# Farama-Foundation/Gymnasium-Robotics

Measured on AMD Instinct MI355X. Metric: env-steps/s (whole node), higher is better.
Workload: dtype f32

## Files before the change

__graft_entry__.py:

```python
import os
import subprocess
import sys

ROOT = os.path.dirname(os.path.abspath(__file__))
sys.path.insert(0, ROOT)

HIP_SRC = os.path.join(ROOT, "gymnasium_robotics_amd", "csrc", "grx_kernels.hip")
import glob

HIP_DEPS = sorted(glob.glob(os.path.join(ROOT, "gymnasium_robotics_amd", "csrc", "*.h")) + glob.glob(os.path.join(ROOT, "include", "*")))
HIP_SO = os.path.join(ROOT, "gymnasium_robotics_amd", "_lib", "libgrx_hip.so")
ENV_SRC = os.path.join(ROOT, "gymnasium_robotics_amd", "csrc", "grx_env.hip")
ENV_DEPS = [os.path.join(ROOT, "include", "grx_env.h"), os.path.join(ROOT, "include", "grx_replay.h"), os.path.join(ROOT, "include", "grx_capi.h"),
            os.path.join(ROOT, "gymnasium_robotics_amd", "csrc", "grx_env_maze.inc"), os.path.join(ROOT, "gymnasium_robotics_amd", "csrc", "grx_env_replay.inc")]
ENV_SO = os.path.join(ROOT, "gymnasium_robotics_amd", "_lib", "libgrx_env.so")


HIPCC_FLAGS = ["--offload-arch=gfx950", "-O3", "-std=c++17", "-shared", "-fPIC", "-fno-hip-fp32-correctly-rounded-divide-sqrt"]
HIP_UNITS = ("FETCH", "HAND", "POINT", "ADROIT", "KITCHEN", "API")


def _stale(target, deps):
    return not os.path.exists(target) or any(os.path.getmtime(d) > os.path.getmtime(target) for d in deps)


def build_hip(out=HIP_SO, extra_flags=()):
    hipcc = os.environ.get("HIPCC", "/opt/rocm/bin/hipcc")
    objdir = os.path.join(os.path.dirname(out), ".obj_" + os.path.splitext(os.path.basename(out))[0])
    os.makedirs(objdir, exist_ok=True)
    compile_flags = [f for f in HIPCC_FLAGS if f != "-shared"] + list(extra_flags)
    procs = []
    for u in HIP_UNITS:
        obj = os.path.join(objdir, f"grx_{u.lower()}.o")
        procs.append((obj, subprocess.Popen([hipcc] + compile_flags + [f"-DGRX_TU_{u}=1", "-c", "-o", obj, HIP_SRC])))
    for obj, p in procs:
        if p.wait() != 0:
            raise subprocess.CalledProcessError(p.returncode, p.args)
    subprocess.check_call([hipcc, "--offload-arch=gfx950", "-shared", "-fPIC", "-o", out] + [o for o, _ in procs])


def build_env(out=ENV_SO):
    hipcc = os.environ.get("HIPCC", "/opt/rocm/bin/hipcc")
    subprocess.check_call([hipcc, "--offload-arch=gfx950", "-O3", "-std=c++17", "-shared", "-fPIC", "-I", os.path.join(ROOT, "include"), "-o", out, ENV_SRC,
                           "-L", os.path.dirname(HIP_SO), "-lgrx_hip", "-Wl,-rpath,$ORIGIN"])


def build(force: bool = False) -> None:
    os.makedirs(os.path.dirname(HIP_SO), exist_ok=True)
    if force or _stale(HIP_SO, [HIP_SRC] + HIP_DEPS):
        build_hip()
    if force or _stale(ENV_SO, [ENV_SRC, HIP_SO] + ENV_DEPS):
        build_env()
    from oracle import oracle_sim

    oracle_sim.build(force)
    sys.path.insert(0, os.path.join(ROOT, "tests", "emu"))
    import emu_sim

    emu_sim.build(force)
    import gymnasium_robotics_amd
    from gymnasium_robotics_amd import _native

    _native.lib()


def smoke() -> None:
    import numpy as np
# ... 31 lines not shown
```

gymnasium_robotics_amd/_native.py:

```python
import ctypes
import os

_HERE = os.path.dirname(os.path.abspath(__file__))
LIB_PATH = os.environ.get("GRX_HIP_LIB") or os.path.join(_HERE, "_lib", "libgrx_hip.so")
_lib = None


class OverflowLaneStruct(ctypes.Structure):
    _fields_ = [(n, ctypes.c_void_p) for n in ("skip", "entry_count", "entry_list", "list", "count", "next_flags", "next_count", "next_list", "ttl")] + [
        (n, ctypes.c_int) for n in ("soft_maxefc", "soft_jpool", "soft_maxcon", "ttl_init", "grid", "entry_cap", "next_cap")] + [
        (n, ctypes.c_void_p) for n in ("ready", "progress", "poll_list")] + [(n, ctypes.c_int) for n in ("ready_cap", "progress_total", "poll_grid", "pad_")]


class FetchBuffersStruct(ctypes.Structure):
    _fields_ = [(n, ctypes.c_void_p) for n in (
        "qpos", "qvel", "qacc_ws", "mocap", "aux", "goal", "action", "obs", "achieved", "reward", "success", "status", "mask", "order", "cost", "packed", "hullcache", "handoff")] + [
        ("handoff_stride", ctypes.c_int), ("handoff_large", ctypes.c_int), ("split_state", ctypes.c_void_p), ("split_parts", ctypes.c_int), ("split_pad_", ctypes.c_int), ("lane", OverflowLaneStruct)]


class FetchResetArgsStruct(ctypes.Structure):
    _fields_ = [(n, ctypes.c_void_p) for n in ("idx", "samples", "init_qpos", "init_qvel", "init_mocap")] + [("obj_qadr", ctypes.c_int), ("keep_outcome", ctypes.c_int), ("final_packed", ctypes.c_void_p)]


class PointTaskStruct(ctypes.Structure):
    _fields_ = [("n_substeps", ctypes.c_int), ("sparse_reward", ctypes.c_int), ("continuing_task", ctypes.c_int), ("agent", ctypes.c_int),
                ("goal_radius", ctypes.c_double), ("vel_clip", ctypes.c_float)]


class PointBuffersStruct(ctypes.Structure):
    _fields_ = [(n, ctypes.c_void_p) for n in (
        "qpos", "qvel", "qacc_ws", "goal", "action", "obs", "achieved", "reward", "success", "terminated", "status", "mask", "packed", "split_state")] + [
        ("split_parts", ctypes.c_int), ("split_pad_", ctypes.c_int)]


class AdroitTaskStruct(ctypes.Structure):
    _fields_ = [("n_substeps", ctypes.c_int), ("sparse_reward", ctypes.c_int), ("kind", ctypes.c_int), ("site", ctypes.c_int * 5), ("obj_body", ctypes.c_int),
                ("nq_obs", ctypes.c_int), ("obs_dim", ctypes.c_int), ("qadr", ctypes.c_int * 2), ("len", ctypes.c_float * 2)]


class AdroitBuffersStruct(ctypes.Structure):
    _fields_ = [(n, ctypes.c_void_p) for n in ("qpos", "qvel", "qacc_ws", "shift", "target", "action", "act_mean", "act_rng", "obs", "reward", "success", "status", "mask")] + [("lane", OverflowLaneStruct), ("compact", ctypes.c_void_p), ("n_compact", ctypes.c_int), ("order", ctypes.c_void_p), ("cost", ctypes.c_void_p), ("split_rows", ctypes.c_void_p), ("split_state", ctypes.c_void_p), ("split_stride", ctypes.c_int), ("split_parts", ctypes.c_int)]


class KitchenTaskStruct(ctypes.Structure):
    _fields_ = [("n_substeps", ctypes.c_int), ("obs_dim", ctypes.c_int), ("dt", ctypes.c_float), ("vel_lo", ctypes.c_float * 9), ("vel_hi", ctypes.c_float * 9),
                ("pos_lo", ctypes.c_float * 9), ("pos_hi", ctypes.c_float * 9), ("noise_scale", ctypes.c_float * 59), ("task_adr", ctypes.c_int * 7),
                ("task_num", ctypes.c_int * 7), ("task_goal", ctypes.c_float * 17), ("bonus_thresh", ctypes.c_float)]


class KitchenBuffersStruct(ctypes.Structure):
    _fields_ = [(n, ctypes.c_void_p) for n in ("qpos", "qvel", "qacc_ws", "last_qpos", "action", "noise", "obs", "completed", "status", "mask", "skin")] + [
        ("skin_stride", ctypes.c_int), ("skin_radius", ctypes.c_float), ("order", ctypes.c_void_p), ("cost", ctypes.c_void_p), ("lane", OverflowLaneStruct),
        ("split_rows", ctypes.c_void_p), ("split_state", ctypes.c_void_p), ("split_stride", ctypes.c_int), ("split_parts", ctypes.c_int)]


class KitchenBookStruct(ctypes.Structure):
    _fields_ = [(n, ctypes.c_void_p) for n in ("completed", "stepped", "tasks_to_complete", "episode_completions", "elapsed", "step_completions", "reward", "terminated",
                                               "truncated", "needs_reset", "reset_now", "qpos", "qvel", "qacc_ws", "init_qpos")] + [
        (n, ctypes.c_int) for n in ("nq", "nv", "all_mask", "max_steps", "remove_when_completed", "terminate_when_completed", "mode")] + [("final_info", ctypes.c_void_p)]


class HerArgsStruct(ctypes.Structure):
    _fields_ = [("rows", ctypes.c_void_p), ("acts", ctypes.c_void_p)] + [(n, ctypes.c_int) for n in ("T", "N", "W", "obs_dim", "goal_dim", "act_dim")] + [
        (n, ctypes.c_void_p) for n in ("t_idx", "w_idx", "t_goal")] + [("kind", ctypes.c_int), ("p0", ctypes.c_double), ("p1", ctypes.c_double)] + [
        (n, ctypes.c_int) for n in ("sparse", "ignore_pos", "ignore_rot", "ignore_z")] + [("out", ctypes.c_void_p), ("term_rows", ctypes.c_void_p), ("term_t", ctypes.c_void_p)]


class MazeResetArgsStruct(ctypes.Structure):
    _fields_ = [(n, ctypes.c_void_p) for n in ("idx", "stage", "qpos0")] + [(n, ctypes.c_int) for n in ("nq", "nv", "obs_dim", "obs_skip")] + [
        ("goal_radius", ctypes.c_double), ("keep_outcome", ctypes.c_int)] + [
        (n, ctypes.c_void_p) for n in ("qpos", "qvel", "qacc_ws", "goal", "obs", "achieved", "reward", "success", "packed")]


class HandCommitArgsStruct(ctypes.Structure):
    _fields_ = [("idx", ctypes.c_void_p), ("k", ctypes.c_int)] + [(n, ctypes.c_int) for n in ("nq", "nv", "obs_dim", "goal_dim")] + [
        (n, ctypes.c_void_p) for n in ("s_qpos", "s_qvel", "s_qacc_ws", "s_obs", "s_achieved", "s_palm", "s_goal", "s_packed", "s_status",
                                       "qpos", "qvel", "qacc_ws", "obs", "achieved", "palm", "goal", "packed", "status")]


class FetchCommitArgsStruct(ctypes.Structure):
    _fields_ = [("idx", ctypes.c_void_p), ("k", ctypes.c_int)] + [(n, ctypes.c_int) for n in ("nq", "nv", "mocap_words", "obs_dim")] + [
        (n, ctypes.c_void_p) for n in ("s_qpos", "s_qvel", "s_qacc_ws", "s_mocap", "s_aux", "s_goal", "s_obs", "s_achieved", "s_status",
                                       "qpos", "qvel", "qacc_ws", "mocap", "aux", "goal", "obs", "achieved", "packed", "final_packed", "status")]


class AdroitCommitArgsStruct(ctypes.Structure):
    _fields_ = [("idx", ctypes.c_void_p), ("k", ctypes.c_int)] + [(n, ctypes.c_int) for n in ("nq", "nv", "obs_dim")] + [
        (n, ctypes.c_void_p) for n in ("s_qpos", "s_qvel", "s_qacc_ws", "s_shift", "s_target", "s_obs", "s_status", "qpos", "qvel", "qacc_ws", "shift", "target", "obs", "status")]


class HandBuffersStruct(ctypes.Structure):
    _fields_ = [(n, ctypes.c_void_p) for n in (
        "qpos", "qvel", "qacc_ws", "goal", "action", "obs", "achieved", "palm", "reward", "success", "status", "mask", "order", "cost", "packed")] + [("lane", OverflowLaneStruct),
        ("split_rows", ctypes.c_void_p), ("split_state", ctypes.c_void_p), ("split_stride", ctypes.c_int), ("split_parts", ctypes.c_int)]


def lib():
    global _lib
    if _lib is None:
        if not os.path.exists(LIB_PATH):
            raise RuntimeError(
                f"HIP extension not built: {LIB_PATH} is missing. Run `python -c 'import __graft_entry__ as g; g.build()'` "
                "(hipcc --offload-arch=gfx950). There is no CPU fallback.")
        import torch

        L = ctypes.CDLL(LIB_PATH)
        vp, ci = ctypes.c_void_p, ctypes.c_int
        L.grx_last_error.restype = ctypes.c_char_p
        L.grx_model_create.argtypes = [vp, ci, vp, ci, vp, ci, ci, ctypes.POINTER(vp)]
        L.grx_model_destroy.argtypes = [vp]
        L.grx_model_set_table.argtypes = [vp, ctypes.c_char_p, vp, ci]
        L.grx_model_lds_bytes.argtypes = [vp]
        L.grx_model_dim.argtypes = [vp, ctypes.c_char_p]
        L.grx_fetch_step.argtypes = [vp, vp, vp, ci, vp]
        L.grx_fetch_forward.argtypes = [vp, vp, vp, ci, ci, vp]
        L.grx_fetch_reset.argtypes = [vp, vp, vp, vp, ci, vp]
        L.grx_fetch_compute_reward.argtypes = [vp, vp, ctypes.c_int64, ctypes.c_double, ci, vp, vp]
        L.grx_her_relabel.argtypes = [vp, ctypes.c_int64, vp]
        L.grx_her_sample.argtypes = [vp, ci, ci, ci, ci, ctypes.c_uint64, ctypes.c_uint64, ctypes.c_int64, vp, vp, vp, vp]
        L.grx_her_sample_final.argtypes = [vp, vp, vp, ci, ci, ci, ci, ctypes.c_uint64, ctypes.c_uint64, ctypes.c_int64, vp, vp, vp, vp]
        L.grx_her_mark_resets.argtypes = [vp, ci, ci, vp, vp, vp, vp]
        L.grx_her_sample_relabel.argtypes = [vp, vp, vp, ci, ci, ctypes.c_uint64, ctypes.c_uint64, ctypes.c_int64, vp, vp, vp]
        L.grx_kitchen_step.argtypes = [vp, vp, vp, ci, ci, vp]
        L.grx_sample_uniform_rows.argtypes = [vp, vp, ci, ci, vp]
        L.grx_uniform_rows_device.argtypes = [vp, vp, ci, ci, vp, vp]
        L.grx_kitchen_bookkeeping.argtypes = [vp, ci, vp]
        L.grx_point_step.argtypes = [vp, vp, vp, ci, vp]
        L.grx_maze_compute_reward.argtypes = [vp, vp, ctypes.c_int64, ctypes.c_double, ci, vp, vp]
        L.grx_hand_step.argtypes = [vp, vp, vp, ci, ci, vp]
        L.grx_hand_step_repeat.argtypes = [vp, vp, vp, ci, ci, vp]
        L.grx_adroit_step.argtypes = [vp, vp, vp, ci, ci, vp]
        L.grx_goal_compute_reward.argtypes = [vp, vp, ctypes.c_int64, ci, ctypes.c_double, ci, vp, vp]
        L.grx_manip_compute_reward.argtypes = [vp, vp, ctypes.c_int64, ci, ci, ci, ctypes.c_float, ctypes.c_float, ci, vp, vp]
        L.grx_order_by_cost.argtypes = [vp, vp, ctypes.c_float, ci, vp, vp]
        L.grx_order_by_cost_slots.argtypes = [vp, vp, ctypes.c_float, ci, ci, vp, vp]
        L.grx_maze_reset_rows.argtypes = [vp, ci, vp]
        L.grx_hand_commit_rows.argtypes = [vp, vp]
        L.grx_fetch_commit_rows.argtypes = [vp, vp]
        L.grx_adroit_commit_rows.argtypes = [vp, vp]
        cd = ctypes.c_double
        L.grx_fetch_sample_resets.argtypes = [vp, vp, ci, ci, ci, cd, cd, vp, vp, cd, vp, vp]
        L.grx_fetch_sample_resets_device.argtypes = [vp, vp, ci, ci, ci, cd, cd, vp, vp, cd, vp, vp]
        L.grx_adroit_sample_resets_device.argtypes = [vp, vp, ci, ci, vp, vp, vp, vp, vp, vp]
        L.grx_maze_sample_resets_device.argtypes = [vp, vp, ci, vp, ci, vp, ci, cd, cd, vp, vp, vp, vp]
        _lib = L
    return _lib


def build_id(path: str = None) -> str:
    import hashlib
    import struct

    with open(path or LIB_PATH, "rb") as f:
        blob = f.read()
    if blob[:4] != b"\x7fELF" or blob[4] != 2:
        raise RuntimeError("libgrx_hip.so is not an ELF64 file")
    shoff, = struct.unpack_from("<Q", blob, 0x28)
    shentsize, shnum, shstrndx = struct.unpack_from("<HHH", blob, 0x3A)
    sec = lambda i: struct.unpack_from("<IIQQQQIIQQ", blob, shoff + i * shentsize)
    stroff = sec(shstrndx)[4]
    for i in range(shnum):
        name, _, _, _, off, size = sec(i)[:6]
        end = blob.index(b"\0", stroff + name)
        if blob[stroff + name: end] == b".hip_fatbin":
            return hashlib.sha256(blob[off: off + size]).hexdigest()[:16]
    raise RuntimeError("libgrx_hip.so holds no .hip_fatbin section (not a HIP build)")


def check(rc: int):
    if rc != 0:
        raise RuntimeError("libgrx_hip: " + lib().grx_last_error().decode())


EXPORTED_SYMBOLS = [
    "grx_model_create", "grx_model_destroy", "grx_model_set_table", "grx_model_lds_bytes", "grx_model_dim",
    "grx_fetch_step", "grx_fetch_forward", "grx_fetch_reset", "grx_fetch_compute_reward", "grx_her_relabel", "grx_her_sample", "grx_her_sample_final", "grx_her_mark_resets", "grx_her_sample_relabel", "grx_fetch_sample_resets", "grx_fetch_sample_resets_device", "grx_adroit_sample_resets_device", "grx_maze_sample_resets_device", "grx_point_step", "grx_maze_compute_reward", "grx_hand_step", "grx_hand_step_repeat", "grx_adroit_step", "grx_kitchen_step", "grx_sample_uniform_rows", "grx_uniform_rows_device", "grx_kitchen_bookkeeping", "grx_goal_compute_reward", "grx_manip_compute_reward", "grx_order_by_cost", "grx_order_by_cost_slots", "grx_maze_reset_rows", "grx_maze_reset_rows_list", "grx_maze_sample_resets_list", "grx_maze_episode_end", "grx_hand_commit_rows", "grx_fetch_commit_rows", "grx_adroit_commit_rows", "grx_last_error",
]


_MODEL_LOCK = __import__("threading").Lock()
_MODELS = {}
_MODEL_KEYS = {}


def acquire_model(H, I, F, device_index):
    import hashlib

    key = (int(device_index), hashlib.sha1(H.tobytes() + I.tobytes() + F.tobytes()).hexdigest(), os.environ.get("GRX_NO_HULLCELLS") is not None)
    with _MODEL_LOCK:
        ent = _MODELS.get(key)
        if ent is None:
            h = ctypes.c_void_p()
            check(lib().grx_model_create(H.ctypes.data, H.size, I.ctypes.data, I.size, F.ctypes.data, F.size, int(device_index), ctypes.byref(h)))
            ent = _MODELS[key] = [h, 0]
            _MODEL_KEYS[h.value] = key
        ent[1] += 1
        return ent[0]


def release_model(h):
    if h is None or not getattr(h, "value", None):
        return
    with _MODEL_LOCK:
        key = _MODEL_KEYS.get(h.value)
        if key is None:
            return
        ent = _MODELS[key]
        ent[1] -= 1
        if ent[1] <= 0:
            del _MODELS[key], _MODEL_KEYS[h.value]
            lib().grx_model_destroy(h)
```

gymnasium_robotics_amd/csrc/grx_env.hip:

```cpp
#include <hip/hip_runtime.h>

#include <sys/random.h>

#include <cstdio>
#include <cstring>
#include <map>
#include <string>
#include <vector>

#include "grx_capi.h"
#include "grx_env.h"
#include "grx_replay.h"

namespace {

constexpr int kEntryCap = 256;
constexpr int kSplitParts = 4;
constexpr int kSplitWide = 12288;
constexpr double kLaneMargin = 0.8;
constexpr int kLaneTtl = 4;
constexpr float kBalanceAlpha = 0.1f;
constexpr int kHullWords = 90;
constexpr int kPinSlots = 16;

thread_local std::string g_err;
int fail(int code, const std::string& msg) { g_err = msg; return code; }

#define ENV_HIP(expr) do { hipError_t e_ = (expr); if (e_ != hipSuccess) return fail(GRX_ENV_EHIP, std::string(#expr) + ": " + hipGetErrorString(e_)); } while (0)
#define ENV_GRX(expr) do { if ((expr) != 0) return fail(GRX_ENV_EHIP, std::string(#expr) + ": " + grx_last_error()); } while (0)
#define ENV_TRY(expr) do { int r_ = (expr); if (r_ != 0) return r_; } while (0)

__global__ void __launch_bounds__(64) grx_env_mask_kernel(unsigned char* __restrict__ mask, const int* __restrict__ idx, int k) {
  const int j = blockIdx.x * 64 + threadIdx.x;
  if (j < k) mask[idx[j]] = 0;
}

__global__ void __launch_bounds__(64) grx_env_zero_outcome_kernel(float* __restrict__ reward, float* __restrict__ packed, int pdim, const int* __restrict__ idx, int k) {
  const int j = blockIdx.x * 64 + threadIdx.x;
  if (j >= k) return;
  const int w = idx[j];
  reward[w] = 0.0f;
  packed[(size_t)w * pdim + pdim - 2] = 0.0f;
}

__global__ void __launch_bounds__(64) grx_env_gather_kernel(float* __restrict__ rows, const float* __restrict__ src, int width, const int* __restrict__ idx, int k) {
  const int j = blockIdx.x * 64 + threadIdx.x;
  if (j >= k) return;
  const float* s = src + (size_t)idx[j] * width;
  float* d = rows + (size_t)j * width;
  for (int c = 0; c < width; ++c) d[c] = s[c];
}

__global__ void __launch_bounds__(64) grx_env_scatter_rng_kernel(unsigned long long* __restrict__ rng, const unsigned long long* __restrict__ rows, const int* __restrict__ idx, int k) {
  const int j = blockIdx.x * 64 + threadIdx.x;
  if (j >= k) return;
  for (int c = 0; c < 4; ++c) rng[(size_t)idx[j] * 4 + c] = rows[(size_t)j * 4 + c];
}

unsigned blocks(int k) { return (unsigned)((k + 63) / 64); }

void pcg64_from_entropy(const std::vector<uint32_t>& ent, uint64_t out[4]) {
  const uint32_t INIT_A = 0x43b0d7e5u, MULT_A = 0x931e8875u, INIT_B = 0x8b51f9ddu, MULT_B = 0x58f38dedu, MIX_L = 0xca01f9ddu, MIX_R = 0x4973f715u;
  uint32_t hc = INIT_A, pool[4];
  auto hashmix = [&hc, MULT_A](uint32_t v) { v ^= hc; hc *= MULT_A; v *= hc; v ^= v >> 16; return v; };
  auto mix = [MIX_L, MIX_R](uint32_t x, uint32_t y) { uint32_t r = MIX_L * x - MIX_R * y; r ^= r >> 16; return r; };
// ... 119 lines not shown
struct MazeEnv;
void maze_free(MazeEnv* m);

int parse_desc(const Container& c, Desc* d) {
  ENV_TRY(take<int32_t>(c, "H", -1, &d->H));
  ENV_TRY(take<int32_t>(c, "I", -1, &d->I));
  ENV_TRY(take<double>(c, "F", -1, &d->F));
  ENV_TRY(take<int32_t>(c, "H_rerun", (int64_t)(d->H.size() * 4), &d->Hr));
  ENV_TRY(take<int32_t>(c, "I_rerun", (int64_t)(d->I.size() * 4), &d->Ir));
  ENV_TRY(take<double>(c, "F_rerun", (int64_t)(d->F.size() * 8), &d->Fr));
  ENV_TRY(take<uint8_t>(c, "task", sizeof(grx_fetch_task), nullptr, &d->task));
  ENV_TRY(take<int32_t>(c, "dims", sizeof d->dims, nullptr, d->dims));
  ENV_TRY(take<double>(c, "consts", sizeof d->consts, nullptr, d->consts));
  ENV_TRY(take<int32_t>(c, "fast_caps", sizeof d->caps, nullptr, d->caps));
  const int nq = d->dims[0], nv = d->dims[1], nmocap = d->dims[2], obs_dim = d->dims[4];
  if (nq <= 0 || nv <= 0 || nmocap != 1 || obs_dim != d->task.obs_dim || d->task.goal_dim != 3 || d->dims[5] >= nq)
    return fail(GRX_ENV_EDESC, "environment description: inconsistent sizes: dims (nq " + std::to_string(nq) + ", nv " + std::to_string(nv) + ", nmocap " + std::to_string(nmocap) +
                                   ", obs_dim " + std::to_string(obs_dim) + ") disagree with the task struct (obs_dim " + std::to_string(d->task.obs_dim) + ")");
  ENV_TRY(take<double>(c, "q0", (int64_t)nq * 8, &d->q0));
  ENV_TRY(take<double>(c, "mocap0", (int64_t)nmocap * 56, &d->mocap0));
  return 0;
}

}

struct grx_env {
  int device = 0, n = 0, mode = GRX_ENV_NEXT_STEP, max_steps = 0;
  uint64_t seed_offset = 0;
  Desc d;
  MazeEnv* mz = nullptr;
  grx_model *h = nullptr, *hbig = nullptr;
  int nq = 0, nv = 0, nmocap = 0, nu = 0, obs_dim = 0, pdim = 0, obj_qadr = -1;
  double g0[3] = {0, 0, 0}, toff[3] = {0, 0, 0}, height_offset = 0, dt = 0;
  int soft[4] = {0, 0, 0, 0};
  std::vector<void*> allocs;
  float *qpos, *qvel, *qacc_ws, *mocap, *aux, *goal, *action, *obs, *achieved, *reward, *packed, *final_packed, *final_rows, *hullcache, *cost_ema = nullptr;
  unsigned char *success, *mask;
  int *status, *cost = nullptr, *order = nullptr;
  float* split_rows = nullptr;
  int* split_state = nullptr;
  uint64_t *rng, *rng_rows;
  float *init_qpos, *init_qvel, *init_mocap;
  int *idx_main, *idx_ahead;
  float *samp_main, *samp_ahead;
  int* lane_head;
  int *lane_next_list, *lane_entry_list;
  signed char* lane_ttl;
  size_t lane_head_bytes = 0;
  float *a_qpos, *a_qvel, *a_qacc_ws, *a_mocap, *a_aux, *a_goal, *a_obs, *a_achieved, *a_reward;
  unsigned char* a_success;
  int* a_status;
  grx_fetch_buffers bufs{}, bufs_masked{}, lane_plain{}, lane_masked{}, ahead_bufs{};
  bool balance = false, ahead = false;
  int slots_per_xcd = 0, split = 1;
  hipStream_t side = nullptr;
  hipEvent_t ev_before = nullptr, ev_ahead = nullptr;
  void* pin[kPinSlots] = {};
  hipEvent_t pin_ev[kPinSlots] = {};
  bool pin_live[kPinSlots] = {};
  size_t pin_bytes = 0;
  int pin_next = 0;
  std::vector<int64_t> elapsed;
  std::vector<uint8_t> needs_reset, terminated, truncated;
  std::vector<int32_t> final_idx, list, will;
  int n_final = 0;
  uint8_t has_reset = 0;
  grx_replay* replay = nullptr;
  const int* step_list = nullptr;
  const int* step_count_dev = nullptr;
  int step_count = 0;
  uint64_t steps = 0, epoch = 0;

  ~grx_env() {
    (void)hipSetDevice(device);
    if (side) (void)hipStreamSynchronize(side);
    (void)hipDeviceSynchronize();
    for (int s = 0; s < kPinSlots; ++s) {
      if (pin_ev[s]) (void)hipEventDestroy(pin_ev[s]);
      if (pin[s]) (void)hipHostFree(pin[s]);
    }
    if (ev_before) (void)hipEventDestroy(ev_before);
    if (ev_ahead) (void)hipEventDestroy(ev_ahead);
    if (side) (void)hipStreamDestroy(side);
    for (void* p : allocs) (void)hipFree(p);
    if (h) grx_model_destroy(h);
    if (hbig) grx_model_destroy(hbig);
    maze_free(mz);
  }

  template <class T>
  int zalloc(T** p, size_t count) {
    void* q = nullptr;
    ENV_HIP(hipMalloc(&q, count * sizeof(T) > 0 ? count * sizeof(T) : 1));
    allocs.push_back(q);
    ENV_HIP(hipMemset(q, 0, count * sizeof(T)));
    *p = (T*)q;
    return 0;
  }

  int upload(void* dst, const void* src, size_t bytes, hipStream_t s) {
    if (bytes == 0) return 0;
    const int k = pin_next;
    pin_next = (pin_next + 1) % kPinSlots;
    if (pin_live[k] && hipEventQuery(pin_ev[k]) == hipErrorNotReady) ENV_HIP(hipEventSynchronize(pin_ev[k]));
    std::memcpy(pin[k], src, bytes);
    ENV_HIP(hipMemcpyAsync(dst, pin[k], bytes, hipMemcpyHostToDevice, s));
    ENV_HIP(hipEventRecord(pin_ev[k], s));
    pin_live[k] = true;
    return 0;
  }
};

namespace {

struct DeviceGuard {
  int prev = -1;
  explicit DeviceGuard(int dev) { if (hipGetDevice(&prev) != hipSuccess) prev = -1; if (prev != dev) (void)hipSetDevice(dev); }
  ~DeviceGuard() { int cur; if (prev >= 0 && hipGetDevice(&cur) == hipSuccess && cur != prev) (void)hipSetDevice(prev); }
};

grx_fetch_buffers make_bufs(grx_env* e, float* qpos, float* qvel, float* qacc, float* mocap, float* aux, float* goal, float* obs, float* ach, float* rew, unsigned char* succ,
                            int* status, const unsigned char* mask, const int* order, int* cost, float* packed, float* hullcache) {
  grx_fetch_buffers b;
  std::memset(&b, 0, sizeof b);
  b.qpos = qpos; b.qvel = qvel; b.qacc_ws = qacc; b.mocap = mocap; b.aux = aux; b.goal = goal; b.action = e->action; b.obs = obs; b.achieved = ach;
  b.reward = rew; b.success = succ; b.status = status; b.mask = mask; b.order = order; b.cost = cost; b.packed = packed; b.hullcache = hullcache;
  return b;
}

int launch_step(grx_env* e, bool masked, hipStream_t s) {
  grx_fetch_buffers& fb = masked ? e->bufs_masked : e->bufs;
  ENV_HIP(hipMemsetAsync(e->lane_head, 0, e->lane_head_bytes, s));
  int* counts = e->lane_head + (e->lane_head_bytes / 4 - 2);
  std::memset(&fb.lane, 0, sizeof fb.lane);
  fb.lane.entry_count = counts + 1; fb.lane.entry_list = e->lane_entry_list; fb.lane.entry_cap = kEntryCap;
  const int rc = grx_fetch_step(e->h, &e->d.task, &fb, e->n, s);
  std::memset(&fb.lane, 0, sizeof fb.lane);
  if (rc != 0) return fail(GRX_ENV_EHIP, std::string("grx_fetch_step: ") + grx_last_error());
  grx_fetch_buffers& b = masked ? e->lane_masked : e->lane_plain;
  std::memset(&b.lane, 0, sizeof b.lane);
  b.lane.grid = kEntryCap; b.lane.list = e->lane_entry_list; b.lane.count = counts + 1;
  b.lane.next_flags = (unsigned char*)e->lane_head; b.lane.next_count = counts; b.lane.next_list = e->lane_next_list; b.lane.ttl = e->lane_ttl; b.lane.next_cap = 0;
  b.lane.soft_maxefc = e->soft[0]; b.lane.soft_jpool = e->soft[1]; b.lane.soft_maxcon = e->soft[2]; b.lane.ttl_init = e->soft[3];
  ENV_GRX(grx_fetch_step(e->hbig, &e->d.task, &b, e->n, s));
  if (e->balance) ENV_GRX(grx_order_by_cost_slots(e->cost, e->cost_ema, kBalanceAlpha, e->n, e->slots_per_xcd, e->order, s));
  return 0;
}

int sample_resets(grx_env* e, const int* idx_dev, int k, float* samples, hipStream_t s) {
  const double* c = e->d.consts;
  ENV_GRX(grx_fetch_sample_resets_device(e->rng, idx_dev, k, (int)c[0], (int)c[2], c[7], c[8], e->toff, e->g0, e->height_offset, samples, s));
  return 0;
}

int reset_inline(grx_env* e, const int* idx_dev, int k, const float* samples, bool keep_outcome, hipStream_t s) {
  grx_fetch_reset_args a;
  std::memset(&a, 0, sizeof a);
  a.idx = idx_dev; a.samples = samples; a.init_qpos = e->init_qpos; a.init_qvel = e->init_qvel; a.init_mocap = e->init_mocap; a.obj_qadr = e->obj_qadr;
  a.keep_outcome = keep_outcome ? 1 : 0; a.final_packed = keep_outcome ? e->final_packed : nullptr;
  ENV_GRX(grx_fetch_reset(e->h, &e->d.task, &e->bufs, &a, k, s));
  return 0;
}

void mark_reset(grx_env* e, const std::vector<int32_t>& idx) {
  for (int w : idx) { e->elapsed[w] = 0; e->needs_reset[w] = 0; }
}

int env_setup(grx_env* e) {
  grx_env one;
  one.device = e->device;
  float *qpos, *qvel, *qacc, *mocap, *aux, *goal, *action, *obs, *ach, *rew, *packed, *hull;
  unsigned char* succ;
  int* status;
  ENV_TRY(one.zalloc(&qpos, e->nq)); ENV_TRY(one.zalloc(&qvel, e->nv)); ENV_TRY(one.zalloc(&qacc, e->nv)); ENV_TRY(one.zalloc(&mocap, 7 * e->nmocap));
  ENV_TRY(one.zalloc(&aux, 8)); ENV_TRY(one.zalloc(&goal, 3)); ENV_TRY(one.zalloc(&action, 4)); ENV_TRY(one.zalloc(&obs, e->obs_dim)); ENV_TRY(one.zalloc(&ach, 3));
  ENV_TRY(one.zalloc(&rew, 1)); ENV_TRY(one.zalloc(&succ, 1)); ENV_TRY(one.zalloc(&status, 1)); ENV_TRY(one.zalloc(&packed, e->pdim)); ENV_TRY(one.zalloc(&hull, kHullWords));
  one.action = action;
  grx_fetch_buffers b = make_bufs(&one, qpos, qvel, qacc, mocap, aux, goal, obs, ach, rew, succ, status, nullptr, nullptr, nullptr, packed, hull);
  std::vector<float> q0(e->d.q0.begin(), e->d.q0.end()), m0(e->d.mocap0.begin(), e->d.mocap0.end());
  ENV_HIP(hipMemcpy(qpos, q0.data(), q0.size() * 4, hipMemcpyHostToDevice));
  ENV_HIP(hipMemcpy(mocap, m0.data(), m0.size() * 4, hipMemcpyHostToDevice));
  hipStream_t s = e->side;
  ENV_GRX(grx_fetch_forward(e->h, &e->d.task, &b, 1, 0, s));
  ENV_HIP(hipStreamSynchronize(s));
  float o[3];
  ENV_HIP(hipMemcpy(o, obs, 12, hipMemcpyDeviceToHost));
  const double geh = e->d.consts[3];
  const double target[3] = {-0.498 + (double)o[0], 0.005 + (double)o[1], (-0.431 + geh) + (double)o[2]};
  const float mrow[7] = {(float)target[0], (float)target[1], (float)target[2], 1.0f, 0.0f, 1.0f, 0.0f};
  ENV_HIP(hipMemcpy(mocap, mrow, sizeof mrow, hipMemcpyHostToDevice));
  ENV_GRX(grx_fetch_forward(e->h, &e->d.task, &b, 1, 10 * e->d.task.n_substeps, s));
  ENV_HIP(hipStreamSynchronize(s));
  int st = 0;
  float a[3];
  ENV_HIP(hipMemcpy(&st, status, 4, hipMemcpyDeviceToHost));
  if (st != 0) return fail(GRX_ENV_EHIP, "engine reported status " + std::to_string(st) + " during env setup");
  ENV_HIP(hipMemcpy(o, obs, 12, hipMemcpyDeviceToHost));
  ENV_HIP(hipMemcpy(a, ach, 12, hipMemcpyDeviceToHost));
  for (int i = 0; i < 3; ++i) e->g0[i] = (double)o[i];
  e->height_offset = e->d.consts[0] != 0.0 ? (double)a[2] : 0.0;
  ENV_HIP(hipMemcpy(e->init_qpos, qpos, e->nq * 4, hipMemcpyDeviceToDevice));
  ENV_HIP(hipMemcpy(e->init_qvel, qvel, e->nv * 4, hipMemcpyDeviceToDevice));
  ENV_HIP(hipMemcpy(e->init_mocap, m0.data(), m0.size() * 4, hipMemcpyHostToDevice));
  return 0;
}

int alloc_all(grx_env* e) {
  const int n = e->n;
  ENV_TRY(e->zalloc(&e->qpos, (size_t)n * e->nq)); ENV_TRY(e->zalloc(&e->qvel, (size_t)n * e->nv)); ENV_TRY(e->zalloc(&e->qacc_ws, (size_t)n * e->nv));
  ENV_TRY(e->zalloc(&e->mocap, (size_t)n * 7 * e->nmocap)); ENV_TRY(e->zalloc(&e->aux, (size_t)n * 8)); ENV_TRY(e->zalloc(&e->goal, (size_t)n * 3));
  ENV_TRY(e->zalloc(&e->action, (size_t)n * 4)); ENV_TRY(e->zalloc(&e->obs, (size_t)n * e->obs_dim)); ENV_TRY(e->zalloc(&e->achieved, (size_t)n * 3));
  ENV_TRY(e->zalloc(&e->reward, n)); ENV_TRY(e->zalloc(&e->success, n)); ENV_TRY(e->zalloc(&e->status, n)); ENV_TRY(e->zalloc(&e->mask, n));
  ENV_HIP(hipMemset(e->mask, 1, n));
  ENV_TRY(e->zalloc(&e->packed, (size_t)n * e->pdim)); ENV_TRY(e->zalloc(&e->final_packed, (size_t)n * e->pdim)); ENV_TRY(e->zalloc(&e->final_rows, (size_t)n * e->pdim));
  ENV_TRY(e->zalloc(&e->hullcache, (size_t)n * kHullWords));
  ENV_TRY(e->zalloc(&e->rng, (size_t)n * 4)); ENV_TRY(e->zalloc(&e->rng_rows, (size_t)n * 4));
  ENV_TRY(e->zalloc(&e->init_qpos, e->nq)); ENV_TRY(e->zalloc(&e->init_qvel, e->nv)); ENV_TRY(e->zalloc(&e->init_mocap, 7 * e->nmocap));
  ENV_TRY(e->zalloc(&e->idx_main, n)); ENV_TRY(e->zalloc(&e->idx_ahead, n)); ENV_TRY(e->zalloc(&e->samp_main, (size_t)n * 5)); ENV_TRY(e->zalloc(&e->samp_ahead, (size_t)n * 5));
  e->lane_head_bytes = (size_t)((n + 3) / 4 + 2) * 4;
  ENV_TRY(e->zalloc(&e->lane_head, e->lane_head_bytes / 4)); ENV_TRY(e->zalloc(&e->lane_next_list, n)); ENV_TRY(e->zalloc(&e->lane_entry_list, n)); ENV_TRY(e->zalloc(&e->lane_ttl, n));
  e->balance = n % 8 == 0 && n >= 1024 && n <= 65536 * 8;
  if (e->balance) {
    ENV_TRY(e->zalloc(&e->cost, n)); ENV_TRY(e->zalloc(&e->cost_ema, n)); ENV_TRY(e->zalloc(&e->order, n));
    const int lds = grx_model_lds_bytes(e->h);
    const int granules = (lds + 1279) / 1280;
    const int per_cu = granules > 0 ? (160 * 1024) / (granules * 1280) : 8;
    e->slots_per_xcd = 32 * (per_cu < 8 ? per_cu : 8);
    std::vector<int> ord(n);
    const int per = n / 8;
    for (int j = 0; j < n; ++j) ord[j] = (j % 8) * per + j / 8;
    ENV_HIP(hipMemcpy(e->order, ord.data(), (size_t)n * 4, hipMemcpyHostToDevice));
  }
  e->bufs = make_bufs(e, e->qpos, e->qvel, e->qacc_ws, e->mocap, e->aux, e->goal, e->obs, e->achieved, e->reward, e->success, e->status, nullptr, e->order, e->cost, e->packed, e->hullcache);
  e->bufs_masked = e->bufs;
  e->bufs_masked.mask = e->mask;
  e->lane_plain = make_bufs(e, e->qpos, e->qvel, e->qacc_ws, e->mocap, e->aux, e->goal, e->obs, e->achieved, e->reward, e->success, e->status, nullptr, nullptr, nullptr, e->packed,
                            e->hullcache);
  e->lane_masked = e->lane_plain;
  e->lane_masked.mask = e->mask;
  e->split = n >= 64 && n > 2048 ? (n <= kSplitWide ? kSplitParts : 2) : 1;
  if (e->split > 1) {
    const int stride = (2 + e->nu + 7 * e->nmocap + e->nq + 2 * e->nv + 15) / 16 * 16;
    ENV_TRY(e->zalloc(&e->split_rows, (size_t)n * stride)); ENV_TRY(e->zalloc(&e->split_state, (size_t)n * 2));
    for (grx_fetch_buffers* b : {&e->bufs, &e->bufs_masked}) { b->handoff = e->split_rows; b->handoff_stride = stride; b->split_state = e->split_state; b->split_parts = e->split; }
  }
  e->ahead = n > 1;
  if (e->ahead) {
    ENV_TRY(e->zalloc(&e->a_qpos, (size_t)n * e->nq)); ENV_TRY(e->zalloc(&e->a_qvel, (size_t)n * e->nv)); ENV_TRY(e->zalloc(&e->a_qacc_ws, (size_t)n * e->nv));
    ENV_TRY(e->zalloc(&e->a_mocap, (size_t)n * 7 * e->nmocap)); ENV_TRY(e->zalloc(&e->a_aux, (size_t)n * 8)); ENV_TRY(e->zalloc(&e->a_goal, (size_t)n * 3));
    ENV_TRY(e->zalloc(&e->a_obs, (size_t)n * e->obs_dim)); ENV_TRY(e->zalloc(&e->a_achieved, (size_t)n * 3)); ENV_TRY(e->zalloc(&e->a_reward, n));
    ENV_TRY(e->zalloc(&e->a_success, n)); ENV_TRY(e->zalloc(&e->a_status, n));
    e->ahead_bufs = make_bufs(e, e->a_qpos, e->a_qvel, e->a_qacc_ws, e->a_mocap, e->a_aux, e->a_goal, e->a_obs, e->a_achieved, e->a_reward, e->a_success, e->a_status, nullptr,
                              nullptr, nullptr, nullptr, nullptr);
  }
  e->pin_bytes = (size_t)n * 32;
  for (int s = 0; s < kPinSlots; ++s) {
    ENV_HIP(hipHostMalloc(&e->pin[s], e->pin_bytes, hipHostMallocDefault));
    ENV_HIP(hipEventCreateWithFlags(&e->pin_ev[s], hipEventDisableTiming));
  }
  ENV_HIP(hipEventCreateWithFlags(&e->ev_before, hipEventDisableTiming));
  ENV_HIP(hipEventCreateWithFlags(&e->ev_ahead, hipEventDisableTiming));
  e->elapsed.assign(n, 0);
  e->needs_reset.assign(n, 0);
  e->terminated.assign(n, 0);
  e->truncated.assign(n, 0);
  e->final_idx.reserve(n);
  e->list.reserve(n);
  e->will.reserve(n);
  return 0;
}

struct Section { const char* name; void* ptr; size_t bytes; bool host; };

#include "grx_env_maze.inc"
// ... 154 lines not shown
  auto& L = e->list;
  L.clear();
  for (int i = 0; i < e->n; ++i)
    if (!mask || mask[i]) L.push_back(i);
  e->n_final = 0;
  std::fill(e->terminated.begin(), e->terminated.end(), 0);
  std::fill(e->truncated.begin(), e->truncated.end(), 0);
  e->has_reset = 1;
  const int k = (int)L.size();
  if (k == 0) return 0;
  ENV_TRY(e->upload(e->idx_main, L.data(), (size_t)k * 4, s));
  if (seeds) {
    std::vector<uint64_t> rows((size_t)k * 4);
    for (int j = 0; j < k; ++j) pcg64_from_seed(seeds[L[j]], &rows[(size_t)j * 4]);
    ENV_TRY(e->upload(e->rng_rows, rows.data(), rows.size() * 8, s));
    hipLaunchKernelGGL(grx_env_scatter_rng_kernel, dim3(blocks(k)), dim3(64), 0, s, (unsigned long long*)e->rng, (const unsigned long long*)e->rng_rows, e->idx_main, k);
    ENV_HIP(hipGetLastError());
  }
  ENV_TRY(sample_resets(e, e->idx_main, k, e->samp_main, s));
  ENV_TRY(reset_inline(e, e->idx_main, k, e->samp_main, false, s));
  mark_reset(e, L);
  return 0;
}

extern "C" int grx_env_step(grx_env* e, const float* actions, void* stream) {
  if (!e) return fail(GRX_ENV_EINVAL, "grx_env_step: NULL handle");
  if (!actions) return fail(GRX_ENV_EINVAL, "grx_env_step: actions is NULL");
  if (!e->has_reset) return fail(GRX_ENV_EINVAL, "grx_env_step: cannot step before grx_env_reset");
  DeviceGuard g(e->device);
  hipStream_t s = (hipStream_t)stream;
  e->steps += 1;
  e->step_list = nullptr; e->step_count_dev = nullptr; e->step_count = 0;
  if (e->mz) return maze_step(e, actions, s);
  const int n = e->n;
  ENV_HIP(hipMemcpyAsync(e->action, actions, (size_t)n * 16, hipMemcpyDefault, s));
  auto& pending = e->list;
  pending.clear();
  if (e->mode == GRX_ENV_NEXT_STEP)
    for (int i = 0; i < n; ++i)
      if (e->needs_reset[i]) pending.push_back(i);
  auto& will = e->will;
  will.clear();
  if (e->ahead && e->mode == GRX_ENV_SAME_STEP && e->max_steps > 0)
    for (int i = 0; i < n; ++i)
      if (e->elapsed[i] + 1 >= e->max_steps) will.push_back(i);
  const int kp = (int)pending.size(), kw = (int)will.size();
  if (kw) ENV_HIP(hipEventRecord(e->ev_before, s));
  if (kp) {
    ENV_TRY(e->upload(e->idx_main, pending.data(), (size_t)kp * 4, s));
    ENV_HIP(hipMemsetAsync(e->mask, 1, n, s));
    hipLaunchKernelGGL(grx_env_mask_kernel, dim3(blocks(kp)), dim3(64), 0, s, e->mask, (const int*)e->idx_main, kp);
    ENV_HIP(hipGetLastError());
  }
  ENV_TRY(launch_step(e, kp > 0, s));
  if (kw) {
    ENV_HIP(hipStreamWaitEvent(e->side, e->ev_before, 0));
    ENV_TRY(e->upload(e->idx_ahead, will.data(), (size_t)kw * 4, e->side));
    ENV_TRY(sample_resets(e, e->idx_ahead, kw, e->samp_ahead, e->side));
    grx_fetch_reset_args a;
    std::memset(&a, 0, sizeof a);
    a.idx = e->idx_ahead; a.samples = e->samp_ahead; a.init_qpos = e->init_qpos; a.init_qvel = e->init_qvel; a.init_mocap = e->init_mocap; a.obj_qadr = e->obj_qadr;
    a.keep_outcome = 1; a.final_packed = nullptr;
    ENV_GRX(grx_fetch_reset(e->h, &e->d.task, &e->ahead_bufs, &a, kw, e->side));
    ENV_HIP(hipEventRecord(e->ev_ahead, e->side));
  }
  e->n_final = 0;
  e->final_idx.clear();
  for (int i = 0; i < n; ++i) {
    const bool stepped = !(kp && e->needs_reset[i]);
    if (stepped) e->elapsed[i] += 1;
    e->truncated[i] = stepped && e->max_steps > 0 && e->elapsed[i] >= e->max_steps;
    e->terminated[i] = 0;
    if (e->truncated[i]) e->final_idx.push_back(i);
  }
  if (kp) {
    ENV_TRY(sample_resets(e, e->idx_main, kp, e->samp_main, s));
    ENV_TRY(reset_inline(e, e->idx_main, kp, e->samp_main, false, s));
    mark_reset(e, pending);
    e->step_list = e->idx_main; e->step_count = kp;
    hipLaunchKernelGGL(grx_env_zero_outcome_kernel, dim3(blocks(kp)), dim3(64), 0, s, e->reward, e->packed, e->pdim, (const int*)e->idx_main, kp);
    ENV_HIP(hipGetLastError());
  }
  const int kd = (int)e->final_idx.size();
  if (e->mode == GRX_ENV_SAME_STEP && kd) {
    const int* idx_dev;
    if (kw) {
      if (kw != kd || !std::equal(will.begin(), will.end(), e->final_idx.begin()))
        return fail(GRX_ENV_EINVAL, "grx_env_step: the worlds reset ahead of the step are not the ones it truncated");
      ENV_HIP(hipStreamWaitEvent(s, e->ev_ahead, 0));
      grx_fetch_commit_args c;
      std::memset(&c, 0, sizeof c);
      c.idx = e->idx_ahead; c.k = kd; c.nq = e->nq; c.nv = e->nv; c.mocap_words = 7 * e->nmocap; c.obs_dim = e->obs_dim;
      c.s_qpos = e->a_qpos; c.s_qvel = e->a_qvel; c.s_qacc_ws = e->a_qacc_ws; c.s_mocap = e->a_mocap; c.s_aux = e->a_aux; c.s_goal = e->a_goal; c.s_obs = e->a_obs;
      c.s_achieved = e->a_achieved; c.s_status = e->a_status;
      c.qpos = e->qpos; c.qvel = e->qvel; c.qacc_ws = e->qacc_ws; c.mocap = e->mocap; c.aux = e->aux; c.goal = e->goal; c.obs = e->obs; c.achieved = e->achieved;
      c.packed = e->packed; c.final_packed = e->final_packed; c.status = e->status;
      ENV_GRX(grx_fetch_commit_rows(&c, s));
      idx_dev = e->idx_ahead;
    } else {
      ENV_TRY(e->upload(e->idx_main, e->final_idx.data(), (size_t)kd * 4, s));
      ENV_TRY(sample_resets(e, e->idx_main, kd, e->samp_main, s));
      ENV_TRY(reset_inline(e, e->idx_main, kd, e->samp_main, true, s));
      idx_dev = e->idx_main;
    }
    mark_reset(e, e->final_idx);
    hipLaunchKernelGGL(grx_env_gather_kernel, dim3(blocks(kd)), dim3(64), 0, s, e->final_rows, (const float*)e->final_packed, e->pdim, idx_dev, kd);
    ENV_HIP(hipGetLastError());
    e->n_final = kd;
    e->step_list = idx_dev; e->step_count = kd;
  } else {
    if (e->mode == GRX_ENV_NEXT_STEP)
      for (int w : e->final_idx) e->needs_reset[w] = 1;
    e->final_idx.clear();
  }
  return 0;
}

extern "C" int grx_env_outputs(const grx_env* e, grx_env_device_outputs* out) {
  if (!e || !out) return fail(GRX_ENV_EINVAL, "grx_env_outputs: NULL argument");
  if (e->mz) return maze_outputs(e, out);
  out->num_envs = e->n; out->obs_dim = e->obs_dim; out->goal_dim = 3; out->packed_dim = e->pdim;
  out->obs = e->obs; out->achieved = e->achieved; out->desired = e->goal; out->reward = e->reward; out->success = e->success; out->status = e->status; out->packed = e->packed;
  out->terminated = e->terminated.data(); out->truncated = e->truncated.data();
  out->n_final = e->n_final; out->final_idx = e->final_idx.data(); out->final_rows = e->final_rows;
  return 0;
}

extern "C" int grx_env_copy_outputs(grx_env* e, grx_env_host_outputs* out) {
  if (!e || !out) return fail(GRX_ENV_EINVAL, "grx_env_copy_outputs: NULL argument");
  DeviceGuard g(e->device);
  if (e->mz) return maze_copy_outputs(e, out);
  ENV_HIP(hipDeviceSynchronize());
  const size_t n = e->n;
  auto d2h = [](void* dst, const void* src, size_t bytes) { return (dst && bytes) ? hipMemcpy(dst, src, bytes, hipMemcpyDeviceToHost) : hipSuccess; };
  ENV_HIP(d2h(out->obs, e->obs, n * e->obs_dim * 4));
  ENV_HIP(d2h(out->achieved, e->achieved, n * 12));
  ENV_HIP(d2h(out->desired, e->goal, n * 12));
  ENV_HIP(d2h(out->reward, e->reward, n * 4));
  ENV_HIP(d2h(out->success, e->success, n));
  ENV_HIP(d2h(out->status, e->status, n * 4));
  ENV_HIP(d2h(out->packed, e->packed, n * e->pdim * 4));
  ENV_HIP(d2h(out->final_rows, e->final_rows, (size_t)e->n_final * e->pdim * 4));
  if (out->terminated) std::memcpy(out->terminated, e->terminated.data(), n);
  if (out->truncated) std::memcpy(out->truncated, e->truncated.data(), n);
  if (out->n_final) *out->n_final = e->n_final;
  if (out->final_idx && e->n_final) std::memcpy(out->final_idx, e->final_idx.data(), (size_t)e->n_final * 4);
  return 0;
}

extern "C" int grx_env_compute_reward(const grx_env* e, const float* achieved, const float* desired, int64_t batch, float* out, void* stream) {
  if (!e || !achieved || !desired || !out) return fail(GRX_ENV_EINVAL, "grx_env_compute_reward: NULL argument");
  if (batch < 0) return fail(GRX_ENV_EINVAL, "grx_env_compute_reward: negative batch");
  DeviceGuard g(e->device);
  if (e->mz) {
    ENV_GRX(grx_maze_compute_reward(achieved, desired, batch, e->mz->d.task.goal_radius, e->mz->d.task.sparse_reward, out, stream));
    return 0;
  }
  ENV_GRX(grx_fetch_compute_reward(achieved, desired, batch, e->d.task.distance_threshold, e->d.task.sparse_reward, out, stream));
  return 0;
}

extern "C" int grx_env_state_size(const grx_env* e, size_t* bytes) {
  if (!e || !bytes) return fail(GRX_ENV_EINVAL, "grx_env_state_size: NULL argument");
  *bytes = state_layout(const_cast<grx_env*>(e), nullptr);
  return 0;
}

// ... 63 lines not shown
```

gymnasium_robotics_amd/csrc/grx_env_replay.inc:

```

struct grx_replay {
  grx_env* e = nullptr;
  int T = 0, R = 0, n = 0, W = 0, od = 0, gd = 0, ad = 0, OW = 0;
  int64_t capacity = 0, max_batch = 0, head = 0, size = 0;
  uint64_t seed = 0, calls = 0;
  bool track = false;
  float *episode = nullptr, *actions = nullptr, *rows = nullptr, *term_rows = nullptr;
  int *start = nullptr, *prev_start = nullptr, *term_t = nullptr, *scratch = nullptr, *valid = nullptr;
  std::vector<void*> allocs;
  int t = 0;
  bool begun = false;
  uint64_t epoch = 0, last_step = 0;
  grx_her_args ha{};
};

namespace {

struct ReplayAppend {
  const float *packed, *action;
  float *row_dst, *act_dst;
  long long n_row, n_act;
  const int* list;
  const int* count_dev;
  int count, max_n, t;
  int *start, *prev_start, *term_t;
  const float* final_rows;
  float* term_rows;
  int W;
};

__device__ __forceinline__ void replay_copy(float* __restrict__ dst, const float* __restrict__ src, long long n, long long tid, long long nth) {
  if ((((uintptr_t)dst | (uintptr_t)src) & 15) == 0) {
    const long long n4 = n >> 2;
    const float4* __restrict__ s4 = (const float4*)src;
    float4* __restrict__ d4 = (float4*)dst;
    for (long long i = tid; i < n4; i += nth) d4[i] = s4[i];
    for (long long i = (n4 << 2) + tid; i < n; i += nth) dst[i] = src[i];
  } else {
    for (long long i = tid; i < n; i += nth) dst[i] = src[i];
  }
}

__global__ void __launch_bounds__(256) grx_replay_append_kernel(ReplayAppend a) {
  const long long tid = (long long)blockIdx.x * blockDim.x + threadIdx.x, nth = (long long)gridDim.x * blockDim.x;
  replay_copy(a.row_dst, a.packed, a.n_row, tid, nth);
  replay_copy(a.act_dst, a.action, a.n_act, tid, nth);
  int k = a.count_dev ? *a.count_dev : a.count;
  k = k < 0 ? 0 : (k > a.max_n ? a.max_n : k);
  for (long long j = tid; j < k; j += nth) {
    const int w = a.list[j];
    if ((unsigned)w >= (unsigned)a.max_n) continue;
    if (a.prev_start) { a.prev_start[w] = a.start[w]; a.term_t[w] = a.t; }
    a.start[w] = a.t;
  }
  if (a.term_rows)
    for (long long i = tid; i < (long long)k * a.W; i += nth) {
      const long long j = i / a.W;
      const int w = a.list[j];
      if ((unsigned)w < (unsigned)a.max_n) a.term_rows[(size_t)w * a.W + (i - j * a.W)] = a.final_rows[i];
    }
}

__global__ void __launch_bounds__(256) grx_replay_begin_kernel(const float* __restrict__ packed, float* __restrict__ row0, long long n_row, const long long* __restrict__ elapsed, int n,
                                                               int* __restrict__ start, int* __restrict__ prev_start, int* __restrict__ term_t) {
  const long long tid = (long long)blockIdx.x * blockDim.x + threadIdx.x, nth = (long long)gridDim.x * blockDim.x;
  replay_copy(row0, packed, n_row, tid, nth);
  for (long long w = tid; w < n; w += nth) {
    if (elapsed) start[w] = -(int)elapsed[w];
    prev_start[w] = 0;
    term_t[w] = -1;
  }
}

unsigned replay_blocks(long long words) {
  long long b = (words / 4 + 255) / 256;
  return (unsigned)(b < 1 ? 1 : (b > 1024 ? 1024 : b));
}

const float* replay_packed(const grx_env* e) { return e->mz ? e->mz->packed : e->packed; }
const float* replay_action(const grx_env* e) { return e->mz ? e->mz->action : e->action; }

template <class T>
int replay_zalloc(grx_replay* r, T** p, size_t count) {
  void* q = nullptr;
  ENV_HIP(hipMalloc(&q, count * sizeof(T) > 0 ? count * sizeof(T) : 1));
  r->allocs.push_back(q);
  ENV_HIP(hipMemset(q, 0, count * sizeof(T)));
  *p = (T*)q;
  return 0;
}

void replay_free(grx_replay* r) {
  for (void* p : r->allocs) (void)hipFree(p);
  delete r;
}

}

extern "C" int grx_replay_create(grx_env* e, const grx_replay_config* cfg, grx_replay** out) {
  if (!out) return fail(GRX_ENV_EINVAL, "grx_replay_create: out is NULL");
  *out = nullptr;
  if (!cfg) return fail(GRX_ENV_EINVAL, "grx_replay_create: NULL config");
  if (cfg->horizon < 1 || cfg->horizon > (1 << 20)) return fail(GRX_ENV_EINVAL, "grx_replay_create: horizon " + std::to_string(cfg->horizon) + " out of range (>= 1)");
  if (cfg->capacity < 1) return fail(GRX_ENV_EINVAL, "grx_replay_create: capacity " + std::to_string(cfg->capacity) + " out of range (>= 1)");
  if (cfg->max_batch > cfg->capacity)
    return fail(GRX_ENV_EINVAL, "grx_replay_create: batch " + std::to_string(cfg->max_batch) + " larger than the replay capacity " + std::to_string(cfg->capacity));
  if (!e) return fail(GRX_ENV_EINVAL, "grx_replay_create: NULL handle");
  if (e->replay) return fail(GRX_ENV_EINVAL, "grx_replay_create: the handle already has a replay attached");
  DeviceGuard g(e->device);
  grx_replay* r = new grx_replay();
  r->e = e;
  r->T = cfg->horizon; r->R = r->T + 1; r->n = e->n; r->W = e->pdim; r->od = e->obs_dim; r->gd = e->mz ? 2 : 3; r->ad = e->mz ? e->mz->nu : 4;
  r->OW = 2 * r->od + 3 * r->gd + r->ad + 2;
  r->capacity = cfg->capacity; r->max_batch = cfg->max_batch > 0 ? cfg->max_batch : cfg->capacity;
  r->seed = cfg->seed;
  r->track = cfg->keep_final != 0 && e->mode == GRX_ENV_SAME_STEP;
  const size_t n = (size_t)r->n;
  int rc = [&]() -> int {
    ENV_TRY(replay_zalloc(r, &r->episode, (size_t)r->R * n * r->W));
    ENV_TRY(replay_zalloc(r, &r->actions, (size_t)r->R * n * r->ad));
    ENV_TRY(replay_zalloc(r, &r->rows, (size_t)r->capacity * r->OW));
    ENV_TRY(replay_zalloc(r, &r->start, n)); ENV_TRY(replay_zalloc(r, &r->prev_start, n)); ENV_TRY(replay_zalloc(r, &r->term_t, n));
    ENV_TRY(replay_zalloc(r, &r->scratch, (size_t)3 * r->max_batch)); ENV_TRY(replay_zalloc(r, &r->valid, 1));
    ENV_HIP(hipMemset(r->term_t, 0xFF, n * 4));
    if (r->track) {
      if (e->mz) ENV_TRY(replay_zalloc(r, &r->term_rows, n * r->W));
      else r->term_rows = e->final_packed;
    }
    ENV_HIP(hipDeviceSynchronize());
    return 0;
  }();
  if (rc != 0) { std::string msg = g_err; replay_free(r); g_err = msg; return rc; }
  grx_her_args& a = r->ha;
  std::memset(&a, 0, sizeof a);
  a.rows = r->episode; a.acts = r->actions; a.T = r->T; a.N = r->n; a.W = r->W; a.obs_dim = r->od; a.goal_dim = r->gd; a.act_dim = r->ad;
  if (e->mz) { a.kind = 2; a.p0 = e->mz->d.task.goal_radius; a.sparse = e->mz->d.task.sparse_reward; }
  else { a.kind = 0; a.p0 = e->d.task.distance_threshold; a.sparse = e->d.task.sparse_reward; }
  if (r->track) { a.term_rows = r->term_rows; a.term_t = r->term_t; }
  e->replay = r;
  *out = r;
  return 0;
}

extern "C" int grx_replay_destroy(grx_replay* r) {
  if (!r) return fail(GRX_ENV_EINVAL, "grx_replay_destroy: NULL replay");
  DeviceGuard g(r->e->device);
  (void)hipDeviceSynchronize();
  r->e->replay = nullptr;
  replay_free(r);
  return 0;
}

extern "C" int grx_replay_dims(const grx_replay* r, int* row_width, int* obs_dim, int* goal_dim, int* act_dim) {
  if (!r) return fail(GRX_ENV_EINVAL, "grx_replay_dims: NULL replay");
  if (row_width) *row_width = r->OW;
  if (obs_dim) *obs_dim = r->od;
  if (goal_dim) *goal_dim = r->gd;
  if (act_dim) *act_dim = r->ad;
  return 0;
}

extern "C" int grx_replay_begin(grx_replay* r, void* stream) {
  if (!r) return fail(GRX_ENV_EINVAL, "grx_replay_begin: NULL replay");
  grx_env* e = r->e;
  if (!e->has_reset) return fail(GRX_ENV_EINVAL, "grx_replay_begin: cannot begin before grx_env_reset");
  DeviceGuard g(e->device);
  hipStream_t s = (hipStream_t)stream;
  const long long* elapsed_dev = nullptr;
  if (e->mz && !e->mz->host_book) elapsed_dev = e->mz->elapsed;
  else {
    const std::vector<int64_t>& el = e->mz ? e->mz->h_elapsed : e->elapsed;
    std::vector<int32_t> neg((size_t)r->n);
    for (int i = 0; i < r->n; ++i) neg[i] = -(int32_t)el[i];
    ENV_TRY(e->upload(r->start, neg.data(), (size_t)r->n * 4, s));
  }
  const long long n_row = (long long)r->n * r->W;
  hipLaunchKernelGGL(grx_replay_begin_kernel, dim3(replay_blocks(n_row)), dim3(256), 0, s, replay_packed(e), r->episode, n_row, elapsed_dev, r->n, r->start, r->prev_start, r->term_t);
  ENV_HIP(hipGetLastError());
  r->t = 0;
  r->begun = true;
  r->epoch = e->epoch;
  r->last_step = e->steps;
  return 0;
}

extern "C" int grx_replay_append(grx_replay* r, void* stream) {
  if (!r) return fail(GRX_ENV_EINVAL, "grx_replay_append: NULL replay");
  grx_env* e = r->e;
  if (!r->begun) return fail(GRX_ENV_EINVAL, "grx_replay_append: append before grx_replay_begin");
  if (e->epoch != r->epoch) return fail(GRX_ENV_EINVAL, "grx_replay_append: grx_env_reset / grx_env_set_state since grx_replay_begin: call grx_replay_begin again");
  if (e->steps == r->last_step) return fail(GRX_ENV_EINVAL, "grx_replay_append: no grx_env_step since the last append (double append)");
  if (e->steps != r->last_step + 1) return fail(GRX_ENV_EINVAL, "grx_replay_append: " + std::to_string(e->steps - r->last_step) + " steps since the last append: every step is appended");
  if (r->t == INT32_MAX - 1) return fail(GRX_ENV_EINVAL, "grx_replay_append: row counter exhausted: call grx_replay_begin");
  DeviceGuard g(e->device);
  const int t = r->t + 1, row = t % r->R;
  ReplayAppend a;
  std::memset(&a, 0, sizeof a);
  a.packed = replay_packed(e); a.action = replay_action(e);
  a.n_row = (long long)r->n * r->W; a.n_act = (long long)r->n * r->ad;
  a.row_dst = r->episode + (size_t)row * a.n_row; a.act_dst = r->actions + (size_t)row * a.n_act;
  a.list = e->step_list; a.count_dev = e->step_count_dev; a.count = e->step_list ? e->step_count : 0; a.max_n = r->n; a.t = t;
  a.start = r->start;
  if (r->track) {
    a.prev_start = r->prev_start; a.term_t = r->term_t;
    if (e->mz) { a.final_rows = e->mz->final_rows; a.term_rows = r->term_rows; }
  }
  a.W = r->W;
  hipLaunchKernelGGL(grx_replay_append_kernel, dim3(replay_blocks(a.n_row)), dim3(256), 0, (hipStream_t)stream, a);
  ENV_HIP(hipGetLastError());
  r->t = t;
  r->last_step = e->steps;
  return 0;
}

extern "C" int grx_replay_relabel(grx_replay* r, int64_t batch, int k_future, grx_replay_batch* out, void* stream) {
  if (!r) return fail(GRX_ENV_EINVAL, "grx_replay_relabel: NULL replay");
  if (batch < 1) return fail(GRX_ENV_EINVAL, "grx_replay_relabel: batch " + std::to_string(batch) + " out of range (>= 1)");
  if (batch > r->capacity) return fail(GRX_ENV_EINVAL, "grx_replay_relabel: batch " + std::to_string(batch) + " larger than the replay capacity " + std::to_string(r->capacity));
  if (batch > r->max_batch) return fail(GRX_ENV_EINVAL, "grx_replay_relabel: batch " + std::to_string(batch) + " larger than max_batch " + std::to_string(r->max_batch));
  if (k_future < 0) return fail(GRX_ENV_EINVAL, "grx_replay_relabel: negative k_future");
  DeviceGuard g(r->e->device);
  if (r->head + batch > r->capacity) r->head = 0;
  grx_her_args a = r->ha;
  a.out = r->rows + (size_t)r->head * r->OW;
  ENV_GRX(grx_her_sample_relabel(&a, r->start, r->track ? r->prev_start : nullptr, r->t, k_future, r->seed, r->calls, batch, r->scratch, r->valid, stream));
  r->calls += 1;
  if (out) { out->rows = a.out; out->batch = batch; out->offset = r->head; out->valid = r->valid; }
  r->head += batch;
  if (r->head > r->size) r->size = r->head;
  return 0;
}

extern "C" int grx_replay_reseed(grx_replay* r, uint64_t seed) {
  if (!r) return fail(GRX_ENV_EINVAL, "grx_replay_reseed: NULL replay");
  r->seed = seed;
  r->calls = 0;
  return 0;
}

extern "C" int grx_replay_ring(const grx_replay* r, const float** rows, int64_t* capacity, int64_t* head, int64_t* size) {
  if (!r) return fail(GRX_ENV_EINVAL, "grx_replay_ring: NULL replay");
  if (rows) *rows = r->rows;
  if (capacity) *capacity = r->capacity;
  if (head) *head = r->head;
  if (size) *size = r->size;
  return 0;
}
```

gymnasium_robotics_amd/csrc/grx_kernels.hip:

```cpp
#if !defined(GRX_TU_FETCH) && !defined(GRX_TU_HAND) && !defined(GRX_TU_POINT) && !defined(GRX_TU_ADROIT) && !defined(GRX_TU_KITCHEN) && !defined(GRX_TU_API)
#define GRX_TU_FETCH 1
#define GRX_TU_HAND 1
#define GRX_TU_POINT 1
#define GRX_TU_ADROIT 1
#define GRX_TU_KITCHEN 1
#define GRX_TU_API 1
#endif
#if GRX_TU_FETCH && !defined(GRX_NO_HULL_HINTS)
#define GRX_HULL_HINTS 1
#endif
#include <hip/hip_runtime.h>

#include <cmath>
#include <cstdio>
#include <cstring>
#include <string>

#include "../../include/grx_capi.h"
#include "grx_fetch_task.h"
#include "grx_point_task.h"
#include "grx_hand_task.h"
#include "grx_adroit_task.h"
#include "grx_kitchen_task.h"
#include "grx_host_model.h"

static_assert(sizeof(grx_fetch_task) == sizeof(GrxFetchTask), "grx_fetch_task must mirror GrxFetchTask");
static_assert(sizeof(grx_fetch_buffers) == sizeof(GrxFetchBuffers), "grx_fetch_buffers must mirror GrxFetchBuffers");
static_assert(sizeof(grx_point_task) == sizeof(GrxPointTask), "grx_point_task must mirror GrxPointTask");
static_assert(sizeof(grx_point_buffers) == sizeof(GrxPointBuffers), "grx_point_buffers must mirror GrxPointBuffers");
static_assert(sizeof(grx_hand_task) == sizeof(GrxHandTask), "grx_hand_task must mirror GrxHandTask");
static_assert(sizeof(grx_hand_buffers) == sizeof(GrxHandBuffers), "grx_hand_buffers must mirror GrxHandBuffers");
static_assert(sizeof(grx_adroit_task) == sizeof(GrxAdroitTask), "grx_adroit_task must mirror GrxAdroitTask");
static_assert(sizeof(grx_adroit_buffers) == sizeof(GrxAdroitBuffers), "grx_adroit_buffers must mirror GrxAdroitBuffers");
static_assert(sizeof(grx_kitchen_task) == sizeof(GrxKitchenTask), "grx_kitchen_task must mirror GrxKitchenTask");
static_assert(sizeof(grx_kitchen_buffers) == sizeof(GrxKitchenBuffers), "grx_kitchen_buffers must mirror GrxKitchenBuffers");

__device__ __forceinline__ void grx_load_world(const GrxModel& m, const GrxFetchBuffers& b, GrxCtx& c, int w, float* lds, int words, int lane_) {
  for (int i = lane_; i < words; i += 64) lds[i] = 0.0f;
  __syncthreads();
  for (int i = lane_; i < m.nq; i += 64) c.qpos[i] = b.qpos[(size_t)w * m.nq + i];
  for (int i = lane_; i < m.nv; i += 64) { c.qvel[i] = b.qvel[(size_t)w * m.nv + i]; c.qacc_ws[i] = b.qacc_ws[(size_t)w * m.nv + i]; }
  for (int i = lane_; i < 7 * m.nmocap; i += 64) {
    int k = i / 7, e = i - 7 * k; float v = b.mocap[(size_t)w * 7 * m.nmocap + i];
    if (e < 3) c.mocap_pos[3 * k + e] = v; else c.mocap_quat[4 * k + e - 3] = v;
  }
  __syncthreads();
}

__device__ __forceinline__ int grx_status_word(int old, int now) { now &= 15; return now | ((((old >> 16) | now) & 0xFFFF) << 16); }

__device__ __forceinline__ void grx_lane_setup(const GrxLane& L, GrxCtx& c, int w, bool stepping) {
  c.bail = (stepping && L.entry_count != nullptr) ? 1 : 0;
  if (c.bail) { c.lane_entry_count = L.entry_count; c.lane_entry_list = L.entry_list; c.lane_entry_cap = L.entry_cap; c.lane_world = w; c.lane_ready = L.ready; c.lane_ready_cap = L.ready_cap; }
  if (stepping && (L.list != nullptr || L.entry_count != nullptr)) { c.soft_maxefc = L.soft_maxefc; c.soft_jpool = L.soft_jpool; c.soft_maxcon = L.soft_maxcon; }
}
__device__ __forceinline__ bool grx_lane_overflowed(const GrxCtx& c) { return c.bail == 2; }
__device__ __forceinline__ void grx_lane_append(const GrxLane& L, int w) {
  const int idx = atomicAdd(L.next_count, 1);
  if (idx < L.next_cap) { L.next_list[idx] = w; L.next_flags[w] = 1; }
}
__device__ __forceinline__ void grx_lane_join(const GrxLane& L, const GrxCtx& c, int w, int lane_) {
  if (L.entry_count == nullptr || L.next_list == nullptr || lane_ != 0 || !(c.cnt[2] & GRX_ST_SOFT)) return;
  L.ttl[w] = (signed char)L.ttl_init;
  grx_lane_append(L, w);
}
__device__ __forceinline__ void grx_lane_ticket(const GrxLane& L, int st, int w, int lane_) {
  if (L.list == nullptr || lane_ != 0) return;
  int t = L.ttl[w];
  if (st >= 0) { t = (st & GRX_ST_SOFT) ? L.ttl_init : (t > 0 ? t - 1 : 0); L.ttl[w] = (signed char)t; }
  else if (t <= 0) t = 1;
  if (t > 0) grx_lane_append(L, w);
}
__device__ __forceinline__ void grx_lane_progress(const GrxLane& L) { if (L.progress && threadIdx.x == 0) atomicAdd(L.progress, 1); }
__device__ __forceinline__ int grx_lane_taken(const GrxLane& L, int e) {
  if (!L.ready || L.poll_grid != 0 || e >= L.ready_cap) return 0;
  int r = 0;
  if (threadIdx.x == 0) r = atomicCAS(L.ready + e, 1, 2) != 1;
// ... 1003 lines not shown
extern "C" __global__ void __launch_bounds__(256)
grx_manip_reward_kernel(const float* __restrict__ ag, const float* __restrict__ dg, long long B, int ignore_pos, int ignore_rot, int ignore_z, float thr_pos, float thr_rot,
                        int sparse, float* __restrict__ out) {
  for (long long i = (long long)blockIdx.x * blockDim.x + threadIdx.x; i < B; i += (long long)gridDim.x * blockDim.x) {
    float dp, dr;
    grx_manip_distance(ag + i * 7, dg + i * 7, ignore_pos, ignore_rot, ignore_z, &dp, &dr);
    out[i] = grx_manip_reward(dp, dr, thr_pos, thr_rot, sparse);
  }
}

extern "C" __global__ void __launch_bounds__(256)
grx_maze_reward_kernel(const float* __restrict__ ag, const float* __restrict__ dg, long long B, double radius, int sparse, float* __restrict__ out) {
  for (long long i = (long long)blockIdx.x * blockDim.x + threadIdx.x; i < B; i += (long long)gridDim.x * blockDim.x) {
    float a[2] = {ag[2 * i], ag[2 * i + 1]}, g[2] = {dg[2 * i], dg[2 * i + 1]};
    out[i] = grx_maze_reward(grx_goal_distance2(a, g), radius, sparse);
  }
}

extern "C" __global__ void __launch_bounds__(256)
grx_fetch_reward_kernel(const float* __restrict__ ag, const float* __restrict__ dg, long long B, double thresh, int sparse, float* __restrict__ out) {
  for (long long i = (long long)blockIdx.x * blockDim.x + threadIdx.x; i < B; i += (long long)gridDim.x * blockDim.x) {
    float a[3] = {ag[3 * i], ag[3 * i + 1], ag[3 * i + 2]}, g[3] = {dg[3 * i], dg[3 * i + 1], dg[3 * i + 2]};
    out[i] = grx_fetch_reward(grx_goal_distance3(a, g), thresh, sparse);
  }
}

struct GrxHerArgs {
  const float* rows; const float* acts;
  int T, N, W, obs_dim, goal_dim, act_dim;
  const int *t_idx, *w_idx, *t_goal;
  int kind;
  double p0, p1;
  int sparse, ignore_pos, ignore_rot, ignore_z;
  float* out;
  const float* term_rows; const int* term_t;
};
static_assert(sizeof(grx_her_args) == sizeof(GrxHerArgs), "grx_her_args must mirror GrxHerArgs");
GRX_DEV void grx_her_outcome(const GrxHerArgs& a, const float* ag, const float* g, float* reward, float* success) {
  if (a.kind == 3) {
    float dp, dr;
    grx_manip_distance(ag, g, a.ignore_pos, a.ignore_rot, a.ignore_z, &dp, &dr);
    *reward = grx_manip_reward(dp, dr, (float)a.p0, (float)a.p1, a.sparse); *success = grx_manip_success(dp, dr, (float)a.p0, (float)a.p1) ? 1.0f : 0.0f;
  } else if (a.kind == 2) {
    const double d = grx_goal_distance2(ag, g);
    *reward = grx_maze_reward(d, a.p0, a.sparse); *success = (d <= a.p0) ? 1.0f : 0.0f;
  } else if (a.kind == 1) {
    const double d = grx_goal_distance_n(ag, g, a.goal_dim);
    *reward = grx_hand_reward(d, a.p0, a.sparse); *success = (d < a.p0) ? 1.0f : 0.0f;
  } else {
    const double d = grx_goal_distance3(ag, g);
    *reward = grx_fetch_reward(d, a.p0, a.sparse); *success = (d < a.p0) ? 1.0f : 0.0f;
  }
}
GRX_DEV float grx_her_word(const GrxHerArgs& a, long long b, int e) {
  const int od = a.obs_dim, gd = a.goal_dim, ad = a.act_dim, OW = 2 * od + 3 * gd + ad + 2;
  const int R = a.T + 1, t = a.t_idx[b] % R, t1 = (a.t_idx[b] + 1) % R, w = a.w_idx[b], tg = a.t_goal[b];
  const int tt = a.term_t ? a.term_t[w] : -1;
  const float* r0 = a.rows + ((size_t)t * a.N + w) * a.W;
  const float* r1 = (a.t_idx[b] + 1 == tt) ? a.term_rows + (size_t)w * a.W : a.rows + ((size_t)t1 * a.N + w) * a.W;
  const float* g = tg < 0 ? r0 + od + gd : ((tg == tt ? a.term_rows + (size_t)w * a.W : a.rows + ((size_t)(tg % R) * a.N + w) * a.W) + od);
  float v;
  if (e < od + gd) v = r0[e];
  else if (e < od + 2 * gd) v = g[e - od - gd];
  else if (e < od + 2 * gd + ad) v = a.acts[((size_t)t1 * a.N + w) * ad + (e - od - 2 * gd)];
  else if (e == od + 2 * gd + ad || e == OW - 1) {
    float ag[16], gg[16], rw, sc;
    for (int k = 0; k < gd; k++) { ag[k] = r1[od + k]; gg[k] = g[k]; }
    grx_her_outcome(a, ag, gg, &rw, &sc);
    v = (e == OW - 1) ? sc : rw;
  } else v = r1[e - (od + 2 * gd + ad + 1)];
  return v;
}
extern "C" __global__ void __launch_bounds__(256)
grx_her_relabel_kernel(GrxHerArgs a, long long B) {
  const int OW = 2 * a.obs_dim + 3 * a.goal_dim + a.act_dim + 2;
  for (long long i = (long long)blockIdx.x * blockDim.x + threadIdx.x; i < B * OW; i += (long long)gridDim.x * blockDim.x) {
    const long long b = i / OW;
    a.out[i] = grx_her_word(a, b, (int)(i - b * OW));
  }
}
extern "C" __global__ void __launch_bounds__(256)
grx_her_relabel_valid_kernel(GrxHerArgs a, long long B, const int* __restrict__ valid) {
  const int OW = 2 * a.obs_dim + 3 * a.goal_dim + a.act_dim + 2;
  const bool ok = *valid != 0;
  for (long long i = (long long)blockIdx.x * blockDim.x + threadIdx.x; i < B * OW; i += (long long)gridDim.x * blockDim.x) {
    const long long b = i / OW;
    a.out[i] = ok ? grx_her_word(a, b, (int)(i - b * OW)) : 0.0f;
  }
}

extern "C" __global__ void __launch_bounds__(64)
grx_debug_kernel(int mode, int nv, int nefc, const float* A_in, const float* b_in, const float* J_in, const float* D_in, float* out) {
  extern __shared__ float lds[];
  const int lane_ = threadIdx.x;
  GrxModel m; m.nv = nv;
  GrxCtx c;
  c.A = lds; c.M = c.A + nv * nv; c.Jp = c.M + nv * nv; c.efc_D = c.Jp + GRX_MAXEFC * nv; c.efc_jv = c.efc_D + GRX_MAXEFC;
  c.efc_quad = (int*)(c.efc_jv + GRX_MAXEFC); c.efc_row = c.efc_quad + GRX_MAXEFC; c.tmpv = (float*)(c.efc_row + GRX_MAXEFC);
  c.grad = c.tmpv + nv; c.efc_force = c.grad + nv; c.efc_id = (int*)(c.efc_force + GRX_MAXEFC);
  for (int i = lane_; i < nv * nv; i += 64) { c.A[i] = A_in[i]; c.M[i] = A_in[i]; }
  for (int i = lane_; i < nv; i += 64) c.tmpv[i] = b_in[i];
  const int na = nv / 3, nb = nv - nv / 3, two = (mode == 2), rl = two ? na + (nv - nb) : nv;
  for (int i = lane_; i < nefc * nv; i += 64) {
    const int r = i / nv, d = i - r * nv;
    if (!two) c.Jp[i] = J_in[i];
    else if (d < na) c.Jp[r * rl + d] = J_in[i];
    else if (d >= nb) c.Jp[r * rl + na + d - nb] = J_in[i];
  }
  for (int i = lane_; i < nefc; i += 64) {
    c.efc_D[i] = fabsf(D_in[i]); c.efc_quad[i] = D_in[i] > 0 ? 1 : 0; c.efc_force[i] = 0.5f + 0.01f * (float)i;
    c.efc_row[i] = GRX_ROW_PACK(i * rl, 0, two ? na : nv); c.efc_id[i] = two ? ((nb << 12) | ((nv - nb) << 20)) : 0;
  }
  __syncthreads();
  if (mode == 0) {
    GrxEngine<GrxShapeAny>::grx_sym_solve_full(c.A, nv, c.tmpv, lane_);
    for (int i = lane_; i < nv; i += 64) out[i] = c.tmpv[i];
  } else {
    GrxEngine<GrxShapeAny>::grx_hessian(&m, &c, nefc, lane_);
    for (int i = lane_; i < nv * nv; i += 64) out[i] = c.A[i];
    for (int i = lane_; i < nv; i += 64) out[nv * nv + i] = c.grad[i];
  }
}

static int g_slot_used[GRX_MAX_MODELS];

// ... 230 lines not shown
  const bool split = b.split_parts > 1 && !b.compact && !forward_only && !b.lane.list;
  if (split) {
    if (!b.split_state || !b.split_rows || b.split_stride < m->dev.nq + 2 * m->dev.nv) return fail("grx_adroit_step: a split step needs split_state [N, 4] and carrier rows split_rows [N, split_stride >= nq + 2 nv]");
    if (b.split_parts > t.n_substeps || b.split_parts > 8) return fail("grx_adroit_step: split_parts <= min(frame_skip, 8): a part runs whole substeps");
  } else b.split_parts = 0;
  const int e = grx_tu_adroit_launch(m->shape, (b.lane.list ? (unsigned)(b.lane.grid > 0 ? b.lane.grid : GRX_LANE_GRID) : (b.compact ? (unsigned)b.n_compact : (split ? (unsigned)b.split_parts : 1u) * grx_grid_for(n_worlds))), (size_t)m->words * 4 + m->lds_pad, stream, m->slot, &t, &b, n_worlds, m->words, forward_only);
  if (e) return fail(std::string("grx_adroit_step launch: ") + hipGetErrorString((hipError_t)e));
  return 0;
}

static const int32_t* grx_host_itable(const grx_model* m, const char* name, int* n) {
  for (size_t k = 0; k < m->pm.name.size(); k++)
    if (m->pm.kind[k] == 'i' && m->pm.name[k] == name) { *n = m->pm.cnt[k]; return m->pm.i.data() + m->pm.off[k]; }
  *n = 0; return nullptr;
}
static bool grx_planes_static(const grx_model* m) {
  int ng, nb, n;
  const int32_t *gt = grx_host_itable(m, "geom_type", &ng), *gb = grx_host_itable(m, "geom_bodyid", &n), *bp = grx_host_itable(m, "body_parent", &nb),
                *dn = grx_host_itable(m, "body_dofnum", &n), *mc = grx_host_itable(m, "body_mocapid", &n);
  if (!gt || !gb || !bp || !dn || !mc) return false;
  for (int g = 0; g < ng; g++) {
    if (gt[g] != 0) continue;
    for (int b = gb[g]; b > 0; b = bp[b]) if (dn[b] > 0 || mc[b] >= 0) return false;
  }
  return true;
}

extern "C" int grx_kitchen_step(const grx_model* m, const grx_kitchen_task* task, const grx_kitchen_buffers* buf, int n_worlds, int forward_only, void* stream) {
  if (!m || !task || !buf) return fail("grx_kitchen_step: null argument");
  if (!buf->qpos || !buf->qvel || !buf->qacc_ws || !buf->last_qpos || !buf->obs || !buf->completed || !buf->status) return fail("grx_kitchen_step: null buffer");
  if (!forward_only && !buf->action) return fail("grx_kitchen_step: null action buffer");
  if (n_worlds <= 0) return 0;
  GrxKitchenTask t; memcpy(&t, task, sizeof(t));
  GrxKitchenBuffers b; memcpy(&b, buf, sizeof(b));
  const GrxModel& g = m->dev;
  if (g.nu != GRX_KITCHEN_NROBOT || t.obs_dim != g.nq + g.nv || t.obs_dim > GRX_KITCHEN_OBS || t.n_substeps <= 0) return fail("grx_kitchen_step: the model is not the kitchen scene (nu 9, obs = nq + nv <= 59)");
  for (int j = 0; j < GRX_KITCHEN_NTASK; j++)
    if (t.task_adr[j] < 0 || t.task_num[j] < 0 || t.task_adr[j] + t.task_num[j] > g.nq) return fail("grx_kitchen_step: task qpos slice out of range");
  if (b.skin) {
    if (b.skin_stride < 4 + 3 * g.ngeom + g.ndevpair || !(b.skin_radius > 0.0f)) return fail("grx_kitchen_step: skin rows need 4 + 3 ngeom + ndevpair words and a positive radius");
    if (!grx_planes_static(m)) return fail("grx_kitchen_step: the skin list needs static plane geoms");
  }
  if (b.lane.list && m->shape != 0 && m->shape < 100) return fail("grx_kitchen_step: the large-table launch of the overflow lane needs a model that runs on the generic kernel (capacities that match no specialised shape)");
  const bool split = b.split_parts > 1 && !forward_only && !b.lane.list;
  if (split) {
    if (!b.split_state || !b.split_rows || b.split_stride < g.nq + 2 * g.nv) return fail("grx_kitchen_step: a split step needs split_state [N, 4] and carrier rows split_rows [N, split_stride >= nq + 2 nv]");
    if (b.split_parts > t.n_substeps || b.split_parts > 8) return fail("grx_kitchen_step: split_parts <= min(n_substeps, 8): a part runs whole substeps");
  } else b.split_parts = 0;
  const int e = grx_tu_kitchen_launch(m->shape, (b.lane.list ? (unsigned)(b.lane.grid > 0 ? b.lane.grid : GRX_LANE_GRID) : (split ? (unsigned)b.split_parts : 1u) * grx_grid_for(n_worlds)), (size_t)m->words * 4 + m->lds_pad, stream, m->slot, &t, &b, n_worlds, m->words, forward_only);
  if (e) return fail(std::string("grx_kitchen_step launch: ") + hipGetErrorString((hipError_t)e));
  return 0;
}

extern "C" __global__ void __launch_bounds__(256)
grx_order_kernel(const int* __restrict__ cost, float* __restrict__ ema, float alpha, int per, int npow2, int slots, int* __restrict__ order) {
  extern __shared__ unsigned long long keys[];
  const int s = blockIdx.x, base = s * per;
  for (int i = threadIdx.x; i < npow2; i += 256) {
    unsigned k = 0;
    if (i < per) {
      float c = (float)cost[base + i];
      if (ema) { c = (1.0f - alpha) * ema[base + i] + alpha * c; ema[base + i] = c; }
      k = (unsigned)fminf(fmaxf(c * 16.0f, 0.0f), 4.0e9f);
    }
    keys[i] = i < per ? (((unsigned long long)k << 32) | (unsigned)(0x7FFFFFFF - i)) : 0ull;
  }
  __syncthreads();
  for (int k = 2; k <= npow2; k <<= 1)
    for (int j = k >> 1; j > 0; j >>= 1) {
      for (int i = threadIdx.x; i < npow2; i += 256) {
        const int l = i ^ j;
        if (l > i) {
          const unsigned long long a = keys[i], b = keys[l];
          const bool desc = (i & k) == 0;
          if (desc ? (a < b) : (a > b)) { keys[i] = b; keys[l] = a; }
        }
      }
      __syncthreads();
    }
  __shared__ int sM;
  if (threadIdx.x == 0) {
    int M = 0;
    if (slots > 0 && per > slots && per <= 2 * slots) {
      const unsigned long long thr = 2ull * (keys[per - 1] >> 32);
      int K = 0, hi = per;
      while (K < hi) { const int mid = (K + hi) >> 1; if ((keys[mid] >> 32) > thr) K = mid + 1; else hi = mid; }
      M = per - 2 * slots + K;
      if (M < 0 || 3 * M > per - slots || M > slots / 4) M = 0;
    }
    sM = M;
  }
  __syncthreads();
  const int M = sM;
  for (int pos = threadIdx.x; pos < per; pos += 256) {
    int i = pos;
    if (M > 0) {
      if (pos < slots - M) i = pos;
      else if (pos < slots) i = per - M + (pos - (slots - M));
      else if (pos < slots + M) i = per - 2 * M + (pos - slots);
      else if (pos < per - M) i = pos - 2 * M;
      else i = per - 3 * M + (pos - (per - M));
    }
    order[pos * 8 + s] = base + (0x7FFFFFFF - (int)(unsigned)(keys[i] & 0xFFFFFFFFull));
  }
}

extern "C" int grx_order_by_cost_slots(const int* cost, float* ema, float alpha, int n_worlds, int slots_per_xcd, int* order, void* stream);
extern "C" int grx_order_by_cost(const int* cost, float* ema, float alpha, int n_worlds, int* order, void* stream) { return grx_order_by_cost_slots(cost, ema, alpha, n_worlds, 0, order, stream); }
extern "C" int grx_order_by_cost_slots(const int* cost, float* ema, float alpha, int n_worlds, int slots_per_xcd, int* order, void* stream) {
  if (!cost || !order) return fail("grx_order_by_cost: null argument");
  if (ema && !(alpha > 0.0f && alpha <= 1.0f)) return fail("grx_order_by_cost: alpha must be in (0, 1]");
  if (n_worlds <= 0 || (n_worlds & 7)) return fail("grx_order_by_cost: the number of worlds must be a positive multiple of 8 (one contiguous slice per XCD)");
  const int per = n_worlds >> 3;
  int npow2 = 1;
  while (npow2 < per) npow2 <<= 1;
  if ((size_t)npow2 * 8 > 64 * 1024) return fail("grx_order_by_cost: more than 65536 worlds per launch are not supported");
  hipLaunchKernelGGL(grx_order_kernel, dim3(8), dim3(256), (size_t)npow2 * 8, (hipStream_t)stream, cost, ema, alpha, per, npow2, slots_per_xcd < 0 ? 0 : slots_per_xcd, order);
  HIP_OK(hipGetLastError());
  return 0;
}

extern "C" int grx_goal_compute_reward(const float* achieved, const float* desired, int64_t batch, int dim, double distance_threshold, int sparse,
                                       float* reward_out, void* stream) {
  if (!achieved || !desired || !reward_out || dim <= 0) return fail("grx_goal_compute_reward: bad argument");
  if (batch <= 0) return 0;
  long long blocks = (batch + 255) / 256;
  if (blocks > 2048) blocks = 2048;
  hipLaunchKernelGGL(grx_goal_reward_kernel, dim3((unsigned)blocks), dim3(256), 0, (hipStream_t)stream, achieved, desired, (long long)batch, dim,
                     distance_threshold, sparse, reward_out);
  HIP_OK(hipGetLastError());
  return 0;
}
// ... 38 lines not shown
  hipLaunchKernelGGL(grx_her_relabel_kernel, dim3((unsigned)blocks), dim3(256), 0, (hipStream_t)stream, a, (long long)batch);
  HIP_OK(hipGetLastError());
  return 0;
}

static __device__ __forceinline__ unsigned long long grx_splitmix(unsigned long long& s) {
  unsigned long long z = (s += 0x9E3779B97F4A7C15ull);
  z = (z ^ (z >> 30)) * 0xBF58476D1CE4E5B9ull; z = (z ^ (z >> 27)) * 0x94D049BB133111EBull;
  return z ^ (z >> 31);
}
static __device__ __forceinline__ bool grx_her_draw(const int* __restrict__ start, const int* __restrict__ prev_start, const int* __restrict__ term_t, int N, int t_now, int T,
                                                    int k_future, unsigned long long seed, unsigned long long call, long long b, int* t_out, int* w_out, int* tg_out) {
  const int lo_min = t_now - T > 0 ? t_now - T : 0;
#define GRX_HER_LO(W_) ((term_t && term_t[W_] == t_now) ? (prev_start[W_] > lo_min ? prev_start[W_] : lo_min) : (start[W_] > lo_min ? start[W_] : lo_min))
  unsigned long long s = seed * 0xD1342543DE82EF95ull + call * 0x2545F4914F6CDD1Dull + (unsigned long long)b;
  (void)grx_splitmix(s);
  int w = 0, lo = t_now;
  for (int attempt = 0; attempt < 64 && lo >= t_now; attempt++) {
    w = (int)(((grx_splitmix(s) >> 32) * (unsigned long long)N) >> 32);
    lo = GRX_HER_LO(w);
  }
  for (int probe = 0; probe < N && lo >= t_now; probe++) { w = w + 1 < N ? w + 1 : 0; lo = GRX_HER_LO(w); }
#undef GRX_HER_LO
  const unsigned long long r = grx_splitmix(s), r2 = grx_splitmix(s);
  const float u0 = (float)(r >> 40) * (1.0f / 16777216.0f), u1 = (float)((r >> 16) & 0xFFFFFF) * (1.0f / 16777216.0f), u2 = (float)(r2 >> 40) * (1.0f / 16777216.0f);
  int t = lo + (int)(u0 * (float)(t_now - lo));
  if (t > t_now - 1) t = t_now - 1;
  int fut = t + 1 + (int)(u1 * (float)(t_now - t));
  if (fut > t_now) fut = t_now;
  *t_out = t; *w_out = w;
  *tg_out = (u2 >= (float)k_future / ((float)k_future + 1.0f)) ? -1 : fut;
  return lo < t_now;
}
extern "C" __global__ void __launch_bounds__(256)
grx_her_sample_kernel(const int* __restrict__ start, const int* __restrict__ prev_start, const int* __restrict__ term_t, int N, int t_now, int T, int k_future,
                      unsigned long long seed, unsigned long long call, long long B, int* __restrict__ t_idx, int* __restrict__ w_idx, int* __restrict__ t_goal) {
  for (long long b = (long long)blockIdx.x * blockDim.x + threadIdx.x; b < B; b += (long long)gridDim.x * blockDim.x) {
    int t, w, tg;
    (void)grx_her_draw(start, prev_start, term_t, N, t_now, T, k_future, seed, call, b, &t, &w, &tg);
    t_idx[b] = t; w_idx[b] = w; t_goal[b] = tg;
  }
}
extern "C" __global__ void __launch_bounds__(256)
grx_her_sample_valid_kernel(const int* __restrict__ start, const int* __restrict__ prev_start, const int* __restrict__ term_t, int N, int t_now, int T, int k_future,
                            unsigned long long seed, unsigned long long call, long long B, int* __restrict__ t_idx, int* __restrict__ w_idx, int* __restrict__ t_goal,
                            int* __restrict__ valid) {
  for (long long b = (long long)blockIdx.x * blockDim.x + threadIdx.x; b < B; b += (long long)gridDim.x * blockDim.x) {
    int t, w, tg;
    const bool found = grx_her_draw(start, prev_start, term_t, N, t_now, T, k_future, seed, call, b, &t, &w, &tg);
    t_idx[b] = t; w_idx[b] = w; t_goal[b] = tg;
    if (b == 0) *valid = found ? (int)B : 0;
  }
}
extern "C" int grx_her_sample_final(const int* episode_start, const int* prev_start, const int* term_t, int n_worlds, int t_now, int T, int k_future, uint64_t seed,
                                    uint64_t call, int64_t batch, int* t_idx, int* w_idx, int* t_goal, void* stream) {
  if (!episode_start || !t_idx || !w_idx || !t_goal) return fail("grx_her_sample: null argument");
  if ((prev_start == nullptr) != (term_t == nullptr)) return fail("grx_her_sample_final: prev_start and term_t go together");
  if (n_worlds <= 0 || T <= 0 || t_now <= 0 || k_future < 0) return fail("grx_her_sample: n_worlds, T and t_now must be positive, k_future >= 0");
  if (batch <= 0) return 0;
  long long blocks = (batch + 255) / 256;
  if (blocks > 4096) blocks = 4096;
  hipLaunchKernelGGL(grx_her_sample_kernel, dim3((unsigned)blocks), dim3(256), 0, (hipStream_t)stream, episode_start, prev_start, term_t, n_worlds, t_now, T, k_future,
                     (unsigned long long)seed, (unsigned long long)call, (long long)batch, t_idx, w_idx, t_goal);
  HIP_OK(hipGetLastError());
  return 0;
}
extern "C" int grx_her_sample(const int* episode_start, int n_worlds, int t_now, int T, int k_future, uint64_t seed, uint64_t call, int64_t batch,
                              int* t_idx, int* w_idx, int* t_goal, void* stream) {
  return grx_her_sample_final(episode_start, nullptr, nullptr, n_worlds, t_now, T, k_future, seed, call, batch, t_idx, w_idx, t_goal, stream);
}
extern "C" int grx_her_sample_relabel(const grx_her_args* args, const int* episode_start, const int* prev_start, int t_now, int k_future, uint64_t seed, uint64_t call,
                                      int64_t batch, int* scratch, int* valid, void* stream) {
  if (!args || !episode_start || !scratch || !valid) return fail("grx_her_sample_relabel: null argument");
  GrxHerArgs a; memcpy(&a, args, sizeof(a));
  if (!a.rows || !a.acts || !a.out) return fail("grx_her_sample_relabel: null buffer");
  if ((a.term_rows == nullptr) != (a.term_t == nullptr) || (prev_start == nullptr) != (a.term_t == nullptr))
    return fail("grx_her_sample_relabel: term_rows, term_t and prev_start go together");
  if (a.T <= 0 || a.N <= 0 || a.obs_dim <= 0 || a.goal_dim <= 0 || a.goal_dim > 16 || a.act_dim <= 0 || a.W < a.obs_dim + 2 * a.goal_dim)
    return fail("grx_her_sample_relabel: dimensions out of range (goal_dim <= 16, W >= obs_dim + 2 goal_dim)");
  if (a.kind < 0 || a.kind > 3 || (a.kind == 0 && a.goal_dim != 3) || (a.kind == 2 && a.goal_dim != 2) || (a.kind == 3 && a.goal_dim != 7))
    return fail("grx_her_sample_relabel: reward kind does not fit goal_dim");
  if (t_now < 0 || k_future < 0 || batch <= 0 || batch > (1ll << 30)) return fail("grx_her_sample_relabel: t_now, k_future >= 0 and 1 <= batch <= 2^30");
  a.t_idx = scratch; a.w_idx = scratch + batch; a.t_goal = scratch + 2 * batch;
  long long blocks = (batch + 255) / 256;
  if (blocks > 4096) blocks = 4096;
  hipLaunchKernelGGL(grx_her_sample_valid_kernel, dim3((unsigned)blocks), dim3(256), 0, (hipStream_t)stream, episode_start, prev_start, a.term_t, a.N, t_now, a.T, k_future,
                     (unsigned long long)seed, (unsigned long long)call, (long long)batch, scratch, scratch + batch, scratch + 2 * batch, valid);
  HIP_OK(hipGetLastError());
  const long long words = (long long)batch * (2 * a.obs_dim + 3 * a.goal_dim + a.act_dim + 2);
  blocks = (words + 255) / 256;
  if (blocks > 4096) blocks = 4096;
  hipLaunchKernelGGL(grx_her_relabel_valid_kernel, dim3((unsigned)blocks), dim3(256), 0, (hipStream_t)stream, a, (long long)batch, (const int*)valid);
  HIP_OK(hipGetLastError());
  return 0;
}
extern "C" __global__ void __launch_bounds__(256)
grx_her_mark_kernel(const unsigned char* __restrict__ mask, int N, int t, int* __restrict__ start, int* __restrict__ prev_start, int* __restrict__ term_t) {
  const int w = blockIdx.x * blockDim.x + threadIdx.x;
  if (w >= N || !mask[w]) return;
  if (prev_start) { prev_start[w] = start[w]; term_t[w] = t; }
  start[w] = t;
}
extern "C" int grx_her_mark_resets(const unsigned char* reset_mask, int n_worlds, int t, int* episode_start, int* prev_start, int* term_t, void* stream) {
  if (!reset_mask || !episode_start || n_worlds <= 0) return fail("grx_her_mark_resets: null argument");
  if ((prev_start == nullptr) != (term_t == nullptr)) return fail("grx_her_mark_resets: prev_start and term_t go together");
  hipLaunchKernelGGL(grx_her_mark_kernel, dim3((unsigned)((n_worlds + 255) / 256)), dim3(256), 0, (hipStream_t)stream, reset_mask, n_worlds, t, episode_start, prev_start, term_t);
  HIP_OK(hipGetLastError());
  return 0;
}

__device__ __forceinline__ void grx_maze_reset_row(const grx_maze_reset_args& a, int k, int l, float* desired) {
  const int w = a.idx[k];
  const float sx = a.stage[4 * k], sy = a.stage[4 * k + 1], gx = a.stage[4 * k + 2], gy = a.stage[4 * k + 3];
  const int nobs_q = a.nq - a.obs_skip;
  float* row = a.packed ? a.packed + (size_t)w * (a.obs_dim + 6) : nullptr;
  for (int i = l; i < a.nq; i += 64) a.qpos[(size_t)w * a.nq + i] = i == 0 ? sx : (i == 1 ? sy : a.qpos0[i]);
  for (int i = l; i < a.nv; i += 64) { a.qvel[(size_t)w * a.nv + i] = 0.0f; a.qacc_ws[(size_t)w * a.nv + i] = 0.0f; }
  for (int i = l; i < a.obs_dim; i += 64) {
    const int q = i + a.obs_skip;
    const float v = i < nobs_q ? (q == 0 ? sx : (q == 1 ? sy : a.qpos0[q])) : 0.0f;
    a.obs[(size_t)w * a.obs_dim + i] = v;
    if (row) row[i] = v;
  }
  if (l == 0) {
    a.goal[2 * (size_t)w] = gx; a.goal[2 * (size_t)w + 1] = gy;
    a.achieved[2 * (size_t)w] = sx; a.achieved[2 * (size_t)w + 1] = sy;
    const float sg[2] = {sx, sy}, gg[2] = {gx, gy};
    const int succ = grx_goal_distance2(sg, gg) <= a.goal_radius;
    a.success[w] = (unsigned char)succ;
    if (row) {
      row[a.obs_dim] = sx; row[a.obs_dim + 1] = sy; row[a.obs_dim + 2] = gx; row[a.obs_dim + 3] = gy;
      if (!a.keep_outcome) { row[a.obs_dim + 4] = 0.0f; row[a.obs_dim + 5] = succ ? 1.0f : 0.0f; }
    }
    if (!a.keep_outcome) a.reward[w] = 0.0f;
    if (desired) { desired[2 * (size_t)w] = gx; desired[2 * (size_t)w + 1] = gy; }
  }
}
extern "C" __global__ void __launch_bounds__(64)
grx_maze_reset_kernel(grx_maze_reset_args a, int n_reset) {
  if ((int)blockIdx.x < n_reset) grx_maze_reset_row(a, (int)blockIdx.x, threadIdx.x, nullptr);
}
__global__ void __launch_bounds__(64)
grx_maze_reset_list_kernel(grx_maze_reset_args a, const int* __restrict__ count, int max_n, float* desired) {
  const int n = *count < max_n ? *count : max_n;
  for (int k = blockIdx.x; k < n; k += gridDim.x) grx_maze_reset_row(a, k, threadIdx.x, desired);
}
extern "C" int grx_maze_reset_rows(const grx_maze_reset_args* args, int n_reset, void* stream) {
  if (!args) return fail("grx_maze_reset_rows: null argument");
  const grx_maze_reset_args& a = *args;
  if (!a.idx || !a.stage || !a.qpos0 || !a.qpos || !a.qvel || !a.qacc_ws || !a.goal || !a.obs || !a.achieved || !a.reward || !a.success) return fail("grx_maze_reset_rows: null buffer");
  if (a.nq < 2 || a.nv <= 0 || a.obs_skip < 0 || a.obs_skip > 2 || a.obs_dim != a.nq + a.nv - a.obs_skip) return fail("grx_maze_reset_rows: obs_dim must be nq + nv - obs_skip");
  if (n_reset <= 0) return 0;
  hipLaunchKernelGGL(grx_maze_reset_kernel, dim3((unsigned)n_reset), dim3(64), 0, (hipStream_t)stream, a, n_reset);
  HIP_OK(hipGetLastError());
  return 0;
}

extern "C" __global__ void __launch_bounds__(64)
grx_hand_commit_kernel(grx_hand_commit_args a) {
  const int j = blockIdx.x, l = threadIdx.x;
  if (j >= a.k) return;
  const size_t w = (size_t)a.idx[j], s = (size_t)j;
  const int od = a.obs_dim, gd = a.goal_dim, pw = od + 2 * gd + 2;
  for (int i = l; i < a.nq; i += 64) a.qpos[w * a.nq + i] = a.s_qpos[s * a.nq + i];
  for (int i = l; i < a.nv; i += 64) { a.qvel[w * a.nv + i] = a.s_qvel[s * a.nv + i]; a.qacc_ws[w * a.nv + i] = a.s_qacc_ws[s * a.nv + i]; }
  for (int i = l; i < od; i += 64) { const float v = a.s_obs[s * od + i]; a.obs[w * od + i] = v; }
  for (int i = l; i < gd; i += 64) { a.achieved[w * gd + i] = a.s_achieved[s * gd + i]; a.goal[w * gd + i] = a.s_goal[s * gd + i]; }
  if (l < 3) a.palm[w * 3 + l] = a.s_palm[s * 3 + l];
  for (int i = l; i < od + gd; i += 64) a.packed[w * pw + i] = a.s_packed[s * pw + i];
  for (int i = l; i < gd; i += 64) a.packed[w * pw + od + gd + i] = a.s_goal[s * gd + i];
  if (l == 0) a.status[w] |= a.s_status[s] & (int)0xFFFF0000;
}
extern "C" int grx_hand_commit_rows(const grx_hand_commit_args* args, void* stream) {
  if (!args) return fail("grx_hand_commit_rows: null argument");
  const grx_hand_commit_args& a = *args;
  if (!a.idx || !a.s_qpos || !a.s_qvel || !a.s_qacc_ws || !a.s_obs || !a.s_achieved || !a.s_palm || !a.s_goal || !a.s_packed || !a.s_status || !a.qpos || !a.qvel ||
      !a.qacc_ws || !a.obs || !a.achieved || !a.palm || !a.goal || !a.packed || !a.status) return fail("grx_hand_commit_rows: null buffer");
  if (a.nq <= 0 || a.nv <= 0 || a.obs_dim <= 0 || a.goal_dim <= 0) return fail("grx_hand_commit_rows: bad dimensions");
  if (a.k <= 0) return 0;
  hipLaunchKernelGGL(grx_hand_commit_kernel, dim3((unsigned)a.k), dim3(64), 0, (hipStream_t)stream, a);
  HIP_OK(hipGetLastError());
  return 0;
}

extern "C" __global__ void __launch_bounds__(64)
grx_fetch_commit_kernel(grx_fetch_commit_args a) {
  const int j = blockIdx.x, l = threadIdx.x;
  if (j >= a.k) return;
  const size_t w = (size_t)a.idx[j];
  const int od = a.obs_dim, pw = od + 8;
  for (int i = l; i < a.nq; i += 64) a.qpos[w * a.nq + i] = a.s_qpos[w * a.nq + i];
  for (int i = l; i < a.nv; i += 64) { a.qvel[w * a.nv + i] = a.s_qvel[w * a.nv + i]; a.qacc_ws[w * a.nv + i] = a.s_qacc_ws[w * a.nv + i]; }
  for (int i = l; i < a.mocap_words; i += 64) a.mocap[w * a.mocap_words + i] = a.s_mocap[w * a.mocap_words + i];
  if (l < 8) a.aux[w * 8 + l] = a.s_aux[w * 8 + l];
  if (l < 3) { a.goal[w * 3 + l] = a.s_goal[w * 3 + l]; a.achieved[w * 3 + l] = a.s_achieved[w * 3 + l]; }
  for (int i = l; i < od; i += 64) a.obs[w * od + i] = a.s_obs[w * od + i];
  for (int i = l; i < pw; i += 64) {
    const float old = a.packed[w * pw + i];
    if (a.final_packed) a.final_packed[w * pw + i] = old;
    a.packed[w * pw + i] = i < od ? a.s_obs[w * od + i] : (i < od + 3 ? a.s_achieved[w * 3 + i - od] : (i < od + 6 ? a.s_goal[w * 3 + i - od - 3] : old));
  }
  if (l == 0) a.status[w] = grx_status_word(a.status[w], a.s_status[w]);
}
extern "C" int grx_fetch_commit_rows(const grx_fetch_commit_args* args, void* stream) {
  if (!args) return fail("grx_fetch_commit_rows: null argument");
  const grx_fetch_commit_args& a = *args;
  if (!a.idx || !a.s_qpos || !a.s_qvel || !a.s_qacc_ws || !a.s_aux || !a.s_goal || !a.s_obs || !a.s_achieved || !a.s_status || !a.qpos || !a.qvel || !a.qacc_ws || !a.aux ||
      !a.goal || !a.obs || !a.achieved || !a.packed || !a.status || (a.mocap_words > 0 && (!a.s_mocap || !a.mocap))) return fail("grx_fetch_commit_rows: null buffer");
  if (a.nq <= 0 || a.nv <= 0 || a.obs_dim <= 0 || a.mocap_words < 0) return fail("grx_fetch_commit_rows: bad dimensions");
  if (a.k <= 0) return 0;
  hipLaunchKernelGGL(grx_fetch_commit_kernel, dim3((unsigned)a.k), dim3(64), 0, (hipStream_t)stream, a);
  HIP_OK(hipGetLastError());
  return 0;
}

extern "C" __global__ void __launch_bounds__(64)
grx_adroit_commit_kernel(grx_adroit_commit_args a) {
  const int j = blockIdx.x, l = threadIdx.x;
  if (j >= a.k) return;
  const size_t w = (size_t)a.idx[j];
  for (int i = l; i < a.nq; i += 64) a.qpos[w * a.nq + i] = a.s_qpos[w * a.nq + i];
  for (int i = l; i < a.nv; i += 64) { a.qvel[w * a.nv + i] = a.s_qvel[w * a.nv + i]; a.qacc_ws[w * a.nv + i] = a.s_qacc_ws[w * a.nv + i]; }
  for (int i = l; i < a.obs_dim; i += 64) a.obs[w * a.obs_dim + i] = a.s_obs[w * a.obs_dim + i];
  if (a.shift && l < 7) a.shift[w * 7 + l] = a.s_shift[w * 7 + l];
  if (a.target && l < 3) a.target[w * 3 + l] = a.s_target[w * 3 + l];
  if (l == 0) a.status[w] = grx_status_word(a.status[w], a.s_status[w]);
}
extern "C" int grx_adroit_commit_rows(const grx_adroit_commit_args* args, void* stream) {
  if (!args) return fail("grx_adroit_commit_rows: null argument");
  const grx_adroit_commit_args& a = *args;
  if (!a.idx || !a.s_qpos || !a.s_qvel || !a.s_qacc_ws || !a.s_obs || !a.s_status || !a.qpos || !a.qvel || !a.qacc_ws || !a.obs || !a.status) return fail("grx_adroit_commit_rows: null buffer");
  if ((a.shift != nullptr) != (a.s_shift != nullptr) || (a.target != nullptr) != (a.s_target != nullptr)) return fail("grx_adroit_commit_rows: shift / target need both the staged and the live buffer");
  if (a.nq <= 0 || a.nv <= 0 || a.obs_dim <= 0) return fail("grx_adroit_commit_rows: bad dimensions");
  if (a.k <= 0) return 0;
  hipLaunchKernelGGL(grx_adroit_commit_kernel, dim3((unsigned)a.k), dim3(64), 0, (hipStream_t)stream, a);
  HIP_OK(hipGetLastError());
  return 0;
}

extern "C" int grx_debug_primitive(int mode, int nv, int nefc, const float* A, const float* b, const float* J, const float* D, float* out, void* stream) {
  int bytes = (2 * nv * nv + GRX_MAXEFC * nv + 6 * GRX_MAXEFC + 2 * nv + 64) * 4;
  hipLaunchKernelGGL(grx_debug_kernel, dim3(1), dim3(64), bytes, (hipStream_t)stream, mode, nv, nefc, A, b, J, D, out);
  HIP_OK(hipGetLastError());
  return 0;
}

typedef unsigned __int128 grx_u128;
static inline uint64_t grx_pcg64_next(uint64_t* st ) {
  const grx_u128 mult = ((grx_u128)0x2360ED051FC65DA4ULL << 64) | 0x4385DF649FCCF645ULL;
  grx_u128 state = ((grx_u128)st[0] << 64) | st[1], inc = ((grx_u128)st[2] << 64) | st[3];
  state = state * mult + inc;
  st[0] = (uint64_t)(state >> 64); st[1] = (uint64_t)state;
  uint64_t hi = st[0], lo = st[1], x = hi ^ lo; unsigned rot = (unsigned)(hi >> 58);
  return (x >> rot) | (x << ((64 - rot) & 63));
}
static inline double grx_pcg64_uniform(uint64_t* st, double lo, double hi) {
  return lo + (hi - lo) * ((double)(grx_pcg64_next(st) >> 11) * (1.0 / 9007199254740992.0));
}

extern "C" int grx_fetch_sample_resets(uint64_t* states, const int64_t* idx, int n, int has_object, int target_in_the_air, double obj_range,
                                       double target_range, const double* target_offset, const double* gripper_xpos, double height_offset,
                                       double* out_oxy, double* out_goal) {
  if (!states || !idx || !out_goal || !gripper_xpos || !target_offset) return fail("grx_fetch_sample_resets: null argument");
  for (int k = 0; k < n; k++) {
// ... 388 lines not shown
```

gymnasium_robotics_amd/envs/fetch.py:

```python
import ctypes
import os
from typing import Optional

import numpy as np
import torch

from .. import _native
from ..core import create_rerun_model, GoalVecEnv, OverflowLane, np_random
from ..mjcf import CompiledModel, compile_mjcf, load_model
from ..spaces import Box, Dict, batch_space
from .fetch_spec import DISTANCE_THRESHOLD, FETCH_TASKS, MAX_EPISODE_STEPS, N_SUBSTEPS, make_fetch_task, parse_env_id

_MODELS_DIR = os.path.join(os.path.dirname(os.path.abspath(__file__)), "..", "models")


FETCH_CAPACITY = {"maxcon": 28, "maxefc": 144, "jpool": 2032, "split_spans": False}
FETCH_FAST_CAPACITY = {"maxcon": 24, "maxefc": 96, "jpool": 1024}
FETCH_SPLIT_PARTS = 4
FETCH_SPLIT_WIDE = 12288
HANDOFF_TASKS = ("FetchPickAndPlace",)


def load_fetch_model(task: str, assets_root: Optional[str] = None) -> CompiledModel:
    xml = FETCH_TASKS[task]["xml"]
# ... 58 lines not shown
        self._L = _native.lib()
        H, I, F = self.model.pack()
        dev_index = self.device.index or 0
        self._h = _native.acquire_model(H, I, F, dev_index)
        self.lds_bytes = self._L.grx_model_lds_bytes(self._h)
        self._h_big = create_rerun_model(self._L, self.model, dev_index, overflow_rerun)
        self._h_fast, self._fast_model = None, None
        if task in HANDOFF_TASKS and self._h_big is not None and self.num_envs >= 64 and os.environ.get("GRX_FETCH_HANDOFF", "0") == "1" and os.environ.get("GRX_FETCH_CAP") is None:
            self._fast_model = self.model.with_capacity(**FETCH_FAST_CAPACITY)
            Hf, If, Ff = self._fast_model.pack()
            self._h_fast = _native.acquire_model(Hf, If, Ff, dev_index)
            self.lds_bytes = self._L.grx_model_lds_bytes(self._h_fast)
        self._alloc(self.num_envs)
        self._env_setup()
        self.single_action_space = Box(-1.0, 1.0, (4,), np.float32)
        self.single_observation_space = Dict(dict(
            desired_goal=Box(-np.inf, np.inf, (3,), np.float64), achieved_goal=Box(-np.inf, np.inf, (3,), np.float64),
            observation=Box(-np.inf, np.inf, (self.obs_dim,), np.float64)))
        self.action_space = batch_space(self.single_action_space, self.num_envs)
        self.observation_space = batch_space(self.single_observation_space, self.num_envs)
        self._check_goal_space()
        self._seed_worlds([None] * self.num_envs)
        self._elapsed = np.zeros(self.num_envs, np.int64)
        self._needs_reset = np.zeros(self.num_envs, bool)
        self._has_reset = False
        self.kernel_events = None
        self.step_events = None

    def _launch_step(self, bufs):
        def fast(b):
            ev = self.kernel_events
            if ev is not None:
                e0, e1 = torch.cuda.Event(enable_timing=True), torch.cuda.Event(enable_timing=True)
                e0.record()
            _native.check(self._L.grx_fetch_step(self._h_fast or self._h, ctypes.byref(self.task), ctypes.byref(b), self.num_envs, self._stream()))
            if ev is not None:
                e1.record()
                ev.append((e0, e1))

        if self.lane is None:
            fast(bufs)
        else:
            large = lambda b: _native.check(self._L.grx_fetch_step(self._h_big, ctypes.byref(self.task), ctypes.byref(b), self.num_envs, self._stream()))
            middle = (lambda b: _native.check(self._L.grx_fetch_step(self._h, ctypes.byref(self.task), ctypes.byref(b), self.num_envs, self._stream()))) if self._h_fast else None
            timed = self.kernel_events is not None and self.step_events is not None
            if timed:
                l0, l1 = torch.cuda.Event(enable_timing=True), torch.cuda.Event(enable_timing=True)
                l0.record()
            self.lane.step(self.mask if bufs is self._bufs_masked else None, fast, large, fast_bufs=bufs, launch_lane=middle)
            if timed:
                l1.record()
                self.step_events.append((l0, l1))
        if self.balance:
            self._rebalance()

    def _alloc(self, n):
        d, f32 = self.device, torch.float32
        z = lambda *s, dtype=f32: torch.zeros(*s, dtype=dtype, device=d)
        self.qpos, self.qvel, self.qacc_ws = z(n, self.nq), z(n, self.nv), z(n, self.nv)
        self.mocap, self.aux, self.goal, self.action = z(n, 7 * self.nmocap), z(n, 8), z(n, 3), z(n, 4)
        self.obs, self.achieved, self.reward = z(n, self.obs_dim), z(n, 3), z(n)
        self.success, self.status = z(n, dtype=torch.uint8), z(n, dtype=torch.int32)
        self.mask = torch.ones(n, dtype=torch.uint8, device=d)
        self.balance = bool(self.balance) and n % 8 == 0 and 1024 <= n <= 65536 * 8
        self._reset_stage = z(n, 6)
        self.packed = z(n, self.obs_dim + 8)
        self.final_packed = z(n, self.obs_dim + 8)
        self.cost = torch.zeros(n, dtype=torch.int32, device=d) if self.balance else None
        self.cost_ema = torch.zeros(n, dtype=torch.float32, device=d) if self.balance else None
        self.balance_alpha = float(os.environ.get("GRX_BALANCE_ALPHA", 0.1))
        self.order = None
        self._slots_per_xcd = 32 * min(12 if self._h_fast else 8, (160 * 1024) // (-(-self.lds_bytes // 1280) * 1280)) if (self.balance and os.environ.get("GRX_TAIL_ORDER", "1") != "0") else 0
        if self.balance:
            per = n // 8
            self._slice_base = (torch.arange(8, device=d, dtype=torch.int32) * per).unsqueeze(1)
            self.order = (self._slice_base + torch.arange(per, device=d, dtype=torch.int32).unsqueeze(0)).t().contiguous().view(-1)
        self.hullcache = z(n, 90) if os.environ.get("GRX_NO_HULLCACHE") is None else None
        common = (self.qpos, self.qvel, self.qacc_ws, self.mocap, self.aux, self.goal, self.action, self.obs, self.achieved, self.reward, self.success, self.status)
        self.handoff, self._handoff_stride = None, 0
        if getattr(self, "_h_fast", None):
            self._handoff_stride = -(-(2 + self.model.dim("nu") + 7 * self.nmocap + self.nq + 2 * self.nv) // 16) * 16
            self.handoff = z(n, self._handoff_stride)
        self._bufs = self._make_bufs(*common, None, self.order, self.cost, self.packed, self.hullcache, self.handoff)
        self._bufs_masked = self._make_bufs(*common, self.mask, self.order, self.cost, self.packed, self.hullcache, self.handoff)
        self._bufs.handoff_stride = self._bufs_masked.handoff_stride = self._handoff_stride
        self._split = max(1, int(os.environ.get("GRX_FETCH_SPLIT", str((FETCH_SPLIT_PARTS if n <= FETCH_SPLIT_WIDE else 2) if n > 2048 else 1)))) if self.handoff is None and n >= 64 else 1
        if self._split > 1:
            stride = -(-(2 + self.model.dim("nu") + 7 * self.nmocap + self.nq + 2 * self.nv) // 16) * 16
            self._split_rows, self._split_state = z(n, stride), z(n, 2, dtype=torch.int32)
            for b in (self._bufs, self._bufs_masked):
                b.handoff, b.handoff_stride, b.split_state, b.split_parts = self._split_rows.data_ptr(), stride, self._split_state.data_ptr(), self._split
        self.lane = None
        if self._h_big is not None:
            packed, hullcache, handoff, stride, mk = self.packed, self.hullcache, self.handoff, self._handoff_stride, FetchVecEnv._make_bufs

            def lane_bufs(m):
                b = mk(*common, m, None, None, packed, hullcache, handoff)
                b.handoff_stride = stride
                return b

            if handoff is not None:
                self.lane = OverflowLane(n, d, self._fast_model, lane_bufs, mode="lane", handoff=True, poll_grid=int(os.environ.get("GRX_FETCH_POLL", max(64, n // 32))),
                                         ttl=int(os.environ.get("GRX_FETCH_TTL", 4)), margin=0.9)
            else:
                self.lane = OverflowLane(n, d, self.model, lane_bufs, mode="entry")
        self._ahead = None
        if n > 1 and os.environ.get("GRX_FETCH_AHEAD_RESET", "1") != "0":
            sq, sv, sa, sm, sx, sg, so, sh = z(n, self.nq), z(n, self.nv), z(n, self.nv), z(n, 7 * self.nmocap), z(n, 8), z(n, 3), z(n, self.obs_dim), z(n, 3)
            sr, ss, st = z(n), z(n, dtype=torch.uint8), z(n, dtype=torch.int32)
            self._ahead = dict(qpos=sq, qvel=sv, qacc_ws=sa, mocap=sm, aux=sx, goal=sg, obs=so, achieved=sh, reward=sr, success=ss, status=st)
            self._ahead_bufs = self._make_bufs(sq, sv, sa, sm, sx, sg, self.action, so, sh, sr, ss, st, None, None, None, None, None)
            self._ahead_stream = torch.cuda.Stream(device=d)
            self._ahead_late = os.environ.get("GRX_FETCH_AHEAD_ORDER", "after") == "after"

    def _rebalance(self):
        _native.check(self._L.grx_order_by_cost_slots(self.cost.data_ptr(), self.cost_ema.data_ptr(), self.balance_alpha, self.num_envs, self._slots_per_xcd, self.order.data_ptr(), self._stream()))

    @staticmethod
# ... 41 lines not shown
        mask = (1 << 64) - 1
        for i, sd in enumerate(seeds):
            s = np_random(sd)[0].bit_generator.state["state"]
            st[i] = [s["state"] >> 64, s["state"] & mask, s["inc"] >> 64, s["inc"] & mask]
        self._rng_dev = torch.from_numpy(st.view(np.int64)).to(self.device)

    @property
    def _rng_state(self):
        return self._rng_dev.cpu().numpy().view(np.uint64)

    @_rng_state.setter
    def _rng_state(self, value):
        value = np.ascontiguousarray(value, dtype=np.uint64).reshape(self.num_envs, 4)
        self._rng_dev.copy_(torch.from_numpy(value.view(np.int64)).to(self.device))

    def _stage_reset(self, idx: np.ndarray):
        n = len(idx)
        cfg = self.cfg
        stage = torch.empty(n, dtype=torch.int32, pin_memory=True)
        stage.numpy()[:] = np.ascontiguousarray(idx, dtype=np.int32)
        dev = self._reset_stage.view(-1)[: 6 * n]
        idx_dev, samples = dev[:n].view(torch.int32), dev[n:]
        idx_dev.copy_(stage, non_blocking=True)
        toff = np.ascontiguousarray(np.broadcast_to(np.asarray(cfg["target_offset"], dtype=np.float64), (3,)))
        g0 = np.ascontiguousarray(self.initial_gripper_xpos, dtype=np.float64)
        _native.check(self._L.grx_fetch_sample_resets_device(
            self._rng_dev.data_ptr(), idx_dev.data_ptr(), n, int(cfg["has_object"]), int(cfg["target_in_the_air"]), float(cfg["obj_range"]), float(cfg["target_range"]),
            toff.ctypes.data, g0.ctypes.data, float(self.height_offset), samples.data_ptr(), self._stream()))
        return n, idx_dev, samples

    def _launch_reset(self, staged, idx, keep_outcome=False):
        n, idx_dev, samples = staged
        args = _native.FetchResetArgsStruct(idx_dev.data_ptr(), samples.data_ptr(), self.initial_qpos.data_ptr(), self.initial_qvel.data_ptr(),
                                            self._mocap0.data_ptr(), int(self._obj_qadr), int(keep_outcome), self.final_packed.data_ptr() if keep_outcome else None)
        _native.check(self._L.grx_fetch_reset(self._h, ctypes.byref(self.task), ctypes.byref(self._bufs), ctypes.byref(args), n, self._stream()))
        self._elapsed[idx] = 0
        self._needs_reset[idx] = False

    def _launch_reset_ahead(self, idx: np.ndarray, after=None):
        if after is None:
            self._ahead_stream.wait_stream(torch.cuda.current_stream(self.device))
        else:
            self._ahead_stream.wait_event(after)
        with torch.cuda.stream(self._ahead_stream):
            staged = self._stage_reset(idx)
            n, idx_dev, samples = staged
            args = _native.FetchResetArgsStruct(idx_dev.data_ptr(), samples.data_ptr(), self.initial_qpos.data_ptr(), self.initial_qvel.data_ptr(),
                                                self._mocap0.data_ptr(), int(self._obj_qadr), 1, None)
            _native.check(self._L.grx_fetch_reset(self._h, ctypes.byref(self.task), ctypes.byref(self._ahead_bufs), ctypes.byref(args), n, self._stream()))
            done = torch.cuda.Event()
            done.record(self._ahead_stream)
        return staged, done

    def _commit_ahead(self, ahead, idx):
        (n, idx_dev, _), done = ahead
        torch.cuda.current_stream(self.device).wait_event(done)
        A = self._ahead
        a = _native.FetchCommitArgsStruct(idx_dev.data_ptr(), n, self.nq, self.nv, 7 * self.nmocap, self.obs_dim,
                                          A["qpos"].data_ptr(), A["qvel"].data_ptr(), A["qacc_ws"].data_ptr(), A["mocap"].data_ptr(), A["aux"].data_ptr(), A["goal"].data_ptr(),
                                          A["obs"].data_ptr(), A["achieved"].data_ptr(), A["status"].data_ptr(),
                                          self.qpos.data_ptr(), self.qvel.data_ptr(), self.qacc_ws.data_ptr(), self.mocap.data_ptr(), self.aux.data_ptr(), self.goal.data_ptr(),
                                          self.obs.data_ptr(), self.achieved.data_ptr(), self.packed.data_ptr(), self.final_packed.data_ptr(), self.status.data_ptr())
        _native.check(self._L.grx_fetch_commit_rows(ctypes.byref(a), self._stream()))
        self._elapsed[idx] = 0
        self._needs_reset[idx] = False

    def _reset_worlds(self, idx: np.ndarray):
        if len(idx) == 0:
            return None
        staged = self._stage_reset(idx)
        self._launch_reset(staged, idx)
        return staged[1].long()

    def reset(self, *, seed=None, options=None):
        if seed is not None:
            seeds = [seed + self.seed_offset + i for i in range(self.num_envs)] if np.isscalar(seed) else list(seed)
            self._seed_worlds(seeds)
        with torch.cuda.device(self.device):
            self._reset_worlds(np.arange(self.num_envs))
        self._has_reset = True
        return self._obs_dict(), {}

    def step(self, actions):
        if not self._has_reset:
            raise RuntimeError("Cannot call env.step() before calling env.reset()")
        if isinstance(actions, torch.Tensor):
            if tuple(actions.shape) != (self.num_envs, 4):
                raise ValueError("Action dimension mismatch")
            self.action.copy_(actions.to(torch.float32), non_blocking=True)
        else:
            a = np.asarray(actions, dtype=np.float32)
            if a.shape != (self.num_envs, 4):
                raise ValueError("Action dimension mismatch")
            self.action.copy_(torch.from_numpy(a), non_blocking=True)
        with torch.cuda.device(self.device):
            pending = np.nonzero(self._needs_reset)[0] if self.autoreset_mode == "next_step" else np.zeros(0, np.int64)
            ahead, will, before = None, np.zeros(0, np.int64), None
            if self._ahead is not None and self.autoreset_mode == "same_step" and self.max_episode_steps is not None:
                will = np.nonzero(self._elapsed + 1 >= self.max_episode_steps)[0]
                if len(will) and self._ahead_late:
                    before = torch.cuda.Event()
                    before.record(torch.cuda.current_stream(self.device))
                elif len(will):
                    ahead = (will, self._launch_reset_ahead(will))
            if len(pending):
                self.mask.fill_(1)
                self.mask.index_fill_(0, self._stage_idx(pending), 0)
                self._launch_step(self._bufs_masked)
            else:
                self._launch_step(self._bufs)
            if before is not None:
                ahead = (will, self._launch_reset_ahead(will, after=before))
            stepped = ~self._needs_reset if len(pending) else np.ones(self.num_envs, bool)
            self._elapsed[stepped] += 1
            truncated = np.zeros(self.num_envs, bool)
            if self.max_episode_steps is not None:
                truncated = stepped & (self._elapsed >= self.max_episode_steps)
            terminated = np.zeros(self.num_envs, bool)
            info = {}
            if len(pending):
                tp = self._reset_worlds(pending)
                self.reward.index_fill_(0, tp, 0.0)
                self.packed[:, -2].index_fill_(0, tp, 0.0)
            if self.autoreset_mode == "same_step" and truncated.any():
                done = np.nonzero(truncated)[0]
                if ahead is not None:
                    if not np.array_equal(ahead[0], done):
                        raise RuntimeError("overlapped reset: the worlds reset ahead of the step are not the ones it truncated")
                    staged = ahead[1][0]
                    if self.output != "torch":
                        info["final_obs"] = self._obs_dict(rows=done)
                    self._commit_ahead(ahead[1], done)
                else:
                    staged = self._stage_reset(done)
                    if self.output != "torch":
                        info["final_obs"] = self._obs_dict(rows=done)
                    self._launch_reset(staged, done, keep_outcome=True)
                if self.output == "torch":
                    fo = self.final_packed[staged[1]]
                    info["final_obs"] = {"observation": fo[:, : self.obs_dim], "achieved_goal": fo[:, self.obs_dim: self.obs_dim + 3],
                                         "desired_goal": fo[:, self.obs_dim + 3: self.obs_dim + 6]}
            elif self.autoreset_mode == "next_step":
                self._needs_reset |= truncated
        obs = self._obs_dict()
        if self.output == "torch":
            info["is_success"] = self.success
            return obs, self.reward, torch.from_numpy(terminated), torch.from_numpy(truncated), self._status_info(info)
        info["is_success"] = self.success.cpu().numpy().astype(np.float32)
        self._status_info(info)
        r = self.reward.cpu().numpy()
        return obs, (r if self.reward_type == "sparse" else r.astype(np.float64)), terminated, truncated, info

    def _obs_dict(self, rows=None, rows_dev=None):
        if self.output == "torch":
            if rows is not None and rows_dev is None:
                rows_dev = torch.from_numpy(rows).to(self.device)
            sel = (lambda t: t) if rows is None else (lambda t: t[rows_dev])
            return {"observation": sel(self.obs), "achieved_goal": sel(self.achieved), "desired_goal": sel(self.goal)}
        sel = (lambda a: a) if rows is None else (lambda a: a[rows])
        return {"observation": sel(self.obs.double().cpu().numpy()), "achieved_goal": sel(self.achieved.double().cpu().numpy()),
                "desired_goal": sel(self.goal.double().cpu().numpy())}

    def compute_reward(self, achieved_goal, desired_goal, info=None):
        as_numpy = not isinstance(achieved_goal, torch.Tensor)
        ag = torch.as_tensor(np.asarray(achieved_goal, dtype=np.float32) if as_numpy else achieved_goal, dtype=torch.float32, device=self.device).contiguous()
        dg = torch.as_tensor(np.asarray(desired_goal, dtype=np.float32) if as_numpy else desired_goal, dtype=torch.float32, device=self.device).contiguous()
        if ag.shape != dg.shape or ag.shape[-1] != 3:
            raise ValueError("achieved_goal and desired_goal must have the same (..., 3) shape")
        out = torch.empty(ag.shape[:-1], dtype=torch.float32, device=self.device)
        with torch.cuda.device(self.device):
            _native.check(self._L.grx_fetch_compute_reward(ag.data_ptr(), dg.data_ptr(), out.numel(), DISTANCE_THRESHOLD,
                                                           int(self.reward_type == "sparse"), out.data_ptr(), self._stream()))
        if not as_numpy:
            return out
        r = out.cpu().numpy()
        return r if self.reward_type == "sparse" else r.astype(np.float64)

    def compute_terminated(self, achieved_goal, desired_goal, info=None):
        return np.zeros(np.asarray(achieved_goal).shape[:-1], bool)

    def compute_truncated(self, achieved_goal, desired_goal, info=None):
        return np.zeros(np.asarray(achieved_goal).shape[:-1], bool)


    def close(self):
        if getattr(self, "_h", None):
            _native.release_model(self._h)
            self._h = None
        if getattr(self, "_h_big", None):
            _native.release_model(self._h_big)
            self._h_big = None
        if getattr(self, "_h_fast", None):
            _native.release_model(self._h_fast)
            self._h_fast = None

    def __del__(self):
# ... 5 lines not shown
```

gymnasium_robotics_amd/her.py:

```python
import ctypes
from typing import Optional

import numpy as np
import torch

from . import _native

FETCH, HAND_REACH, MAZE, MANIPULATE = 0, 1, 2, 3


def reward_spec(env) -> dict:
    name = type(env).__name__
    sparse = int(getattr(env, "reward_type", "sparse") == "sparse")
    if name == "FetchVecEnv":
        return dict(kind=FETCH, p0=float(env.task.distance_threshold), p1=0.0, sparse=sparse)
    if name == "HandReachVecEnv":
        return dict(kind=HAND_REACH, p0=float(env.distance_threshold), p1=0.0, sparse=sparse)
    if name in ("PointMazeVecEnv", "AntMazeVecEnv"):
        return dict(kind=MAZE, p0=0.45, p1=0.0, sparse=sparse)
    if name == "HandBlockVecEnv":
        from .envs.manipulate_spec import ROTATION_THRESHOLD

        return dict(kind=MANIPULATE, p0=float(env.distance_threshold), p1=float(ROTATION_THRESHOLD), sparse=sparse, ignore_pos=int(env.target_position == "ignore"),
                    ignore_rot=int(env.target_rotation == "ignore"), ignore_z=int(env._objcfg["ignore_z_target_rotation"]))
    raise TypeError(f"{name} is not a goal-conditioned environment")


class HerReplay:

    def __init__(self, env, horizon: int, capacity: int, obs_dim: Optional[int] = None, goal_dim: Optional[int] = None, seed: int = 0, continuous: bool = False):
        self.env, self.T, self.N = env, int(horizon), int(env.num_envs)
        self.device = env.device
        self.W = int(env.packed.shape[1])
        self.goal_dim = int(goal_dim if goal_dim is not None else env.single_observation_space["desired_goal"].shape[0])
        self.obs_dim = int(obs_dim if obs_dim is not None else self.W - 2 * self.goal_dim - 2)
        self.act_dim = int(env.single_action_space.shape[0])
        self.OW = 2 * self.obs_dim + 3 * self.goal_dim + self.act_dim + 2
        self.spec = reward_spec(env)
        self.continuous = bool(continuous)
        z = lambda *s, dtype=torch.float32: torch.zeros(*s, dtype=dtype, device=self.device)
        self.R = self.T + 1
        self.episode, self.actions = z(self.R, self.N, self.W), z(self.R, self.N, self.act_dim)
        self.episode_start = z(self.N, dtype=torch.int32)
        self.prev_start, self.term_t = z(self.N, dtype=torch.int32), torch.full((self.N,), -1, dtype=torch.int32, device=self.device)
        self._final_rows = None
        self._just_ended = np.zeros(self.N, bool)
        self._start_host = np.zeros(self.N, np.int64)
        self.rows, self.capacity, self.head, self.size = z(int(capacity), self.OW), int(capacity), 0, 0
        self.t = 0
        self._seed, self._calls = int(seed), 0
        self._L = _native.lib()
        self._mask_pin = [dict(buf=torch.empty(self.N, dtype=torch.bool, pin_memory=True), event=None) for _ in range(4)]
        self._mask_next, self._mask_dev = 0, torch.zeros(self.N, dtype=torch.bool, device=self.device)

    def begin_episode(self, packed_rows: torch.Tensor):
        self.episode[0].copy_(packed_rows)
        self.episode_start.zero_()
        self.prev_start.zero_(); self.term_t.fill_(-1)
        self._start_host[:] = 0
        self._just_ended[:] = False
        self.t = 0

    def append(self, actions: torch.Tensor, packed_rows: torch.Tensor, reset_mask: Optional[torch.Tensor] = None, final_rows: Optional[torch.Tensor] = None):
        if self.t >= self.T and not self.continuous:
            raise RuntimeError("episode buffer is full: call begin_episode()")
        self.t += 1
        r = self.t % self.R
        self.actions[r].copy_(actions)
        self.episode[r].copy_(packed_rows)
        if reset_mask is not None:
            host = reset_mask.cpu().numpy() if isinstance(reset_mask, torch.Tensor) else np.asarray(reset_mask)
            self._start_host[host.astype(bool)] = self.t
            if isinstance(reset_mask, torch.Tensor) and reset_mask.device == self.device:
                dev = reset_mask
            else:
                slot = self._mask_pin[self._mask_next]
                self._mask_next = (self._mask_next + 1) % len(self._mask_pin)
                if slot["event"] is not None:
                    slot["event"].synchronize()
                slot["buf"].numpy()[:] = host.astype(bool)
                dev = self._mask_dev
                dev.copy_(slot["buf"], non_blocking=True)
                slot["event"] = torch.cuda.Event()
                slot["event"].record(torch.cuda.current_stream(self.device))
            if final_rows is not None:
                assert tuple(final_rows.shape) == (self.N, self.W) and final_rows.is_contiguous()
                self._final_rows = final_rows
            track = self._final_rows is not None
            self._just_ended = host.astype(bool) if track else self._just_ended
            _native.check(self._L.grx_her_mark_resets(dev.data_ptr(), self.N, self.t, self.episode_start.data_ptr(), self.prev_start.data_ptr() if track else None,
                                                      self.term_t.data_ptr() if track else None, ctypes.c_void_p(torch.cuda.current_stream(self.device).cuda_stream)))
        elif self._final_rows is not None:
            self._just_ended = np.zeros(self.N, bool)

    def set_episode_start(self, starts):
        self._start_host[:] = np.asarray(starts, dtype=np.int64)
        self.episode_start.copy_(torch.from_numpy(self._start_host.astype(np.int32)).to(self.device))

    def reseed(self, seed: int):
        self._seed, self._calls = int(seed), 0

    def sample_indices(self, batch: int, k_future: int = 4):
        track = self._final_rows is not None
        if not ((np.maximum(self._start_host, max(self.t - self.T, 0)) < self.t) | (self._just_ended if track else False)).any():
            return None
        t, w, tg = (torch.empty(batch, dtype=torch.int32, device=self.device) for _ in range(3))
        _native.check(self._L.grx_her_sample_final(self.episode_start.data_ptr(), self.prev_start.data_ptr() if track else None, self.term_t.data_ptr() if track else None,
                                                   self.N, self.t, self.T, int(k_future), self._seed, self._calls, batch,
                                                   t.data_ptr(), w.data_ptr(), tg.data_ptr(), ctypes.c_void_p(torch.cuda.current_stream(self.device).cuda_stream)))
        self._calls += 1
        return t, w, tg

    def relabel_into(self, out: torch.Tensor, t: torch.Tensor, w: torch.Tensor, t_goal: torch.Tensor):
        a = _native.HerArgsStruct()
        a.rows, a.acts = self.episode.data_ptr(), self.actions.data_ptr()
        a.T, a.N, a.W, a.obs_dim, a.goal_dim, a.act_dim = self.T, self.N, self.W, self.obs_dim, self.goal_dim, self.act_dim
        a.t_idx, a.w_idx, a.t_goal, a.out = t.data_ptr(), w.data_ptr(), t_goal.data_ptr(), out.data_ptr()
        if self._final_rows is not None:
            a.term_rows, a.term_t = self._final_rows.data_ptr(), self.term_t.data_ptr()
        for k, v in self.spec.items():
            setattr(a, k, v)
        assert out.is_contiguous() and tuple(out.shape) == (len(t), self.OW) and t.dtype == w.dtype == t_goal.dtype == torch.int32
        _native.check(self._L.grx_her_relabel(ctypes.byref(a), len(t), ctypes.c_void_p(torch.cuda.current_stream(self.device).cuda_stream)))
        return out

    def relabel(self, batch: int, k_future: int = 4):
        if batch > self.capacity:
            raise ValueError("batch larger than the replay capacity")
        if self.head + batch > self.capacity:
            self.head = 0
        idx = self.sample_indices(batch, k_future)
        if idx is None:
            return self.rows[self.head: self.head]
        t, w, tg = idx
        view = self.rows[self.head: self.head + batch]
        self.relabel_into(view, t, w, tg)
        self.head += batch
        self.size = min(self.capacity, max(self.size, self.head))
        return view

    def split(self, rows: torch.Tensor) -> dict:
        o, g, a = self.obs_dim, self.goal_dim, self.act_dim
        c = np.cumsum([0, o, g, g, a, 1, o, g, 1])
        names = ("observation", "achieved_goal", "desired_goal", "action", "reward", "next_observation", "next_achieved_goal", "success")
        return {n: rows[:, c[i]: c[i + 1]] for i, n in enumerate(names)}
```

include/grx_capi.h:

```cpp
#ifndef GRX_CAPI_H
#define GRX_CAPI_H

#include <stdint.h>

#ifdef __cplusplus
extern "C" {
#endif

typedef struct grx_model grx_model;

typedef struct grx_overflow_lane {
  const unsigned char* skip;
  int* entry_count; int* entry_list;
  const int* list; const int* count;
  unsigned char* next_flags; int* next_count; int* next_list;
  signed char* ttl;
  int soft_maxefc, soft_jpool, soft_maxcon, ttl_init;
  int grid;
  int entry_cap, next_cap;
  int* ready; int* progress; const int* poll_list;
  int ready_cap, progress_total, poll_grid, pad_;
} grx_overflow_lane;

typedef struct grx_fetch_task {
// ... 166 lines not shown
  const float* samples;
  const float *init_qpos, *init_qvel, *init_mocap;
  int obj_qadr;
  int keep_outcome;
  float* final_packed;
} grx_fetch_reset_args;
int grx_fetch_reset(const grx_model* m, const grx_fetch_task* task, const grx_fetch_buffers* buf, const grx_fetch_reset_args* args, int n_reset, void* stream);
int grx_order_by_cost(const int* cost, float* ema , float alpha, int n_worlds, int* order, void* stream);
int grx_order_by_cost_slots(const int* cost, float* ema, float alpha, int n_worlds, int slots_per_xcd, int* order, void* stream);
int grx_fetch_compute_reward(const float* achieved, const float* desired, int64_t batch, double distance_threshold, int sparse,
                             float* reward_out, void* stream);
int grx_point_step(const grx_model* m, const grx_point_task* task, const grx_point_buffers* buf, int n_worlds, void* stream);
int grx_maze_compute_reward(const float* achieved, const float* desired, int64_t batch, double goal_radius, int sparse, float* reward_out,
                            void* stream);

int grx_hand_step(const grx_model* m, const grx_hand_task* task, const grx_hand_buffers* buf, int n_worlds, int forward_only, void* stream);
int grx_hand_step_repeat(const grx_model* m, const grx_hand_task* task, const grx_hand_buffers* buf, int n_worlds, int repeat, void* stream);
int grx_adroit_step(const grx_model* m, const grx_adroit_task* task, const grx_adroit_buffers* buf, int n_worlds, int forward_only, void* stream);
int grx_kitchen_step(const grx_model* m, const grx_kitchen_task* task, const grx_kitchen_buffers* buf, int n_worlds, int forward_only, void* stream);
int grx_sample_uniform_rows(uint64_t* states, const int64_t* idx, int n, int count, float* out);
int grx_uniform_rows_device(uint64_t* states, const unsigned char* mask, int n, int count, float* out, void* stream);
typedef struct grx_kitchen_book {
  const int* completed; const unsigned char* stepped;
  int *tasks_to_complete, *episode_completions, *elapsed, *step_completions;
  float* reward; unsigned char *terminated, *truncated, *needs_reset, *reset_now;
  float *qpos, *qvel, *qacc_ws; const float* init_qpos;
  int nq, nv, all_mask, max_steps, remove_when_completed, terminate_when_completed, mode;
  int* final_info;
} grx_kitchen_book;
int grx_kitchen_bookkeeping(const grx_kitchen_book* args, int n_worlds, void* stream);
int grx_goal_compute_reward(const float* achieved, const float* desired, int64_t batch, int dim, double distance_threshold, int sparse,
                            float* reward_out, void* stream);
int grx_manip_compute_reward(const float* achieved, const float* desired, int64_t batch, int ignore_position, int ignore_rotation,
                             int ignore_z, float distance_threshold, float rotation_threshold, int sparse, float* reward_out, void* stream);

typedef struct grx_her_args {
  const float* rows; const float* acts;
  int T, N, W, obs_dim, goal_dim, act_dim;
  const int *t_idx, *w_idx, *t_goal;
  int kind;
  double p0, p1;
  int sparse, ignore_pos, ignore_rot, ignore_z;
  float* out;
  const float* term_rows; const int* term_t;
} grx_her_args;
int grx_her_relabel(const grx_her_args* args, int64_t batch, void* stream);
int grx_her_sample(const int* episode_start, int n_worlds, int t_now, int T, int k_future, uint64_t seed, uint64_t call, int64_t batch,
                   int* t_idx, int* w_idx, int* t_goal, void* stream);
int grx_her_sample_final(const int* episode_start, const int* prev_start, const int* term_t, int n_worlds, int t_now, int T, int k_future, uint64_t seed, uint64_t call,
                         int64_t batch, int* t_idx, int* w_idx, int* t_goal, void* stream);
int grx_her_mark_resets(const unsigned char* reset_mask, int n_worlds, int t, int* episode_start, int* prev_start, int* term_t, void* stream);
int grx_her_sample_relabel(const grx_her_args* args, const int* episode_start, const int* prev_start, int t_now, int k_future, uint64_t seed, uint64_t call, int64_t batch,
                           int* scratch, int* valid, void* stream);

typedef struct grx_maze_reset_args {
  const int* idx; const float* stage; const float* qpos0;
  int nq, nv, obs_dim, obs_skip;
  double goal_radius;
  int keep_outcome;
  float *qpos, *qvel, *qacc_ws, *goal, *obs, *achieved, *reward; unsigned char* success; float* packed;
} grx_maze_reset_args;
int grx_maze_reset_rows(const grx_maze_reset_args* args, int n_reset, void* stream);
int grx_maze_reset_rows_list(const grx_maze_reset_args* args, const int* count, int max_n, float* desired, void* stream);

typedef struct grx_maze_episode_args {
  long long* elapsed;
  unsigned char* needs_reset;
  const unsigned char* success;
  const float* achieved;
  float* goal;
  int* status;
  const float* packed;
  uint64_t* rng;
  const double* goal_xy;
  int n_goal, mode, limit, continuing_task, reset_target, packed_dim;
  double noise_range, scaling, goal_radius;
  unsigned char *terminated, *truncated;
  unsigned char* mask;
  unsigned char* step_success;
  float* desired;
  int *reset_count, *reset_idx;
  int *n_final, *final_idx;
  float* final_rows;
} grx_maze_episode_args;
int grx_maze_episode_end(const grx_maze_episode_args* args, int n_worlds, void* stream);

typedef struct grx_hand_commit_args {
  const int64_t* idx; int k;
  int nq, nv, obs_dim, goal_dim;
  const float *s_qpos, *s_qvel, *s_qacc_ws, *s_obs, *s_achieved, *s_palm, *s_goal, *s_packed; const int* s_status;
  float *qpos, *qvel, *qacc_ws, *obs, *achieved, *palm, *goal, *packed; int* status;
} grx_hand_commit_args;
int grx_hand_commit_rows(const grx_hand_commit_args* args, void* stream);

typedef struct grx_fetch_commit_args {
  const int* idx; int k;
  int nq, nv, mocap_words, obs_dim;
  const float *s_qpos, *s_qvel, *s_qacc_ws, *s_mocap, *s_aux, *s_goal, *s_obs, *s_achieved; const int* s_status;
  float *qpos, *qvel, *qacc_ws, *mocap, *aux, *goal, *obs, *achieved, *packed, *final_packed; int* status;
} grx_fetch_commit_args;
int grx_fetch_commit_rows(const grx_fetch_commit_args* args, void* stream);

typedef struct grx_adroit_commit_args {
  const int64_t* idx; int k;
  int nq, nv, obs_dim;
  const float *s_qpos, *s_qvel, *s_qacc_ws, *s_shift, *s_target, *s_obs; const int* s_status;
  float *qpos, *qvel, *qacc_ws, *shift, *target, *obs; int* status;
} grx_adroit_commit_args;
int grx_adroit_commit_rows(const grx_adroit_commit_args* args, void* stream);

int grx_fetch_sample_resets(uint64_t* states, const int64_t* idx, int n, int has_object, int target_in_the_air, double obj_range,
                            double target_range, const double* target_offset, const double* gripper_xpos, double height_offset,
                            double* out_oxy, double* out_goal);
int grx_fetch_sample_resets_device(uint64_t* states, const int* idx, int n, int has_object, int target_in_the_air, double obj_range, double target_range,
                                   const double* target_offset, const double* gripper_xpos, double height_offset, float* samples, void* stream);
int grx_adroit_sample_resets_device(uint64_t* states, const int64_t* idx, int n, int kind, const double* shift_pos0, double* edit, double* target64, float* shift, float* target,
                                    void* stream);
int grx_maze_sample_resets_device(uint64_t* states, const int* idx, int n, const double* goal_xy, int n_goal, const double* reset_xy, int n_reset, double noise_range, double scaling,
                                  const double* fixed_goal_xy, const double* fixed_reset_xy, float* stage, void* stream);
int grx_maze_sample_resets_list(uint64_t* states, const int* idx, const int* count, int max_n, const double* goal_xy, int n_goal, const double* reset_xy, int n_reset,
                                double noise_range, double scaling, float* stage, void* stream);
const char* grx_last_error(void);

#ifdef __cplusplus
}
#endif
#endif
```

Baseline: 1.427 million.

## Fuse fetch post-step ordering/commit/gather and HER append/sample-relabel kernels

Adds a fused grx_fetch_post_step that combines cost-based world ordering, commit of rows reset ahead, and the final-row gather into one launch in same-step mode. It also moves replay append into a shared grx_her_append kernel that accepts a device mask, and adds a fused draw+relabel path for HER sampling that drops the index scratch buffers. The aim is fewer kernel launches and less host overhead per step. The cost is more complex control flow, including an environment toggle and an error path that must still run the ordering.

```diff
diff --git a/__graft_entry__.py b/__graft_entry__.py
--- a/__graft_entry__.py
+++ b/__graft_entry__.py
@@ -12,7 +12,8 @@
 HIP_SO = os.path.join(ROOT, "gymnasium_robotics_amd", "_lib", "libgrx_hip.so")
 ENV_SRC = os.path.join(ROOT, "gymnasium_robotics_amd", "csrc", "grx_env.hip")
 ENV_DEPS = [os.path.join(ROOT, "include", "grx_env.h"), os.path.join(ROOT, "include", "grx_replay.h"), os.path.join(ROOT, "include", "grx_capi.h"),
-            os.path.join(ROOT, "gymnasium_robotics_amd", "csrc", "grx_env_maze.inc"), os.path.join(ROOT, "gymnasium_robotics_amd", "csrc", "grx_env_replay.inc")]
+            os.path.join(ROOT, "gymnasium_robotics_amd", "csrc", "grx_env_maze.inc"), os.path.join(ROOT, "gymnasium_robotics_amd", "csrc", "grx_env_replay.inc"),
+            os.path.join(ROOT, "gymnasium_robotics_amd", "csrc", "grx_copy.h")]
 ENV_SO = os.path.join(ROOT, "gymnasium_robotics_amd", "_lib", "libgrx_env.so")
 
 
diff --git a/gymnasium_robotics_amd/_native.py b/gymnasium_robotics_amd/_native.py
--- a/gymnasium_robotics_amd/_native.py
+++ b/gymnasium_robotics_amd/_native.py
@@ -64,6 +64,12 @@
     _fields_ = [("rows", ctypes.c_void_p), ("acts", ctypes.c_void_p)] + [(n, ctypes.c_int) for n in ("T", "N", "W", "obs_dim", "goal_dim", "act_dim")] + [
         (n, ctypes.c_void_p) for n in ("t_idx", "w_idx", "t_goal")] + [("kind", ctypes.c_int), ("p0", ctypes.c_double), ("p1", ctypes.c_double)] + [
         (n, ctypes.c_int) for n in ("sparse", "ignore_pos", "ignore_rot", "ignore_z")] + [("out", ctypes.c_void_p), ("term_rows", ctypes.c_void_p), ("term_t", ctypes.c_void_p)]
+
+
+class HerAppendArgsStruct(ctypes.Structure):
+    _fields_ = [(n, ctypes.c_void_p) for n in ("packed", "action", "row_dst", "act_dst")] + [("n_row", ctypes.c_longlong), ("n_act", ctypes.c_longlong)] + [
+        (n, ctypes.c_void_p) for n in ("list", "count_dev", "mask")] + [(n, ctypes.c_int) for n in ("count", "n_worlds", "t", "W")] + [
+        (n, ctypes.c_void_p) for n in ("start", "prev_start", "term_t", "final_rows", "term_rows")]
 
 
 class MazeResetArgsStruct(ctypes.Structure):
@@ -121,6 +127,9 @@
         L.grx_her_sample_final.argtypes = [vp, vp, vp, ci, ci, ci, ci, ctypes.c_uint64, ctypes.c_uint64, ctypes.c_int64, vp, vp, vp, vp]
         L.grx_her_mark_resets.argtypes = [vp, ci, ci, vp, vp, vp, vp]
         L.grx_her_sample_relabel.argtypes = [vp, vp, vp, ci, ci, ctypes.c_uint64, ctypes.c_uint64, ctypes.c_int64, vp, vp, vp]
+        L.grx_her_draw_relabel.argtypes = [vp, vp, vp, ci, ci, ctypes.c_uint64, ctypes.c_uint64, ctypes.c_int64, vp, vp]
+        L.grx_her_append.argtypes = [vp, vp]
+        L.grx_fetch_post_step.argtypes = [vp, vp, ctypes.c_float, ci, ci, vp, vp, vp, vp]
         L.grx_kitchen_step.argtypes = [vp, vp, vp, ci, ci, vp]
         L.grx_sample_uniform_rows.argtypes = [vp, vp, ci, ci, vp]
         L.grx_uniform_rows_device.argtypes = [vp, vp, ci, ci, vp, vp]
@@ -174,7 +183,7 @@
 
 EXPORTED_SYMBOLS = [
     "grx_model_create", "grx_model_destroy", "grx_model_set_table", "grx_model_lds_bytes", "grx_model_dim",
-    "grx_fetch_step", "grx_fetch_forward", "grx_fetch_reset", "grx_fetch_compute_reward", "grx_her_relabel", "grx_her_sample", "grx_her_sample_final", "grx_her_mark_resets", "grx_her_sample_relabel", "grx_fetch_sample_resets", "grx_fetch_sample_resets_device", "grx_adroit_sample_resets_device", "grx_maze_sample_resets_device", "grx_point_step", "grx_maze_compute_reward", "grx_hand_step", "grx_hand_step_repeat", "grx_adroit_step", "grx_kitchen_step", "grx_sample_uniform_rows", "grx_uniform_rows_device", "grx_kitchen_bookkeeping", "grx_goal_compute_reward", "grx_manip_compute_reward", "grx_order_by_cost", "grx_order_by_cost_slots", "grx_maze_reset_rows", "grx_maze_reset_rows_list", "grx_maze_sample_resets_list", "grx_maze_episode_end", "grx_hand_commit_rows", "grx_fetch_commit_rows", "grx_adroit_commit_rows", "grx_last_error",
+    "grx_fetch_step", "grx_fetch_forward", "grx_fetch_reset", "grx_fetch_compute_reward", "grx_her_relabel", "grx_her_sample", "grx_her_sample_final", "grx_her_mark_resets", "grx_her_sample_relabel", "grx_her_draw_relabel", "grx_her_append", "grx_fetch_post_step", "grx_fetch_sample_resets", "grx_fetch_sample_resets_device", "grx_adroit_sample_resets_device", "grx_maze_sample_resets_device", "grx_point_step", "grx_maze_compute_reward", "grx_hand_step", "grx_hand_step_repeat", "grx_adroit_step", "grx_kitchen_step", "grx_sample_uniform_rows", "grx_uniform_rows_device", "grx_kitchen_bookkeeping", "grx_goal_compute_reward", "grx_manip_compute_reward", "grx_order_by_cost", "grx_order_by_cost_slots", "grx_maze_reset_rows", "grx_maze_reset_rows_list", "grx_maze_sample_resets_list", "grx_maze_episode_end", "grx_hand_commit_rows", "grx_fetch_commit_rows", "grx_adroit_commit_rows", "grx_last_error",
 ]
 
 
diff --git a/gymnasium_robotics_amd/csrc/grx_copy.h b/gymnasium_robotics_amd/csrc/grx_copy.h
--- /dev/null
+++ b/gymnasium_robotics_amd/csrc/grx_copy.h
@@ -0,0 +1,15 @@
+#pragma once
+#include <hip/hip_runtime.h>
+#include <cstdint>
+
+static __device__ __forceinline__ void grx_copy_words(float* __restrict__ dst, const float* __restrict__ src, long long n, long long tid, long long nth) {
+  if ((((uintptr_t)dst | (uintptr_t)src) & 15) == 0) {
+    const long long n4 = n >> 2;
+    const float4* __restrict__ s4 = (const float4*)src;
+    float4* __restrict__ d4 = (float4*)dst;
+    for (long long i = tid; i < n4; i += nth) d4[i] = s4[i];
+    for (long long i = (n4 << 2) + tid; i < n; i += nth) dst[i] = src[i];
+  } else {
+    for (long long i = tid; i < n; i += nth) dst[i] = src[i];
+  }
+}
diff --git a/gymnasium_robotics_amd/csrc/grx_env.hip b/gymnasium_robotics_amd/csrc/grx_env.hip
--- a/gymnasium_robotics_amd/csrc/grx_env.hip
+++ b/gymnasium_robotics_amd/csrc/grx_env.hip
@@ -3,6 +3,7 @@
 #include <sys/random.h>
 
 #include <cstdio>
+#include <cstdlib>
 #include <cstring>
 #include <map>
 #include <string>
@@ -11,6 +12,7 @@
 #include "grx_capi.h"
 #include "grx_env.h"
 #include "grx_replay.h"
+#include "grx_copy.h"
 
 namespace {
 
@@ -236,6 +238,7 @@
   int* a_status;
   grx_fetch_buffers bufs{}, bufs_masked{}, lane_plain{}, lane_masked{}, ahead_bufs{};
   bool balance = false, ahead = false;
+  bool fused_tail = true;
   int slots_per_xcd = 0, split = 1;
   hipStream_t side = nullptr;
   hipEvent_t ev_before = nullptr, ev_ahead = nullptr;
@@ -312,7 +315,7 @@
   return b;
 }
 
-int launch_step(grx_env* e, bool masked, hipStream_t s) {
+int launch_step(grx_env* e, bool masked, bool order_now, hipStream_t s) {
   grx_fetch_buffers& fb = masked ? e->bufs_masked : e->bufs;
   ENV_HIP(hipMemsetAsync(e->lane_head, 0, e->lane_head_bytes, s));
   int* counts = e->lane_head + (e->lane_head_bytes / 4 - 2);
@@ -327,7 +330,7 @@
   b.lane.next_flags = (unsigned char*)e->lane_head; b.lane.next_count = counts; b.lane.next_list = e->lane_next_list; b.lane.ttl = e->lane_ttl; b.lane.next_cap = 0;
   b.lane.soft_maxefc = e->soft[0]; b.lane.soft_jpool = e->soft[1]; b.lane.soft_maxcon = e->soft[2]; b.lane.ttl_init = e->soft[3];
   ENV_GRX(grx_fetch_step(e->hbig, &e->d.task, &b, e->n, s));
-  if (e->balance) ENV_GRX(grx_order_by_cost_slots(e->cost, e->cost_ema, kBalanceAlpha, e->n, e->slots_per_xcd, e->order, s));
+  if (e->balance && order_now) ENV_GRX(grx_order_by_cost_slots(e->cost, e->cost_ema, kBalanceAlpha, e->n, e->slots_per_xcd, e->order, s));
   return 0;
 }
 
@@ -404,6 +407,7 @@
   e->lane_head_bytes = (size_t)((n + 3) / 4 + 2) * 4;
   ENV_TRY(e->zalloc(&e->lane_head, e->lane_head_bytes / 4)); ENV_TRY(e->zalloc(&e->lane_next_list, n)); ENV_TRY(e->zalloc(&e->lane_entry_list, n)); ENV_TRY(e->zalloc(&e->lane_ttl, n));
   e->balance = n % 8 == 0 && n >= 1024 && n <= 65536 * 8;
+  { const char* v = std::getenv("GRX_FETCH_FUSED_TAIL"); e->fused_tail = !(v && v[0] == '0' && v[1] == 0); }
   if (e->balance) {
     ENV_TRY(e->zalloc(&e->cost, n)); ENV_TRY(e->zalloc(&e->cost_ema, n)); ENV_TRY(e->zalloc(&e->order, n));
     const int lds = grx_model_lds_bytes(e->h);
@@ -664,7 +668,9 @@
     hipLaunchKernelGGL(grx_env_mask_kernel, dim3(blocks(kp)), dim3(64), 0, s, e->mask, (const int*)e->idx_main, kp);
     ENV_HIP(hipGetLastError());
   }
-  ENV_TRY(launch_step(e, kp > 0, s));
+  const bool post = e->fused_tail && e->mode == GRX_ENV_SAME_STEP && kp == 0;
+  bool ordered = !(post && e->balance);
+  ENV_TRY(launch_step(e, kp > 0, !post, s));
   if (kw) {
     ENV_HIP(hipStreamWaitEvent(e->side, e->ev_before, 0));
     ENV_TRY(e->upload(e->idx_ahead, will.data(), (size_t)kw * 4, e->side));
@@ -694,11 +700,14 @@
     ENV_HIP(hipGetLastError());
   }
   const int kd = (int)e->final_idx.size();
+  bool gathered = false;
   if (e->mode == GRX_ENV_SAME_STEP && kd) {
     const int* idx_dev;
     if (kw) {
-      if (kw != kd || !std::equal(will.begin(), will.end(), e->final_idx.begin()))
+      if (kw != kd || !std::equal(will.begin(), will.end(), e->final_idx.begin())) {
+        if (!ordered) (void)grx_fetch_post_step(e->cost, e->cost_ema, kBalanceAlpha, e->n, e->slots_per_xcd, e->order, nullptr, nullptr, s);
         return fail(GRX_ENV_EINVAL, "grx_env_step: the worlds reset ahead of the step are not the ones it truncated");
+      }
       ENV_HIP(hipStreamWaitEvent(s, e->ev_ahead, 0));
       grx_fetch_commit_args c;
       std::memset(&c, 0, sizeof c);
@@ -707,7 +716,10 @@
       c.s_achieved = e->a_achieved; c.s_status = e->a_status;
       c.qpos = e->qpos; c.qvel = e->qvel; c.qacc_ws = e->qacc_ws; c.mocap = e->mocap; c.aux = e->aux; c.goal = e->goal; c.obs = e->obs; c.achieved = e->achieved;
       c.packed = e->packed; c.final_packed = e->final_packed; c.status = e->status;
-      ENV_GRX(grx_fetch_commit_rows(&c, s));
+      if (post) {
+        ENV_GRX(grx_fetch_post_step(e->cost, e->cost_ema, kBalanceAlpha, e->n, e->slots_per_xcd, e->balance ? e->order : nullptr, &c, e->final_rows, s));
+        ordered = gathered = true;
+      } else ENV_GRX(grx_fetch_commit_rows(&c, s));
       idx_dev = e->idx_ahead;
     } else {
       ENV_TRY(e->upload(e->idx_main, e->final_idx.data(), (size_t)kd * 4, s));
@@ -716,8 +728,10 @@
       idx_dev = e->idx_main;
     }
     mark_reset(e, e->final_idx);
-    hipLaunchKernelGGL(grx_env_gather_kernel, dim3(blocks(kd)), dim3(64), 0, s, e->final_rows, (const float*)e->final_packed, e->pdim, idx_dev, kd);
-    ENV_HIP(hipGetLastError());
+    if (!gathered) {
+      hipLaunchKernelGGL(grx_env_gather_kernel, dim3(blocks(kd)), dim3(64), 0, s, e->final_rows, (const float*)e->final_packed, e->pdim, idx_dev, kd);
+      ENV_HIP(hipGetLastError());
+    }
     e->n_final = kd;
     e->step_list = idx_dev; e->step_count = kd;
   } else {
@@ -725,6 +739,7 @@
       for (int w : e->final_idx) e->needs_reset[w] = 1;
     e->final_idx.clear();
   }
+  if (!ordered) ENV_GRX(grx_fetch_post_step(e->cost, e->cost_ema, kBalanceAlpha, e->n, e->slots_per_xcd, e->order, nullptr, nullptr, s));
   return 0;
 }
 
diff --git a/gymnasium_robotics_amd/csrc/grx_env_replay.inc b/gymnasium_robotics_amd/csrc/grx_env_replay.inc
--- a/gymnasium_robotics_amd/csrc/grx_env_replay.inc
+++ b/gymnasium_robotics_amd/csrc/grx_env_replay.inc
@@ -6,7 +6,7 @@
   uint64_t seed = 0, calls = 0;
   bool track = false;
   float *episode = nullptr, *actions = nullptr, *rows = nullptr, *term_rows = nullptr;
-  int *start = nullptr, *prev_start = nullptr, *term_t = nullptr, *scratch = nullptr, *valid = nullptr;
+  int *start = nullptr, *prev_start = nullptr, *term_t = nullptr, *valid = nullptr;
   std::vector<void*> allocs;
   int t = 0;
   bool begun = false;
@@ -16,55 +16,10 @@
 
 namespace {
 
-struct ReplayAppend {
-  const float *packed, *action;
-  float *row_dst, *act_dst;
-  long long n_row, n_act;
-  const int* list;
-  const int* count_dev;
-  int count, max_n, t;
-  int *start, *prev_start, *term_t;
-  const float* final_rows;
-  float* term_rows;
-  int W;
-};
-
-__device__ __forceinline__ void replay_copy(float* __restrict__ dst, const float* __restrict__ src, long long n, long long tid, long long nth) {
-  if ((((uintptr_t)dst | (uintptr_t)src) & 15) == 0) {
-    const long long n4 = n >> 2;
-    const float4* __restrict__ s4 = (const float4*)src;
-    float4* __restrict__ d4 = (float4*)dst;
-    for (long long i = tid; i < n4; i += nth) d4[i] = s4[i];
-    for (long long i = (n4 << 2) + tid; i < n; i += nth) dst[i] = src[i];
-  } else {
-    for (long long i = tid; i < n; i += nth) dst[i] = src[i];
-  }
-}
-
-__global__ void __launch_bounds__(256) grx_replay_append_kernel(ReplayAppend a) {
-  const long long tid = (long long)blockIdx.x * blockDim.x + threadIdx.x, nth = (long long)gridDim.x * blockDim.x;
-  replay_copy(a.row_dst, a.packed, a.n_row, tid, nth);
-  replay_copy(a.act_dst, a.action, a.n_act, tid, nth);
-  int k = a.count_dev ? *a.count_dev : a.count;
-  k = k < 0 ? 0 : (k > a.max_n ? a.max_n : k);
-  for (long long j = tid; j < k; j += nth) {
-    const int w = a.list[j];
-    if ((unsigned)w >= (unsigned)a.max_n) continue;
-    if (a.prev_start) { a.prev_start[w] = a.start[w]; a.term_t[w] = a.t; }
-    a.start[w] = a.t;
-  }
-  if (a.term_rows)
-    for (long long i = tid; i < (long long)k * a.W; i += nth) {
-      const long long j = i / a.W;
-      const int w = a.list[j];
-      if ((unsigned)w < (unsigned)a.max_n) a.term_rows[(size_t)w * a.W + (i - j * a.W)] = a.final_rows[i];
-    }
-}
-
 __global__ void __launch_bounds__(256) grx_replay_begin_kernel(const float* __restrict__ packed, float* __restrict__ row0, long long n_row, const long long* __restrict__ elapsed, int n,
                                                                int* __restrict__ start, int* __restrict__ prev_start, int* __restrict__ term_t) {
   const long long tid = (long long)blockIdx.x * blockDim.x + threadIdx.x, nth = (long long)gridDim.x * blockDim.x;
-  replay_copy(row0, packed, n_row, tid, nth);
+  grx_copy_words(row0, packed, n_row, tid, nth);
   for (long long w = tid; w < n; w += nth) {
     if (elapsed) start[w] = -(int)elapsed[w];
     prev_start[w] = 0;
@@ -121,7 +76,7 @@
     ENV_TRY(replay_zalloc(r, &r->actions, (size_t)r->R * n * r->ad));
     ENV_TRY(replay_zalloc(r, &r->rows, (size_t)r->capacity * r->OW));
     ENV_TRY(replay_zalloc(r, &r->start, n)); ENV_TRY(replay_zalloc(r, &r->prev_start, n)); ENV_TRY(replay_zalloc(r, &r->term_t, n));
-    ENV_TRY(replay_zalloc(r, &r->scratch, (size_t)3 * r->max_batch)); ENV_TRY(replay_zalloc(r, &r->valid, 1));
+    ENV_TRY(replay_zalloc(r, &r->valid, 1));
     ENV_HIP(hipMemset(r->term_t, 0xFF, n * 4));
     if (r->track) {
       if (e->mz) ENV_TRY(replay_zalloc(r, &r->term_rows, n * r->W));
@@ -194,20 +149,19 @@
   if (r->t == INT32_MAX - 1) return fail(GRX_ENV_EINVAL, "grx_replay_append: row counter exhausted: call grx_replay_begin");
   DeviceGuard g(e->device);
   const int t = r->t + 1, row = t % r->R;
-  ReplayAppend a;
+  grx_her_append_args a;
   std::memset(&a, 0, sizeof a);
   a.packed = replay_packed(e); a.action = replay_action(e);
   a.n_row = (long long)r->n * r->W; a.n_act = (long long)r->n * r->ad;
   a.row_dst = r->episode + (size_t)row * a.n_row; a.act_dst = r->actions + (size_t)row * a.n_act;
-  a.list = e->step_list; a.count_dev = e->step_count_dev; a.count = e->step_list ? e->step_count : 0; a.max_n = r->n; a.t = t;
+  a.list = e->step_list; a.count_dev = e->step_list ? e->step_count_dev : nullptr; a.count = e->step_list ? e->step_count : 0; a.n_worlds = r->n; a.t = t;
   a.start = r->start;
   if (r->track) {
     a.prev_start = r->prev_start; a.term_t = r->term_t;
-    if (e->mz) { a.final_rows = e->mz->final_rows; a.term_rows = r->term_rows; }
+    if (e->mz && a.list) { a.final_rows = e->mz->final_rows; a.term_rows = r->term_rows; }
   }
   a.W = r->W;
-  hipLaunchKernelGGL(grx_replay_append_kernel, dim3(replay_blocks(a.n_row)), dim3(256), 0, (hipStream_t)stream, a);
-  ENV_HIP(hipGetLastError());
+  ENV_GRX(grx_her_append(&a, stream));
   r->t = t;
   r->last_step = e->steps;
   return 0;
@@ -223,7 +177,8 @@
   if (r->head + batch > r->capacity) r->head = 0;
   grx_her_args a = r->ha;
   a.out = r->rows + (size_t)r->head * r->OW;
-  ENV_GRX(grx_her_sample_relabel(&a, r->start, r->track ? r->prev_start : nullptr, r->t, k_future, r->seed, r->calls, batch, r->scratch, r->valid, stream));
+  ENV_GRX(grx_her_sample_relabel(&a, r->start, r->track ? r->prev_start : nullptr, r->t, k_future, r->seed, r->calls, batch,
+                                  r->valid, r->valid, stream));
   r->calls += 1;
   if (out) { out->rows = a.out; out->batch = batch; out->offset = r->head; out->valid = r->valid; }
   r->head += batch;
diff --git a/gymnasium_robotics_amd/csrc/grx_kernels.hip b/gymnasium_robotics_amd/csrc/grx_kernels.hip
--- a/gymnasium_robotics_amd/csrc/grx_kernels.hip
+++ b/gymnasium_robotics_amd/csrc/grx_kernels.hip
@@ -23,6 +23,7 @@
 #include "grx_adroit_task.h"
 #include "grx_kitchen_task.h"
 #include "grx_host_model.h"
+#include "grx_copy.h"
 
 static_assert(sizeof(grx_fetch_task) == sizeof(GrxFetchTask), "grx_fetch_task must mirror GrxFetchTask");
 static_assert(sizeof(grx_fetch_buffers) == sizeof(GrxFetchBuffers), "grx_fetch_buffers must mirror GrxFetchBuffers");
@@ -1132,12 +1133,12 @@
     *reward = grx_fetch_reward(d, a.p0, a.sparse); *success = (d < a.p0) ? 1.0f : 0.0f;
   }
 }
-GRX_DEV float grx_her_word(const GrxHerArgs& a, long long b, int e) {
+GRX_DEV float grx_her_word_at(const GrxHerArgs& a, int ti, int w, int tg, int e) {
   const int od = a.obs_dim, gd = a.goal_dim, ad = a.act_dim, OW = 2 * od + 3 * gd + ad + 2;
-  const int R = a.T + 1, t = a.t_idx[b] % R, t1 = (a.t_idx[b] + 1) % R, w = a.w_idx[b], tg = a.t_goal[b];
+  const int R = a.T + 1, t = ti % R, t1 = (ti + 1) % R;
   const int tt = a.term_t ? a.term_t[w] : -1;
   const float* r0 = a.rows + ((size_t)t * a.N + w) * a.W;
-  const float* r1 = (a.t_idx[b] + 1 == tt) ? a.term_rows + (size_t)w * a.W : a.rows + ((size_t)t1 * a.N + w) * a.W;
+  const float* r1 = (ti + 1 == tt) ? a.term_rows + (size_t)w * a.W : a.rows + ((size_t)t1 * a.N + w) * a.W;
   const float* g = tg < 0 ? r0 + od + gd : ((tg == tt ? a.term_rows + (size_t)w * a.W : a.rows + ((size_t)(tg % R) * a.N + w) * a.W) + od);
   float v;
   if (e < od + gd) v = r0[e];
@@ -1151,6 +1152,7 @@
   } else v = r1[e - (od + 2 * gd + ad + 1)];
   return v;
 }
+GRX_DEV float grx_her_word(const GrxHerArgs& a, long long b, int e) { return grx_her_word_at(a, a.t_idx[b], a.w_idx[b], a.t_goal[b], e); }
 extern "C" __global__ void __launch_bounds__(256)
 grx_her_relabel_kernel(GrxHerArgs a, long long B) {
   const int OW = 2 * a.obs_dim + 3 * a.goal_dim + a.act_dim + 2;
@@ -1487,19 +1489,19 @@
   return 0;
 }
 
+static __device__ __forceinline__ unsigned long long grx_order_key(const int* __restrict__ cost, float* __restrict__ ema, float alpha, int base, int per, int i) {
+  if (i >= per) return 0ull;
+  float c = (float)cost[base + i];
+  if (ema) { c = (1.0f - alpha) * ema[base + i] + alpha * c; ema[base + i] = c; }
+  const unsigned k = (unsigned)fminf(fmaxf(c * 16.0f, 0.0f), 4.0e9f);
+  return ((unsigned long long)k << 32) | (unsigned)(0x7FFFFFFF - i);
+}
+static __device__ void grx_order_place(const unsigned long long* keys, int s, int base, int per, int slots, int* __restrict__ order);
 extern "C" __global__ void __launch_bounds__(256)
 grx_order_kernel(const int* __restrict__ cost, float* __restrict__ ema, float alpha, int per, int npow2, int slots, int* __restrict__ order) {
   extern __shared__ unsigned long long keys[];
   const int s = blockIdx.x, base = s * per;
-  for (int i = threadIdx.x; i < npow2; i += 256) {
-    unsigned k = 0;
-    if (i < per) {
-      float c = (float)cost[base + i];
-      if (ema) { c = (1.0f - alpha) * ema[base + i] + alpha * c; ema[base + i] = c; }
-      k = (unsigned)fminf(fmaxf(c * 16.0f, 0.0f), 4.0e9f);
-    }
-    keys[i] = i < per ? (((unsigned long long)k << 32) | (unsigned)(0x7FFFFFFF - i)) : 0ull;
-  }
+  for (int i = threadIdx.x; i < npow2; i += 256) keys[i] = grx_order_key(cost, ema, alpha, base, per, i);
   __syncthreads();
   for (int k = 2; k <= npow2; k <<= 1)
     for (int j = k >> 1; j > 0; j >>= 1) {
@@ -1513,6 +1515,9 @@
       }
       __syncthreads();
     }
+  grx_order_place(keys, s, base, per, slots, order);
+}
+static __device__ void grx_order_place(const unsigned long long* keys, int s, int base, int per, int slots, int* __restrict__ order) {
   __shared__ int sM;
   if (threadIdx.x == 0) {
     int M = 0;
@@ -1657,6 +1662,29 @@
     if (b == 0) *valid = found ? (int)B : 0;
   }
 }
+#define GRX_HER_CHUNK 32
+extern "C" __global__ void __launch_bounds__(256)
+grx_her_draw_relabel_kernel(GrxHerArgs a, const int* __restrict__ start, const int* __restrict__ prev_start, int t_now, int k_future, unsigned long long seed,
+                            unsigned long long call, long long B, int* __restrict__ valid) {
+  __shared__ int s_t[GRX_HER_CHUNK], s_w[GRX_HER_CHUNK], s_g[GRX_HER_CHUNK], s_ok[GRX_HER_CHUNK];
+  const int OW = 2 * a.obs_dim + 3 * a.goal_dim + a.act_dim + 2, x = threadIdx.x;
+  for (long long b0 = (long long)blockIdx.x * GRX_HER_CHUNK; b0 < B; b0 += (long long)gridDim.x * GRX_HER_CHUNK) {
+    const int rows = B - b0 < GRX_HER_CHUNK ? (int)(B - b0) : GRX_HER_CHUNK;
+    if (x < rows) {
+      int t, w, tg;
+      const bool found = grx_her_draw(start, prev_start, a.term_t, a.N, t_now, a.T, k_future, seed, call, b0 + x, &t, &w, &tg);
+      s_t[x] = t; s_w[x] = w; s_g[x] = tg; s_ok[x] = (found || !valid) ? 1 : 0;
+      if (valid && b0 + x == 0) *valid = found ? (int)B : 0;
+    }
+    __syncthreads();
+    float* __restrict__ out = a.out + b0 * OW;
+    for (int i = x; i < rows * OW; i += 256) {
+      const int r = i / OW;
+      out[i] = s_ok[r] ? grx_her_word_at(a, s_t[r], s_w[r], s_g[r], i - r * OW) : 0.0f;
+    }
+    __syncthreads();
+  }
+}
 extern "C" int grx_her_sample_final(const int* episode_start, const int* prev_start, const int* term_t, int n_worlds, int t_now, int T, int k_future, uint64_t seed,
                                     uint64_t call, int64_t batch, int* t_idx, int* w_idx, int* t_goal, void* stream) {
   if (!episode_start || !t_idx || !w_idx || !t_goal) return fail("grx_her_sample: null argument");
@@ -1674,30 +1702,35 @@
                               int* t_idx, int* w_idx, int* t_goal, void* stream) {
   return grx_her_sample_final(episode_start, nullptr, nullptr, n_worlds, t_now, T, k_future, seed, call, batch, t_idx, w_idx, t_goal, stream);
 }
+static int grx_her_draw_relabel_impl(const char* who, const grx_her_args* args, const int* episode_start, const int* prev_start, int t_now, int k_future, uint64_t seed,
+                                     uint64_t call, int64_t batch, int* valid, void* stream) {
+  GrxHerArgs a; memcpy(&a, args, sizeof(a));
+  if (!a.rows || !a.acts || !a.out) return fail(std::string(who) + ": null buffer");
+  if ((a.term_rows == nullptr) != (a.term_t == nullptr) || (prev_start == nullptr) != (a.term_t == nullptr))
+    return fail(std::string(who) + ": term_rows, term_t and prev_start go together");
+  if (a.T <= 0 || a.N <= 0 || a.obs_dim <= 0 || a.goal_dim <= 0 || a.goal_dim > 16 || a.act_dim <= 0 || a.W < a.obs_dim + 2 * a.goal_dim)
+    return fail(std::string(who) + ": dimensions out of range (goal_dim <= 16, W >= obs_dim + 2 goal_dim)");
+  if (a.kind < 0 || a.kind > 3 || (a.kind == 0 && a.goal_dim != 3) || (a.kind == 2 && a.goal_dim != 2) || (a.kind == 3 && a.goal_dim != 7))
+    return fail(std::string(who) + ": reward kind does not fit goal_dim");
+  if (t_now < 0 || k_future < 0 || batch <= 0 || batch > (1ll << 30)) return fail(std::string(who) + ": t_now, k_future >= 0 and 1 <= batch <= 2^30");
+  a.t_idx = a.w_idx = a.t_goal = nullptr;
+  long long blocks = (batch + GRX_HER_CHUNK - 1) / GRX_HER_CHUNK;
+  if (blocks > 4096) blocks = 4096;
+  hipLaunchKernelGGL(grx_her_draw_relabel_kernel, dim3((unsigned)blocks), dim3(256), 0, (hipStream_t)stream, a, episode_start, prev_start, t_now, k_future,
+                     (unsigned long long)seed, (unsigned long long)call, (long long)batch, valid);
+  HIP_OK(hipGetLastError());
+  return 0;
+}
+extern "C" int grx_her_draw_relabel(const grx_her_args* args, const int* episode_start, const int* prev_start, int t_now, int k_future, uint64_t seed, uint64_t call,
+                                    int64_t batch, int* valid, void* stream) {
+  if (!args || !episode_start) return fail("grx_her_draw_relabel: null argument");
+  if (!valid && t_now <= 0) return fail("grx_her_draw_relabel: without valid the caller vouches for a world with a transition (t_now > 0)");
+  return grx_her_draw_relabel_impl("grx_her_draw_relabel", args, episode_start, prev_start, t_now, k_future, seed, call, batch, valid, stream);
+}
 extern "C" int grx_her_sample_relabel(const grx_her_args* args, const int* episode_start, const int* prev_start, int t_now, int k_future, uint64_t seed, uint64_t call,
                                       int64_t batch, int* scratch, int* valid, void* stream) {
   if (!args || !episode_start || !scratch || !valid) return fail("grx_her_sample_relabel: null argument");
-  GrxHerArgs a; memcpy(&a, args, sizeof(a));
-  if (!a.rows || !a.acts || !a.out) return fail("grx_her_sample_relabel: null buffer");
-  if ((a.term_rows == nullptr) != (a.term_t == nullptr) || (prev_start == nullptr) != (a.term_t == nullptr))
-    return fail("grx_her_sample_relabel: term_rows, term_t and prev_start go together");
-  if (a.T <= 0 || a.N <= 0 || a.obs_dim <= 0 || a.goal_dim <= 0 || a.goal_dim > 16 || a.act_dim <= 0 || a.W < a.obs_dim + 2 * a.goal_dim)
-    return fail("grx_her_sample_relabel: dimensions out of range (goal_dim <= 16, W >= obs_dim + 2 goal_dim)");
-  if (a.kind < 0 || a.kind > 3 || (a.kind == 0 && a.goal_dim != 3) || (a.kind == 2 && a.goal_dim != 2) || (a.kind == 3 && a.goal_dim != 7))
-    return fail("grx_her_sample_relabel: reward kind does not fit goal_dim");
-  if (t_now < 0 || k_future < 0 || batch <= 0 || batch > (1ll << 30)) return fail("grx_her_sample_relabel: t_now, k_future >= 0 and 1 <= batch <= 2^30");
-  a.t_idx = scratch; a.w_idx = scratch + batch; a.t_goal = scratch + 2 * batch;
-  long long blocks = (batch + 255) / 256;
-  if (blocks > 4096) blocks = 4096;
-  hipLaunchKernelGGL(grx_her_sample_valid_kernel, dim3((unsigned)blocks), dim3(256), 0, (hipStream_t)stream, episode_start, prev_start, a.term_t, a.N, t_now, a.T, k_future,
-                     (unsigned long long)seed, (unsigned long long)call, (long long)batch, scratch, scratch + batch, scratch + 2 * batch, valid);
-  HIP_OK(hipGetLastError());
-  const long long words = (long long)batch * (2 * a.obs_dim + 3 * a.goal_dim + a.act_dim + 2);
-  blocks = (words + 255) / 256;
-  if (blocks > 4096) blocks = 4096;
-  hipLaunchKernelGGL(grx_her_relabel_valid_kernel, dim3((unsigned)blocks), dim3(256), 0, (hipStream_t)stream, a, (long long)batch, (const int*)valid);
-  HIP_OK(hipGetLastError());
-  return 0;
+  return grx_her_draw_relabel_impl("grx_her_sample_relabel", args, episode_start, prev_start, t_now, k_future, seed, call, batch, valid, stream);
 }
 extern "C" __global__ void __launch_bounds__(256)
 grx_her_mark_kernel(const unsigned char* __restrict__ mask, int N, int t, int* __restrict__ start, int* __restrict__ prev_start, int* __restrict__ term_t) {
@@ -1710,6 +1743,47 @@
   if (!reset_mask || !episode_start || n_worlds <= 0) return fail("grx_her_mark_resets: null argument");
   if ((prev_start == nullptr) != (term_t == nullptr)) return fail("grx_her_mark_resets: prev_start and term_t go together");
   hipLaunchKernelGGL(grx_her_mark_kernel, dim3((unsigned)((n_worlds + 255) / 256)), dim3(256), 0, (hipStream_t)stream, reset_mask, n_worlds, t, episode_start, prev_start, term_t);
+  HIP_OK(hipGetLastError());
+  return 0;
+}
+
+static __device__ __forceinline__ void grx_her_mark(const grx_her_append_args& a, int w) {
+  if (a.prev_start) { a.prev_start[w] = a.start[w]; a.term_t[w] = a.t; }
+  a.start[w] = a.t;
+}
+extern "C" __global__ void __launch_bounds__(256)
+grx_her_append_kernel(grx_her_append_args a) {
+  const long long tid = (long long)blockIdx.x * blockDim.x + threadIdx.x, nth = (long long)gridDim.x * blockDim.x;
+  grx_copy_words(a.row_dst, a.packed, a.n_row, tid, nth);
+  grx_copy_words(a.act_dst, a.action, a.n_act, tid, nth);
+  if (a.mask)
+    for (long long w = tid; w < a.n_worlds; w += nth)
+      if (a.mask[w]) grx_her_mark(a, (int)w);
+  if (!a.list) return;
+  int k = a.count_dev ? *a.count_dev : a.count;
+  k = k < 0 ? 0 : (k > a.n_worlds ? a.n_worlds : k);
+  for (long long j = tid; j < k; j += nth) {
+    const int w = a.list[j];
+    if ((unsigned)w < (unsigned)a.n_worlds) grx_her_mark(a, w);
+  }
+  if (a.term_rows)
+    for (long long i = tid; i < (long long)k * a.W; i += nth) {
+      const long long j = i / a.W;
+      const int w = a.list[j];
+      if ((unsigned)w < (unsigned)a.n_worlds) a.term_rows[(size_t)w * a.W + (i - j * a.W)] = a.final_rows[i];
+    }
+}
+extern "C" int grx_her_append(const grx_her_append_args* args, void* stream) {
+  if (!args) return fail("grx_her_append: null argument");
+  const grx_her_append_args& a = *args;
+  if (!a.packed || !a.action || !a.row_dst || !a.act_dst || !a.start) return fail("grx_her_append: null buffer");
+  if (a.n_worlds <= 0 || a.n_row <= 0 || a.n_act <= 0 || a.W <= 0) return fail("grx_her_append: bad dimensions");
+  if ((a.prev_start == nullptr) != (a.term_t == nullptr)) return fail("grx_her_append: prev_start and term_t go together");
+  if (a.list && a.mask) return fail("grx_her_append: the reset worlds come as a list or as a mask, not both");
+  if ((a.term_rows == nullptr) != (a.final_rows == nullptr) || (a.term_rows && !a.list)) return fail("grx_her_append: final_rows and term_rows go together, with a list");
+  long long blocks = (a.n_row / 4 + 255) / 256;
+  blocks = blocks < 1 ? 1 : (blocks > 1024 ? 1024 : blocks);
+  hipLaunchKernelGGL(grx_her_append_kernel, dim3((unsigned)blocks), dim3(256), 0, (hipStream_t)stream, a);
   HIP_OK(hipGetLastError());
   return 0;
 }
@@ -1788,10 +1862,7 @@
   return 0;
 }
 
-extern "C" __global__ void __launch_bounds__(64)
-grx_fetch_commit_kernel(grx_fetch_commit_args a) {
-  const int j = blockIdx.x, l = threadIdx.x;
-  if (j >= a.k) return;
+static __device__ __forceinline__ void grx_fetch_commit_world(const grx_fetch_commit_args& a, int j, int l, float* __restrict__ rows) {
   const size_t w = (size_t)a.idx[j];
   const int od = a.obs_dim, pw = od + 8;
   for (int i = l; i < a.nq; i += 64) a.qpos[w * a.nq + i] = a.s_qpos[w * a.nq + i];
@@ -1803,18 +1874,110 @@
   for (int i = l; i < pw; i += 64) {
     const float old = a.packed[w * pw + i];
     if (a.final_packed) a.final_packed[w * pw + i] = old;
+    if (rows) rows[(size_t)j * pw + i] = old;
     a.packed[w * pw + i] = i < od ? a.s_obs[w * od + i] : (i < od + 3 ? a.s_achieved[w * 3 + i - od] : (i < od + 6 ? a.s_goal[w * 3 + i - od - 3] : old));
   }
   if (l == 0) a.status[w] = grx_status_word(a.status[w], a.s_status[w]);
+}
+extern "C" __global__ void __launch_bounds__(64)
+grx_fetch_commit_kernel(grx_fetch_commit_args a) {
+  if ((int)blockIdx.x < a.k) grx_fetch_commit_world(a, blockIdx.x, threadIdx.x, nullptr);
+}
+static int grx_fetch_commit_check(const grx_fetch_commit_args& a, const char* who) {
+  if (!a.idx || !a.s_qpos || !a.s_qvel || !a.s_qacc_ws || !a.s_aux || !a.s_goal || !a.s_obs || !a.s_achieved || !a.s_status || !a.qpos || !a.qvel || !a.qacc_ws || !a.aux ||
+      !a.goal || !a.obs || !a.achieved || !a.packed || !a.status || (a.mocap_words > 0 && (!a.s_mocap || !a.mocap))) return fail(std::string(who) + ": null buffer");
+  if (a.nq <= 0 || a.nv <= 0 || a.obs_dim <= 0 || a.mocap_words < 0) return fail(std::string(who) + ": bad dimensions");
+  return 0;
 }
 extern "C" int grx_fetch_commit_rows(const grx_fetch_commit_args* args, void* stream) {
   if (!args) return fail("grx_fetch_commit_rows: null argument");
   const grx_fetch_commit_args& a = *args;
-  if (!a.idx || !a.s_qpos || !a.s_qvel || !a.s_qacc_ws || !a.s_aux || !a.s_goal || !a.s_obs || !a.s_achieved || !a.s_status || !a.qpos || !a.qvel || !a.qacc_ws || !a.aux ||
-      !a.goal || !a.obs || !a.achieved || !a.packed || !a.status || (a.mocap_words > 0 && (!a.s_mocap || !a.mocap))) return fail("grx_fetch_commit_rows: null buffer");
-  if (a.nq <= 0 || a.nv <= 0 || a.obs_dim <= 0 || a.mocap_words < 0) return fail("grx_fetch_commit_rows: bad dimensions");
+  if (grx_fetch_commit_check(a, "grx_fetch_commit_rows")) return -1;
   if (a.k <= 0) return 0;
   hipLaunchKernelGGL(grx_fetch_commit_kernel, dim3((unsigned)a.k), dim3(64), 0, (hipStream_t)stream, a);
+  HIP_OK(hipGetLastError());
+  return 0;
+}
+
+template <int E>
+static __device__ __forceinline__ void grx_order_sort(unsigned long long* __restrict__ lds, const int* __restrict__ cost, float* __restrict__ ema, float alpha, int s, int per,
+                                                      int slots, int* __restrict__ order) {
+  constexpr int P = 256 * E;
+  const int x = threadIdx.x, base = s * per;
+  unsigned long long key[E];
+#pragma unroll
+  for (int e = 0; e < E; e++) key[e] = grx_order_key(cost, ema, alpha, base, per, x + 256 * e);
+  for (int k = 2; k <= P; k <<= 1)
+    for (int j = k >> 1; j > 0; j >>= 1) {
+      if (j >= 64) {
+#pragma unroll
+        for (int e = 0; e < E; e++) lds[x + 256 * e] = key[e];
+        __syncthreads();
+#pragma unroll
+        for (int e = 0; e < E; e++) {
+          const int i = x + 256 * e;
+          const unsigned long long o = lds[i ^ j];
+          const bool keep_max = ((i & k) == 0) == ((i & j) == 0);
+          key[e] = keep_max ? (key[e] > o ? key[e] : o) : (key[e] < o ? key[e] : o);
+        }
+        __syncthreads();
+      } else {
+#pragma unroll
+        for (int e = 0; e < E; e++) {
+          const int i = x + 256 * e;
+          const unsigned long long o = __shfl_xor(key[e], j);
+          const bool keep_max = ((i & k) == 0) == ((i & j) == 0);
+          key[e] = keep_max ? (key[e] > o ? key[e] : o) : (key[e] < o ? key[e] : o);
+        }
+      }
+    }
+#pragma unroll
+  for (int e = 0; e < E; e++) lds[x + 256 * e] = key[e];
+  __syncthreads();
+  grx_order_place(lds, s, base, per, slots, order);
+}
+extern "C" __global__ void __launch_bounds__(256)
+grx_fetch_post_step_kernel(const int* __restrict__ cost, float* __restrict__ ema, float alpha, int per, int epl, int slots, int* __restrict__ order, int n_sort,
+                           grx_fetch_commit_args a, float* __restrict__ rows) {
+  extern __shared__ unsigned long long post_keys[];
+  if ((int)blockIdx.x < n_sort) {
+    const int s = blockIdx.x;
+    switch (epl) {
+      case 1: grx_order_sort<1>(post_keys, cost, ema, alpha, s, per, slots, order); break;
+      case 2: grx_order_sort<2>(post_keys, cost, ema, alpha, s, per, slots, order); break;
+      case 4: grx_order_sort<4>(post_keys, cost, ema, alpha, s, per, slots, order); break;
+      case 8: grx_order_sort<8>(post_keys, cost, ema, alpha, s, per, slots, order); break;
+      case 16: grx_order_sort<16>(post_keys, cost, ema, alpha, s, per, slots, order); break;
+      default: grx_order_sort<32>(post_keys, cost, ema, alpha, s, per, slots, order); break;
+    }
+    return;
+  }
+  const int j = ((int)blockIdx.x - n_sort) * 4 + (int)(threadIdx.x >> 6);
+  if (j < a.k) grx_fetch_commit_world(a, j, threadIdx.x & 63, rows);
+}
+extern "C" int grx_fetch_post_step(const int* cost, float* ema, float alpha, int n_worlds, int slots_per_xcd, int* order, const grx_fetch_commit_args* commit, float* final_rows,
+                                   void* stream) {
+  int per = 0, epl = 1, n_sort = 0;
+  if (order) {
+    if (!cost) return fail("grx_fetch_post_step: order without cost");
+    if (ema && !(alpha > 0.0f && alpha <= 1.0f)) return fail("grx_fetch_post_step: alpha must be in (0, 1]");
+    if (n_worlds <= 0 || (n_worlds & 7)) return fail("grx_fetch_post_step: the number of worlds must be a positive multiple of 8 (one contiguous slice per XCD)");
+    per = n_worlds >> 3;
+    while (256 * epl < per) epl <<= 1;
+    if (epl > 32) return fail("grx_fetch_post_step: more than 65536 worlds per launch are not supported");
+    n_sort = 8;
+  }
+  grx_fetch_commit_args a;
+  memset(&a, 0, sizeof(a));
+  if (commit) {
+    a = *commit;
+    if (grx_fetch_commit_check(a, "grx_fetch_post_step")) return -1;
+    if (a.k < 0) a.k = 0;
+  }
+  const unsigned grid = (unsigned)n_sort + (unsigned)((a.k + 3) / 4);
+  if (grid == 0) return 0;
+  hipLaunchKernelGGL(grx_fetch_post_step_kernel, dim3(grid), dim3(256), n_sort ? (size_t)256 * epl * 8 : 0, (hipStream_t)stream, cost, ema, alpha, per, epl,
+                     slots_per_xcd < 0 ? 0 : slots_per_xcd, order, n_sort, a, final_rows);
   HIP_OK(hipGetLastError());
   return 0;
 }
diff --git a/gymnasium_robotics_amd/envs/fetch.py b/gymnasium_robotics_amd/envs/fetch.py
--- a/gymnasium_robotics_amd/envs/fetch.py
+++ b/gymnasium_robotics_amd/envs/fetch.py
@@ -134,7 +134,10 @@
                 l1.record()
                 self.step_events.append((l0, l1))
         if self.balance:
-            self._rebalance()
+            if self._defer_order:
+                self._order_pending = True
+            else:
+                self._rebalance()
 
     def _alloc(self, n):
         d, f32 = self.device, torch.float32
@@ -146,6 +149,9 @@
         self.mask = torch.ones(n, dtype=torch.uint8, device=d)
         self.balance = bool(self.balance) and n % 8 == 0 and 1024 <= n <= 65536 * 8
         self._reset_stage = z(n, 6)
+        self._fused = os.environ.get("GRX_FETCH_FUSED_TAIL", "1") != "0"
+        self._defer_order, self._order_pending = False, False
+        self.step_reset_list = None
         self.packed = z(n, self.obs_dim + 8)
         self.final_packed = z(n, self.obs_dim + 8)
         self.cost = torch.zeros(n, dtype=torch.int32, device=d) if self.balance else None
@@ -293,7 +299,14 @@
             done.record(self._ahead_stream)
         return staged, done
 
-    def _commit_ahead(self, ahead, idx):
+    def _post_step(self, commit=None, rows=None):
+        order = self._order_pending
+        self._order_pending = False
+        _native.check(self._L.grx_fetch_post_step(self.cost.data_ptr() if order else None, self.cost_ema.data_ptr() if order else None, self.balance_alpha, self.num_envs,
+                                                  self._slots_per_xcd, self.order.data_ptr() if order else None, None if commit is None else ctypes.byref(commit),
+                                                  None if rows is None else rows.data_ptr(), self._stream()))
+
+    def _commit_ahead(self, ahead, idx, rows=None):
         (n, idx_dev, _), done = ahead
         torch.cuda.current_stream(self.device).wait_event(done)
         A = self._ahead
@@ -302,7 +315,10 @@
                                           A["obs"].data_ptr(), A["achieved"].data_ptr(), A["status"].data_ptr(),
                                           self.qpos.data_ptr(), self.qvel.data_ptr(), self.qacc_ws.data_ptr(), self.mocap.data_ptr(), self.aux.data_ptr(), self.goal.data_ptr(),
                                           self.obs.data_ptr(), self.achieved.data_ptr(), self.packed.data_ptr(), self.final_packed.data_ptr(), self.status.data_ptr())
-        _native.check(self._L.grx_fetch_commit_rows(ctypes.byref(a), self._stream()))
+        if self._fused:
+            self._post_step(a, rows)
+        else:
+            _native.check(self._L.grx_fetch_commit_rows(ctypes.byref(a), self._stream()))
         self._elapsed[idx] = 0
         self._needs_reset[idx] = False
 
@@ -319,7 +335,7 @@
             self._seed_worlds(seeds)
         with torch.cuda.device(self.device):
             self._reset_worlds(np.arange(self.num_envs))
-        self._has_reset = True
+        self._has_reset, self.step_reset_list = True, None
         return self._obs_dict(), {}
 
     def step(self, actions):
@@ -344,12 +360,17 @@
                     before.record(torch.cuda.current_stream(self.device))
                 elif len(will):
                     ahead = (will, self._launch_reset_ahead(will))
+            self.step_reset_list = None
+            if self._order_pending:
+                self._post_step()
+            self._defer_order = self._fused and self.autoreset_mode == "same_step" and not len(pending)
             if len(pending):
                 self.mask.fill_(1)
                 self.mask.index_fill_(0, self._stage_idx(pending), 0)
                 self._launch_step(self._bufs_masked)
             else:
                 self._launch_step(self._bufs)
+            self._defer_order = False
             if before is not None:
                 ahead = (will, self._launch_reset_ahead(will, after=before))
             stepped = ~self._needs_reset if len(pending) else np.ones(self.num_envs, bool)
@@ -364,25 +385,33 @@
                 self.reward.index_fill_(0, tp, 0.0)
                 self.packed[:, -2].index_fill_(0, tp, 0.0)
             if self.autoreset_mode == "same_step" and truncated.any():
-                done = np.nonzero(truncated)[0]
+                done, fo = np.nonzero(truncated)[0], None
                 if ahead is not None:
                     if not np.array_equal(ahead[0], done):
+                        if self._order_pending:
+                            self._post_step()
                         raise RuntimeError("overlapped reset: the worlds reset ahead of the step are not the ones it truncated")
                     staged = ahead[1][0]
                     if self.output != "torch":
                         info["final_obs"] = self._obs_dict(rows=done)
-                    self._commit_ahead(ahead[1], done)
+                    elif self._fused:
+                        fo = torch.empty(len(done), self.obs_dim + 8, dtype=torch.float32, device=self.device)
+                    self._commit_ahead(ahead[1], done, rows=fo)
                 else:
                     staged = self._stage_reset(done)
                     if self.output != "torch":
                         info["final_obs"] = self._obs_dict(rows=done)
                     self._launch_reset(staged, done, keep_outcome=True)
+                self.step_reset_list = (staged[1], len(done))
                 if self.output == "torch":
-                    fo = self.final_packed[staged[1]]
+                    if fo is None:
+                        fo = self.final_packed[staged[1]]
                     info["final_obs"] = {"observation": fo[:, : self.obs_dim], "achieved_goal": fo[:, self.obs_dim: self.obs_dim + 3],
                                          "desired_goal": fo[:, self.obs_dim + 3: self.obs_dim + 6]}
             elif self.autoreset_mode == "next_step":
                 self._needs_reset |= truncated
+            if self._order_pending:
+                self._post_step()
         obs = self._obs_dict()
         if self.output == "torch":
             info["is_success"] = self.success
diff --git a/gymnasium_robotics_amd/her.py b/gymnasium_robotics_amd/her.py
--- a/gymnasium_robotics_amd/her.py
+++ b/gymnasium_robotics_amd/her.py
@@ -1,4 +1,5 @@
 import ctypes
+import os
 from typing import Optional
 
 import numpy as np
@@ -50,6 +51,8 @@
         self.t = 0
         self._seed, self._calls = int(seed), 0
         self._L = _native.lib()
+        self._fused = os.environ.get("GRX_FETCH_FUSED_TAIL", "1") != "0"
+        self._last_list = None
         self._mask_pin = [dict(buf=torch.empty(self.N, dtype=torch.bool, pin_memory=True), event=None) for _ in range(4)]
         self._mask_next, self._mask_dev = 0, torch.zeros(self.N, dtype=torch.bool, device=self.device)
 
@@ -66,6 +69,8 @@
             raise RuntimeError("episode buffer is full: call begin_episode()")
         self.t += 1
         r = self.t % self.R
+        if self._fused:
+            return self._append_fused(r, actions, packed_rows, reset_mask, final_rows)
         self.actions[r].copy_(actions)
         self.episode[r].copy_(packed_rows)
         if reset_mask is not None:
@@ -93,6 +98,52 @@
         elif self._final_rows is not None:
             self._just_ended = np.zeros(self.N, bool)
 
+    def _upload_mask(self, host):
+        slot = self._mask_pin[self._mask_next]
+        self._mask_next = (self._mask_next + 1) % len(self._mask_pin)
+        if slot["event"] is not None:
+            slot["event"].synchronize()
+        slot["buf"].numpy()[:] = host
+        self._mask_dev.copy_(slot["buf"], non_blocking=True)
+        slot["event"] = torch.cuda.Event()
+        slot["event"].record(torch.cuda.current_stream(self.device))
+        return self._mask_dev
+
+    def _append_fused(self, r, actions, packed_rows, reset_mask, final_rows):
+        dev_rows = lambda x, shape: (x if isinstance(x, torch.Tensor) else torch.as_tensor(np.asarray(x))).to(device=self.device, dtype=torch.float32).contiguous().view(shape)
+        acts, rows = dev_rows(actions, (self.N, self.act_dim)), dev_rows(packed_rows, (self.N, self.W))
+        a = _native.HerAppendArgsStruct()
+        a.packed, a.action, a.row_dst, a.act_dst = rows.data_ptr(), acts.data_ptr(), self.episode[r].data_ptr(), self.actions[r].data_ptr()
+        a.n_row, a.n_act, a.n_worlds, a.t, a.W = self.N * self.W, self.N * self.act_dim, self.N, self.t, self.W
+        a.start = self.episode_start.data_ptr()
+        keep = None
+        if reset_mask is not None:
+            host = (reset_mask.cpu().numpy() if isinstance(reset_mask, torch.Tensor) else np.asarray(reset_mask)).astype(bool)
+            self._start_host[host] = self.t
+            if final_rows is not None:
+                assert tuple(final_rows.shape) == (self.N, self.W) and final_rows.is_contiguous()
+                self._final_rows = final_rows
+            track = self._final_rows is not None
+            self._just_ended = host if track else self._just_ended
+            if track:
+                a.prev_start, a.term_t = self.prev_start.data_ptr(), self.term_t.data_ptr()
+            count, lst = int(host.sum()), getattr(self.env, "step_reset_list", None)
+            if lst is self._last_list:
+                lst = None
+            self._last_list = lst
+            if count == 0:
+                pass
+            elif lst is not None and lst[1] == count and lst[0].dtype == torch.int32 and lst[0].device == self.device:
+                a.list, a.count = lst[0].data_ptr(), count
+            elif isinstance(reset_mask, torch.Tensor) and reset_mask.device == self.device:
+                keep = reset_mask if reset_mask.dtype in (torch.bool, torch.uint8) else reset_mask.bool()
+                a.mask = keep.data_ptr()
+            else:
+                a.mask = self._upload_mask(host).data_ptr()
+        elif self._final_rows is not None:
+            self._just_ended = np.zeros(self.N, bool)
+        _native.check(self._L.grx_her_append(ctypes.byref(a), ctypes.c_void_p(torch.cuda.current_stream(self.device).cuda_stream)))
+
     def set_episode_start(self, starts):
         self._start_host[:] = np.asarray(starts, dtype=np.int64)
         self.episode_start.copy_(torch.from_numpy(self._start_host.astype(np.int32)).to(self.device))
@@ -100,9 +151,13 @@
     def reseed(self, seed: int):
         self._seed, self._calls = int(seed), 0
 
+    def _can_sample(self) -> bool:
+        track = self._final_rows is not None
+        return bool(((np.maximum(self._start_host, max(self.t - self.T, 0)) < self.t) | (self._just_ended if track else False)).any())
+
     def sample_indices(self, batch: int, k_future: int = 4):
         track = self._final_rows is not None
-        if not ((np.maximum(self._start_host, max(self.t - self.T, 0)) < self.t) | (self._just_ended if track else False)).any():
+        if not self._can_sample():
             return None
         t, w, tg = (torch.empty(batch, dtype=torch.int32, device=self.device) for _ in range(3))
         _native.check(self._L.grx_her_sample_final(self.episode_start.data_ptr(), self.prev_start.data_ptr() if track else None, self.term_t.data_ptr() if track else None,
@@ -111,15 +166,19 @@
         self._calls += 1
         return t, w, tg
 
-    def relabel_into(self, out: torch.Tensor, t: torch.Tensor, w: torch.Tensor, t_goal: torch.Tensor):
+    def _her_args(self, out: torch.Tensor):
         a = _native.HerArgsStruct()
-        a.rows, a.acts = self.episode.data_ptr(), self.actions.data_ptr()
+        a.rows, a.acts, a.out = self.episode.data_ptr(), self.actions.data_ptr(), out.data_ptr()
         a.T, a.N, a.W, a.obs_dim, a.goal_dim, a.act_dim = self.T, self.N, self.W, self.obs_dim, self.goal_dim, self.act_dim
-        a.t_idx, a.w_idx, a.t_goal, a.out = t.data_ptr(), w.data_ptr(), t_goal.data_ptr(), out.data_ptr()
         if self._final_rows is not None:
             a.term_rows, a.term_t = self._final_rows.data_ptr(), self.term_t.data_ptr()
         for k, v in self.spec.items():
             setattr(a, k, v)
+        return a
+
+    def relabel_into(self, out: torch.Tensor, t: torch.Tensor, w: torch.Tensor, t_goal: torch.Tensor):
+        a = self._her_args(out)
+        a.t_idx, a.w_idx, a.t_goal = t.data_ptr(), w.data_ptr(), t_goal.data_ptr()
         assert out.is_contiguous() and tuple(out.shape) == (len(t), self.OW) and t.dtype == w.dtype == t_goal.dtype == torch.int32
         _native.check(self._L.grx_her_relabel(ctypes.byref(a), len(t), ctypes.c_void_p(torch.cuda.current_stream(self.device).cuda_stream)))
         return out
@@ -129,12 +188,20 @@
             raise ValueError("batch larger than the replay capacity")
         if self.head + batch > self.capacity:
             self.head = 0
-        idx = self.sample_indices(batch, k_future)
-        if idx is None:
-            return self.rows[self.head: self.head]
-        t, w, tg = idx
         view = self.rows[self.head: self.head + batch]
-        self.relabel_into(view, t, w, tg)
+        if self._fused:
+            if not self._can_sample():
+                return self.rows[self.head: self.head]
+            track = self._final_rows is not None
+            _native.check(self._L.grx_her_draw_relabel(ctypes.byref(self._her_args(view)), self.episode_start.data_ptr(), self.prev_start.data_ptr() if track else None,
+                                                       self.t, int(k_future), self._seed, self._calls, batch, None,
+                                                       ctypes.c_void_p(torch.cuda.current_stream(self.device).cuda_stream)))
+            self._calls += 1
+        else:
+            idx = self.sample_indices(batch, k_future)
+            if idx is None:
+                return self.rows[self.head: self.head]
+            self.relabel_into(view, *idx)
         self.head += batch
         self.size = min(self.capacity, max(self.size, self.head))
         return view
diff --git a/include/grx_capi.h b/include/grx_capi.h
--- a/include/grx_capi.h
+++ b/include/grx_capi.h
@@ -242,6 +242,19 @@
 int grx_her_mark_resets(const unsigned char* reset_mask, int n_worlds, int t, int* episode_start, int* prev_start, int* term_t, void* stream);
 int grx_her_sample_relabel(const grx_her_args* args, const int* episode_start, const int* prev_start, int t_now, int k_future, uint64_t seed, uint64_t call, int64_t batch,
                            int* scratch, int* valid, void* stream);
+int grx_her_draw_relabel(const grx_her_args* args, const int* episode_start, const int* prev_start, int t_now, int k_future, uint64_t seed, uint64_t call, int64_t batch,
+                         int* valid, void* stream);
+typedef struct grx_her_append_args {
+  const float *packed, *action;
+  float *row_dst, *act_dst;
+  long long n_row, n_act;
+  const int* list; const int* count_dev;
+  const unsigned char* mask;
+  int count, n_worlds, t, W;
+  int *start, *prev_start, *term_t;
+  const float* final_rows; float* term_rows;
+} grx_her_append_args;
+int grx_her_append(const grx_her_append_args* args, void* stream);
 
 typedef struct grx_maze_reset_args {
   const int* idx; const float* stage; const float* qpos0;
@@ -290,6 +303,8 @@
   float *qpos, *qvel, *qacc_ws, *mocap, *aux, *goal, *obs, *achieved, *packed, *final_packed; int* status;
 } grx_fetch_commit_args;
 int grx_fetch_commit_rows(const grx_fetch_commit_args* args, void* stream);
+int grx_fetch_post_step(const int* cost, float* ema, float alpha, int n_worlds, int slots_per_xcd, int* order, const grx_fetch_commit_args* commit, float* final_rows,
+                        void* stream);
 
 typedef struct grx_adroit_commit_args {
   const int64_t* idx; int k;
```

Measured after the change: 1.444 million, median of 6. +1.2%, better.
